# Ericonaldo/ILSwiss

Hardware: AMD Instinct MI355X
Metric: env-steps/s + SAC grad-steps/s, Hopper-v2 4096 envs (higher is better)
Workload: dtype f32

## Files before the change

ilswiss_amd/_lib.py:

```python
import ctypes as C
import os

_HERE = os.path.dirname(os.path.abspath(__file__))
LIB_PATH = os.path.join(_HERE, "libilsx.so")

c_f32p = C.POINTER(C.c_float)
c_u8p = C.POINTER(C.c_uint8)
c_i64p = C.POINTER(C.c_int64)
vp = C.c_void_p


class MlpCfg(C.Structure):
    _fields_ = [("in_dim", C.c_int32), ("n_hidden", C.c_int32), ("hidden", C.c_int32),
                ("out_dim", C.c_int32), ("n_heads", C.c_int32), ("act", C.c_int32), ("hidden_sizes", C.c_int32 * 3)]


class SacCfg(C.Structure):
    _fields_ = [("reward_scale", C.c_float), ("discount", C.c_float), ("policy_lr", C.c_float),
                ("qf_lr", C.c_float), ("alpha_lr", C.c_float), ("soft_target_tau", C.c_float),
                ("alpha", C.c_float), ("train_alpha", C.c_int32),
                ("policy_mean_reg_weight", C.c_float), ("policy_std_reg_weight", C.c_float),
                ("beta_1", C.c_float), ("has_target_entropy", C.c_int32), ("target_entropy", C.c_float),
                ("max_batch", C.c_int32), ("grad_world", C.c_int32)]

# ... 152 lines not shown


PROTOTYPES = {
    "ilsx_sac_group_create": (C.c_int, [vp, C.POINTER(vp), C.c_int, C.POINTER(vp)]),
    "ilsx_sac_group_destroy": (C.c_int, [vp]),
    "ilsx_sac_group_train_from_replay": (C.c_int, [vp, C.POINTER(vp), C.c_int, C.c_int, C.c_int]),
    "ilsx_advirl_train": (C.c_int, [vp, vp, vp, vp, C.c_int, C.c_int, C.c_int, C.c_int, C.c_int, C.c_int, C.c_int, C.c_float,
                                    C.c_int, C.c_float, C.POINTER(DiscStats), C.POINTER(SacStats), vp]),
    "ilsx_net_set_noise_policy": (C.c_int, [vp, C.c_float, C.c_float, C.c_float]),
    "ilsx_net_set_output_linear": (C.c_int, [vp, C.c_int]),
    "ilsx_td3_create": (C.c_int, [vp, C.POINTER(Td3Cfg), vp, vp, vp, C.POINTER(vp)]),
    "ilsx_td3_destroy": (C.c_int, [vp]),
    "ilsx_td3_train_step": (C.c_int, [vp, vp, vp, vp, vp, vp, C.c_int, vp, C.POINTER(Td3Stats)]),
    "ilsx_td3_train_from_replay": (C.c_int, [vp, vp, C.c_int, C.c_int, C.POINTER(Td3Stats)]),
    "ilsx_td3_get_params": (C.c_int, [vp, C.c_int, vp, C.c_size_t]),
    "ilsx_td3_set_params": (C.c_int, [vp, C.c_int, vp, C.c_size_t]),
    "ilsx_sacv_create": (C.c_int, [vp, C.POINTER(SacvCfg), vp, vp, vp, vp, C.POINTER(vp)]),
    "ilsx_sacv_destroy": (C.c_int, [vp]),
    "ilsx_sacv_train_step": (C.c_int, [vp, vp, vp, vp, vp, vp, C.c_int, vp, C.POINTER(SacvStats)]),
    "ilsx_sacv_train_from_replay": (C.c_int, [vp, vp, C.c_int, C.c_int, C.POINTER(SacvStats)]),
    "ilsx_sacv_get_params": (C.c_int, [vp, C.c_int, vp, C.c_size_t]),
    "ilsx_sacv_set_params": (C.c_int, [vp, C.c_int, vp, C.c_size_t]),
    "ilsx_bc_create": (C.c_int, [vp, C.POINTER(BcCfg), vp, C.POINTER(vp)]),
    "ilsx_bc_destroy": (C.c_int, [vp]),
    "ilsx_bc_train_step": (C.c_int, [vp, vp, vp, C.c_int, vp, C.POINTER(C.c_float)]),
    "ilsx_bc_train_from_replay": (C.c_int, [vp, vp, C.c_int, C.c_int, C.POINTER(C.c_float)]),
    "ilsx_ppo_create": (C.c_int, [vp, C.POINTER(PpoCfg), C.POINTER(vp)]),
    "ilsx_ppo_destroy": (C.c_int, [vp]),
    "ilsx_ppo_num_params": (C.c_int, [vp, C.c_int, C.POINTER(C.c_size_t)]),
    "ilsx_ppo_set_params": (C.c_int, [vp, C.c_int, vp, C.c_size_t]),
    "ilsx_ppo_get_params": (C.c_int, [vp, C.c_int, vp, C.c_size_t]),
    "ilsx_ppo_gae": (C.c_int, [vp, vp, vp, vp, vp, C.c_int, vp, vp, vp, vp, vp]),
    "ilsx_ppo_values": (C.c_int, [vp, vp, C.c_int, vp]),
    "ilsx_ppo_train": (C.c_int, [vp, vp, vp, vp, vp, C.c_int, vp, vp]),
    "ilsx_rollout_step_relabel": (C.c_int, [vp, vp, vp, C.c_int, vp, C.c_int, C.c_int]),
    "ilsx_eval_rollout": (C.c_int, [vp, vp, vp, C.c_int, C.c_int, C.c_int, vp]),
    "ilsx_ppo_rollout": (C.c_int, [vp, vp, C.c_int, C.c_int, vp, vp, vp, vp, vp]),
    "ilsx_vecenv_set_obs_affine": (C.c_int, [vp, vp, vp]),
    "ilsx_is_terminal": (C.c_int, [vp, C.c_int, vp, C.c_int, C.c_int, vp]),
    "ilsx_vecenv_obs_norm": (C.c_int, [vp, C.c_int, C.c_int]),
    "ilsx_vecenv_get_obs_rms": (C.c_int, [vp, vp, vp, C.POINTER(C.c_double)]),
    "ilsx_vecenv_set_obs_rms": (C.c_int, [vp, vp, vp, C.c_double]),
    "ilsx_ppo_debug_perm": (C.c_int, [vp, C.c_int, C.c_uint32, vp]),
    "ilsx_ppo_debug_grad_norm": (C.c_int, [vp, C.POINTER(C.c_float)]),
    "ilsx_ppo_policy_act": (C.c_int, [vp, vp, C.c_int, C.c_int, vp, vp, vp]),
    "ilsx_disc_create": (C.c_int, [vp, C.POINTER(DiscCfg), C.POINTER(vp)]),
    "ilsx_advirl_set_policy_batch_from_expert": (C.c_int, [vp, C.c_int]),
    "ilsx_her_gather": (C.c_int, [vp, vp, vp, C.c_int, C.c_int, C.c_int, C.c_int, C.c_int, C.c_int, C.c_float, vp, vp, vp, vp, vp]),
    "ilsx_debug_rng_stream": (C.c_int, [vp, C.c_int, C.POINTER(C.c_uint32), C.POINTER(C.c_uint64)]),
    "ilsx_debug_philox": (C.c_int, [vp, C.c_uint64, C.c_uint64, C.c_uint32, C.c_int, C.c_int, vp, vp]),
    "ilsx_disc_destroy": (C.c_int, [vp]),
    "ilsx_disc_num_params": (C.c_int, [vp, C.POINTER(C.c_size_t)]),
    "ilsx_disc_set_params": (C.c_int, [vp, vp, C.c_size_t]),
    "ilsx_disc_get_params": (C.c_int, [vp, vp, C.c_size_t]),
    "ilsx_disc_get_grads": (C.c_int, [vp, vp, C.c_size_t]),
    "ilsx_disc_get_bn_stats": (C.c_int, [vp, vp, vp, C.c_size_t]),
    "ilsx_disc_set_bn_stats": (C.c_int, [vp, vp, vp, C.c_size_t]),
    "ilsx_disc_train_step": (C.c_int, [vp, vp, vp, vp, vp, C.c_int, vp, C.POINTER(DiscStats)]),
    "ilsx_disc_reward": (C.c_int, [vp, vp, vp, C.c_int, C.c_int, C.c_int, C.c_float, C.c_int, C.c_float, vp, vp]),
    "ilsx_vecenv_create": (C.c_int, [vp, C.POINTER(PlanarModel), C.c_int, C.c_uint64, C.POINTER(vp)]),
    "ilsx_vecenv_create_spatial": (C.c_int, [vp, C.POINTER(SpatialModel), C.c_int, C.c_uint64, C.POINTER(vp)]),
    "ilsx_vecenv_state_dims": (C.c_int, [vp, C.POINTER(C.c_int), C.POINTER(C.c_int)]),
    "ilsx_vecenv_set_path_mode": (C.c_int, [vp, C.c_int]),
    "ilsx_vecenv_destroy": (C.c_int, [vp]),
    "ilsx_vecenv_dims": (C.c_int, [vp, C.POINTER(C.c_int), C.POINTER(C.c_int), C.POINTER(C.c_int), C.POINTER(C.c_int)]),
    "ilsx_vecenv_reset": (C.c_int, [vp, vp, C.c_int, vp]),
    "ilsx_vecenv_step": (C.c_int, [vp, vp, vp, C.c_int, vp, vp, vp]),
    "ilsx_vecenv_get_state": (C.c_int, [vp, vp, vp]),
    "ilsx_vecenv_set_state": (C.c_int, [vp, vp, vp]),
    "ilsx_vecenv_cur_obs": (C.c_int, [vp, C.POINTER(vp)]),
    "ilsx_rollout_step": (C.c_int, [vp, vp, vp, C.c_int, C.c_int, C.c_int, C.c_int]),
    "ilsx_rollout_step_begin": (C.c_int, [vp, vp, vp, C.c_int, C.c_int, C.c_int, C.c_int]),
    "ilsx_rollout_step_end": (C.c_int, [vp]),
    "ilsx_eval_rollouts_lockstep": (C.c_int, [C.POINTER(vp), C.POINTER(vp), C.c_int, C.c_int, C.c_int, C.c_int64, C.POINTER(C.c_double)]),
    "ilsx_rollout_steps_lockstep": (C.c_int, [C.POINTER(vp), C.POINTER(vp), C.POINTER(vp), C.c_int, C.c_int, C.c_int, C.POINTER(C.c_int64), C.c_int, C.c_int]),
    "ilsx_rollout_stats": (C.c_int, [vp, C.POINTER(C.c_double), C.POINTER(C.c_double), C.c_int]),
    "ilsx_abi_version": (C.c_int, []),
    "ilsx_last_error": (C.c_char_p, []),
    "ilsx_ctx_create": (C.c_int, [C.c_int, vp, C.c_uint64, C.POINTER(vp)]),
    "ilsx_ctx_sync": (C.c_int, [vp]),
    "ilsx_ctx_destroy": (C.c_int, [vp]),
    "ilsx_ctx_stream": (vp, [vp]),
    "ilsx_ctx_rng_stream_cursor": (C.c_int, [vp, C.c_uint32, C.POINTER(C.c_uint32)]),
    "ilsx_ctx_alloc": (C.c_int, [vp, C.c_size_t, C.POINTER(vp)]),
    "ilsx_ctx_free": (C.c_int, [vp, vp]),
    "ilsx_memcpy_h2d": (C.c_int, [vp, vp, vp, C.c_size_t]),
    "ilsx_memcpy_d2h": (C.c_int, [vp, vp, vp, C.c_size_t]),
    "ilsx_comm_unique_id": (C.c_int, [vp]),
    "ilsx_comm_init": (C.c_int, [vp, vp, C.c_int, C.c_int]),
    "ilsx_comm_destroy": (C.c_int, [vp]),
    "ilsx_comm_info": (C.c_int, [vp, C.POINTER(C.c_int), C.POINTER(C.c_int)]),
    "ilsx_comm_allreduce_sum": (C.c_int, [vp, vp, C.c_size_t]),
    "ilsx_td3_get_opt": (C.c_int, [vp, C.c_int, vp, vp, C.c_size_t, C.POINTER(OptMeta)]),
    "ilsx_td3_set_opt": (C.c_int, [vp, C.c_int, vp, vp, C.c_size_t, C.POINTER(OptMeta)]),
    "ilsx_sacv_get_opt": (C.c_int, [vp, C.c_int, vp, vp, C.c_size_t, C.POINTER(OptMeta)]),
    "ilsx_sacv_set_opt": (C.c_int, [vp, C.c_int, vp, vp, C.c_size_t, C.POINTER(OptMeta)]),
    "ilsx_bc_get_opt": (C.c_int, [vp, vp, vp, C.c_size_t, C.POINTER(OptMeta)]),
    "ilsx_bc_set_opt": (C.c_int, [vp, vp, vp, C.c_size_t, C.POINTER(OptMeta)]),
    "ilsx_ppo_get_opt": (C.c_int, [vp, C.c_int, vp, vp, C.c_size_t, C.POINTER(OptMeta)]),
    "ilsx_ppo_set_opt": (C.c_int, [vp, C.c_int, vp, vp, C.c_size_t, C.POINTER(OptMeta)]),
    "ilsx_disc_get_opt": (C.c_int, [vp, vp, vp, C.c_size_t, C.POINTER(OptMeta)]),
    "ilsx_disc_set_opt": (C.c_int, [vp, vp, vp, C.c_size_t, C.POINTER(OptMeta)]),
    "ilsx_prof_enable": (C.c_int, [vp, C.c_int]),
    "ilsx_prof_reset": (C.c_int, [vp]),
    "ilsx_prof_read": (C.c_int, [vp, C.c_int, C.POINTER(C.c_uint64), C.POINTER(C.c_double)]),
    "ilsx_prof_kernel": (C.c_char_p, [vp, C.c_int]),
    "ilsx_kernel_name": (C.c_char_p, [C.c_int]),
    "ilsx_debug_set_stamp_buffer": (C.c_int, [vp, vp, C.c_int, C.POINTER(C.c_int)]),
    "ilsx_debug_dw_split": (C.c_int, [C.c_int, C.c_int, C.POINTER(C.c_int), C.POINTER(C.c_int)]),
    "ilsx_net_create": (C.c_int, [vp, C.POINTER(MlpCfg), C.POINTER(vp)]),
    "ilsx_net_destroy": (C.c_int, [vp]),
    "ilsx_net_num_params": (C.c_int, [vp, C.POINTER(C.c_size_t)]),
    "ilsx_net_init": (C.c_int, [vp, C.c_uint64, C.c_float, C.c_float]),
    "ilsx_net_set_params": (C.c_int, [vp, vp, C.c_size_t, C.c_int]),
    "ilsx_net_get_params": (C.c_int, [vp, vp, C.c_size_t, C.c_int]),
    "ilsx_mlp_forward": (C.c_int, [vp, vp, C.c_int, vp]),
    "ilsx_policy_act": (C.c_int, [vp, vp, C.c_int, C.c_int, vp, vp, vp]),
    "ilsx_policy_log_prob": (C.c_int, [vp, vp, vp, C.c_int, vp]),
    "ilsx_replay_create": (C.c_int, [vp, C.c_int64, C.c_int, C.c_int, C.c_uint64, C.POINTER(vp)]),
    "ilsx_replay_destroy": (C.c_int, [vp]),
    "ilsx_replay_add": (C.c_int, [vp, vp, vp, vp, vp, vp, C.c_int, vp, C.c_int]),
    "ilsx_replay_terminate_episode": (C.c_int, [vp]),
    "ilsx_replay_set_absorbing": (C.c_int, [vp, C.c_int64, C.c_int, vp]),
    "ilsx_replay_get_absorbing": (C.c_int, [vp, vp, C.c_int, vp]),
    "ilsx_replay_sample": (C.c_int, [vp, C.c_int, vp, vp, vp, vp, vp, vp, vp]),
    "ilsx_replay_sample_many": (C.c_int, [vp, C.c_int, C.c_int, vp]),
    "ilsx_replay_record_floats": (C.c_int, [vp, C.POINTER(C.c_int)]),
    "ilsx_replay_size": (C.c_int, [vp, c_i64p, c_i64p]),
    "ilsx_replay_clear": (C.c_int, [vp]),
    "ilsx_replay_traj_endpoints": (C.c_int, [vp, c_i64p, c_i64p, C.c_int, C.POINTER(C.c_int)]),
    "ilsx_sac_create": (C.c_int, [vp, C.POINTER(SacCfg), vp, vp, vp, C.POINTER(vp)]),
    "ilsx_sac_destroy": (C.c_int, [vp]),
    "ilsx_sac_train_step": (C.c_int, [vp, vp, vp, vp, vp, vp, C.c_int, vp, vp, C.POINTER(SacStats)]),
    "ilsx_sac_train_from_replay": (C.c_int, [vp, vp, C.c_int, C.c_int, C.POINTER(SacStats)]),
    "ilsx_sac_set_batch": (C.c_int, [vp, vp, vp, vp, vp, vp, C.c_int, vp, vp]),
    "ilsx_sac_critic_backward": (C.c_int, [vp]),
    "ilsx_sac_critic_update": (C.c_int, [vp]),
    "ilsx_sac_actor_backward": (C.c_int, [vp]),
    "ilsx_sac_actor_update": (C.c_int, [vp]),
    "ilsx_sac_last_stats": (C.c_int, [vp, C.POINTER(SacStats)]),
    "ilsx_sac_get_params": (C.c_int, [vp, C.c_int, vp, C.c_size_t, C.c_int]),
    "ilsx_sac_set_params": (C.c_int, [vp, C.c_int, vp, C.c_size_t, C.c_int]),
    "ilsx_sac_get_grads": (C.c_int, [vp, C.c_int, vp, C.c_size_t, C.c_int]),
    "ilsx_sac_grads_ptr": (C.c_int, [vp, C.c_int, C.POINTER(vp), C.POINTER(C.c_size_t)]),
    "ilsx_sac_get_log_alpha": (C.c_int, [vp, C.POINTER(C.c_double)]),
    "ilsx_sac_set_log_alpha": (C.c_int, [vp, C.c_double]),
    "ilsx_sac_get_adam": (C.c_int, [vp, C.c_int, vp, vp, C.c_size_t, c_i64p]),
    "ilsx_sac_set_adam": (C.c_int, [vp, C.c_int, vp, vp, C.c_size_t, C.c_int64]),
    "ilsx_sac_get_alpha_opt": (C.c_int, [vp, C.POINTER(C.c_double), C.POINTER(C.c_double), c_i64p, C.POINTER(C.c_uint64)]),
    "ilsx_sac_debug_batch": (C.c_int, [vp, vp, C.c_uint64, C.c_int, vp, vp, vp, vp, vp, vp, vp, vp]),
    "ilsx_sac_debug_last_batch": (C.c_int, [vp, C.c_int, vp, vp, vp, vp, vp, vp]),
    "ilsx_sac_phase_state": (C.c_int, [vp, C.POINTER(C.c_int), C.POINTER(C.c_int), C.POINTER(C.c_int), C.POINTER(C.c_int), C.POINTER(C.c_int)]),
    "ilsx_sac_debug_break_phase": (C.c_int, [vp]),
    "ilsx_sac_set_alpha_opt": (C.c_int, [vp, C.c_double, C.c_double, C.c_int64, C.c_uint64]),
    "ilsx_bnn_create": (C.c_int, [vp, C.POINTER(BnnCfg), C.POINTER(vp)]),
    "ilsx_bnn_destroy": (C.c_int, [vp]),
    "ilsx_bnn_num_params": (C.c_int, [vp, C.POINTER(C.c_size_t)]),
    "ilsx_bnn_init": (C.c_int, [vp, C.c_uint64]),
    "ilsx_bnn_get_params": (C.c_int, [vp, vp, C.c_size_t]),
    "ilsx_bnn_set_params": (C.c_int, [vp, vp, C.c_size_t]),
    "ilsx_bnn_get_opt": (C.c_int, [vp, vp, vp, C.c_size_t, C.POINTER(OptMeta)]),
    "ilsx_bnn_set_opt": (C.c_int, [vp, vp, vp, C.c_size_t, C.POINTER(OptMeta)]),
    "ilsx_bnn_set_normalizer": (C.c_int, [vp, vp, vp]),
    "ilsx_bnn_get_normalizer": (C.c_int, [vp, vp, vp]),
    "ilsx_bnn_fit_stats": (C.c_int, [vp, vp, vp, C.c_int]),
    "ilsx_bnn_train_batch": (C.c_int, [vp, vp, vp, C.c_int64, C.c_int, vp]),
    "ilsx_bnn_mse": (C.c_int, [vp, vp, vp, C.c_int64, C.c_int, C.c_int, vp]),
    "ilsx_bnn_predict": (C.c_int, [vp, vp, C.c_int, vp, vp, C.c_int]),
    "ilsx_bnn_debug_padding": (C.c_int, [vp, C.POINTER(C.c_double)]),
    "ilsx_net_set_categorical": (C.c_int, [vp, C.c_int]),
    "ilsx_policy_log_pis": (C.c_int, [vp, vp, C.c_int, vp]),
    "ilsx_vecenv_create_classic": (C.c_int, [vp, C.c_int, C.c_int, C.c_uint64, C.POINTER(vp)]),
    "ilsx_vecenv_create_cartchain": (C.c_int, [vp, C.POINTER(CartChainModel), C.c_int, C.c_uint64, C.POINTER(vp)]),
    "ilsx_vecenv_create_swimmer": (C.c_int, [vp, C.POINTER(SwimmerModel), C.c_int, C.c_uint64, C.POINTER(vp)]),
    "ilsx_vecenv_action_space": (C.c_int, [vp, C.POINTER(C.c_int)]),
    "ilsx_dsac_create": (C.c_int, [vp, C.POINTER(DsacCfg), vp, vp, vp, C.POINTER(vp)]),
    "ilsx_dsac_destroy": (C.c_int, [vp]),
    "ilsx_dsac_train_step": (C.c_int, [vp, vp, vp, vp, vp, vp, C.c_int, C.POINTER(DsacStats)]),
    "ilsx_dsac_train_from_replay": (C.c_int, [vp, vp, C.c_int, C.c_int, C.POINTER(DsacStats)]),
    "ilsx_dsac_get_params": (C.c_int, [vp, C.c_int, vp, C.c_size_t]),
    "ilsx_dsac_set_params": (C.c_int, [vp, C.c_int, vp, C.c_size_t]),
    "ilsx_dsac_get_opt": (C.c_int, [vp, C.c_int, vp, vp, C.c_size_t, C.POINTER(OptMeta)]),
    "ilsx_dsac_set_opt": (C.c_int, [vp, C.c_int, vp, vp, C.c_size_t, C.POINTER(OptMeta)]),
    "ilsx_mbpo_model_step": (C.c_int, [vp, vp, vp, C.c_int, vp, vp, C.c_int, vp, C.c_int, C.c_int, vp, vp, vp, vp, vp,
                                       C.POINTER(C.c_int)]),
    "ilsx_her_horizon_gather": (C.c_int, [vp, vp, vp, C.c_int, C.c_int, C.c_int, C.c_int, C.c_int, vp, vp, vp]),
    "ilsx_bncat_create": (C.c_int, [vp, C.c_int, C.c_int, C.c_int, C.c_int, C.c_int, C.POINTER(vp)]),
    "ilsx_bncat_destroy": (C.c_int, [vp]),
    "ilsx_bncat_num_params": (C.c_int, [vp, C.POINTER(C.c_int)]),
    "ilsx_bncat_get": (C.c_int, [vp, C.c_int, vp, C.c_size_t]),
    "ilsx_bncat_set": (C.c_int, [vp, C.c_int, vp, C.c_size_t]),
    "ilsx_bncat_get_meta": (C.c_int, [vp, C.POINTER(C.c_int64), C.POINTER(C.c_uint64)]),
    "ilsx_bncat_set_meta": (C.c_int, [vp, C.c_int64, C.c_uint64]),
    "ilsx_bncat_input": (C.c_int, [vp, C.POINTER(vp), C.POINTER(vp)]),
    "ilsx_bncat_train_step": (C.c_int, [vp, C.c_int, C.c_float, vp]),
    "ilsx_bncat_act": (C.c_int, [vp, vp, C.c_int, C.c_int, vp, vp]),
    "ilsx_gcsl_create": (C.c_int, [vp, C.POINTER(GcslCfg), vp, vp, C.c_int, C.POINTER(vp)]),
    "ilsx_gcsl_destroy": (C.c_int, [vp]),
    "ilsx_gcsl_train_from_replay": (C.c_int, [vp, vp, vp, vp, C.c_int, vp]),
    "ilsx_gcsl_train_step": (C.c_int, [vp, vp, vp, C.c_int, vp]),
}

_lib = None


def load():
    global _lib
    if _lib is not None:
        return _lib
    path = os.environ.get("ILSX_LIB", LIB_PATH)
    if not os.path.exists(path):
        raise RuntimeError(
            f"{path} is missing: build it with `python -c 'import __graft_entry__ as g; g.build()'` "
            "or `make -C ilswiss_amd/csrc`.  ilswiss_amd has no CPU fallback.")
    lib = C.CDLL(path)
    for name, (res, args) in PROTOTYPES.items():
        fn = getattr(lib, name)
        fn.restype = res
        fn.argtypes = args
    if lib.ilsx_abi_version() != 1:
        raise RuntimeError(f"libilsx ABI {lib.ilsx_abi_version()} != 1")
    _lib = lib
    return lib


ILSX_ERR_UNSUPPORTED = -5


def check(rc):
    if rc != 0:
        msg = load().ilsx_last_error()
        raise RuntimeError(f"libilsx error {rc}: {msg.decode() if msg else '?'}")
```

ilswiss_amd/csrc/bwd_split_tile.inc:

```
  constexpr int NTH = 4 * H / CS, NWV = NTH / 64, NC = H / 16, SLW = H / CS, RPW = 16 / NWV, KPL = SLW / 64;
  constexpr int RPT = 16 * H / NTH, RSTEP = NTH / H;
  constexpr int LDH = H + ILSX_LDS_PAD, LDSL = SLW + ILSX_LDS_PAD;
  constexpr int MR = 16 * MT;
  static_assert(NTH % H == 0 && RPW >= 1 && KPL >= 1, "unsupported split geometry");
  static_assert(MT == 1 || MT == 2 || MT == 4, "macro tile = 1, 2 or 4 row tiles");
  const NetView& N = T.net;
  const int NO = N.NO;
  float* d1 = smem;
  float* d0s = d1 + MR * LDH;
  float* dout = d0s + MR * LDSL;
  if (bx & ((1u << A.xs) - 1u)) return;
  if ((int)(bx >> A.xs) * MR >= A.rows) return;
  const int tid = threadIdx.x, lane = tid & 63, wave = tid >> 6, li = lane & 15, g = lane >> 4;
  const int r0 = (bx >> A.xs) * MR, rows = A.rows;
  const bool lead = cs == 0;
  const bool full_tile = r0 + MR <= rows;
  ILSX_STAMP(A.dbg, 0);

  const int k1 = tid % H, rb1 = tid / H;
  const int lc = wave * 16 + li, col0 = cs * SLW + lc;
  float h1v[MT > 1 ? 2 : 1][RPT];
  float h0v[MT][4];
  float4 wreg[NC];
  constexpr int WHP = 12;
  float whp[WHP];
#pragma unroll
  for (int j = 0; j < WHP; ++j) whp[j] = (N.base + N.off_Wh)[(size_t)(j < NO ? j : 0) * H + k1];
  constexpr int DXT = 2;
  static_assert(SLW / 16 == NWV, "one k16 chunk of the slice per wave in the dL/dx phase");
  float w0b[DXT][4];
  if (T.dx) {
    const float* W0 = N.base + N.off_W[0];
    const int ld0 = N.ld[0];
#pragma unroll
    for (int t = 0; t < DXT; ++t)
#pragma unroll
      for (int s4 = 0; s4 < 4; ++s4) {
        const int c = 16 * t + li;
        w0b[t][s4] = c < T.dx_cols ? W0[pack_f(cs * SLW + 16 * wave + 4 * g + s4, T.dx_col0 + c, ld0)] : 0.0f;
      }
  }
  if constexpr (XCH) {
    {
      const float* wp = N.base + N.off_Wb[1] + (size_t)(cs * NWV + wave) * NC * 256 + 4 * lane;
#pragma unroll
      for (int c = 0; c < NC; ++c) wreg[c] = *reinterpret_cast<const float4*>(wp + 256 * c);
    }
  }
  XCH_HOOK_ACT
  {
    const float* const h1p = T.hsave[1] + (size_t)(r0 + rb1) * H + k1;
    const float* const h0p = T.hsave[0] + (size_t)(r0 + 4 * g) * H + col0;
    if (full_tile) {
#pragma unroll
      for (int i = 0; i < RPT; ++i) h1v[0][i] = ldx<XCH>(h1p + (size_t)(RSTEP * i) * H);
#pragma unroll
      for (int m = 0; m < MT; ++m)
#pragma unroll
        for (int v = 0; v < 4; ++v) h0v[m][v] = ldx<XCH>(h0p + (size_t)(16 * m + v) * H);
    } else {
#pragma unroll
      for (int i = 0; i < RPT; ++i) {
        const int gr = r0 + rb1 + RSTEP * i;
        h1v[0][i] = gr < rows ? ldx<XCH>(h1p + (size_t)(RSTEP * i) * H) : 0.0f;
      }
#pragma unroll
      for (int m = 0; m < MT; ++m)
#pragma unroll
        for (int v = 0; v < 4; ++v) {
          const int gr = r0 + 16 * m + 4 * g + v;
          h0v[m][v] = gr < rows ? ldx<XCH>(h0p + (size_t)(16 * m + v) * H) : 0.0f;
        }
    }
  }
  XCH_HOOK_HEAD
  for (int e = tid; e < MR * NO; e += NTH) {
    const int row = e / NO, j = e - row * NO, gr = r0 + row;
    float d = 0.0f;
    if (gr < rows) {
      d = bwd_head_grad<XCH>(T, A, gr, j, NO);
      if (T.dhead && lead) T.dhead[(size_t)gr * NO + j] = d;
    }
    dout[row * ILSX_MAX_NO + j] = d;
  }
  constexpr bool LATEW = GRP == 3 && MT == 1 && !XCH;
  if constexpr (!XCH && !LATEW) {
    {
      const float* wp = N.base + N.off_Wb[1] + (size_t)(cs * NWV + wave) * NC * 256 + 4 * lane;
#pragma unroll
      for (int c = 0; c < NC; ++c) wreg[c] = *reinterpret_cast<const float4*>(wp + 256 * c);
    }
  }
  lds_barrier();
  ILSX_STAMP(A.dbg, 1);
#pragma unroll
  for (int m = 0; m < MT; ++m) {
    if (m + 1 < MT) {
#pragma unroll
      for (int i = 0; i < RPT; ++i) {
        const int gr = r0 + 16 * (m + 1) + rb1 + RSTEP * i;
        h1v[(m + 1) & 1][i] = gr < rows ? T.hsave[1][(size_t)gr * H + k1] : 0.0f;
      }
    }
    const float* Wh = N.base + N.off_Wh;
    const float* dom = dout + 16 * m * ILSX_MAX_NO;
    float accd[RPT];
#pragma unroll
    for (int i = 0; i < RPT; ++i) accd[i] = 0.0f;
#pragma unroll
    for (int j = 0; j < WHP; ++j) {
      if (j < NO) {
#pragma unroll
        for (int i = 0; i < RPT; ++i) accd[i] = fmaf(dom[(rb1 + RSTEP * i) * ILSX_MAX_NO + j], whp[j], accd[i]);
      }
    }
#pragma unroll 4
    for (int j = WHP; j < NO; ++j) {
      const float w = Wh[(size_t)j * H + k1];
#pragma unroll
      for (int i = 0; i < RPT; ++i) accd[i] = fmaf(dom[(rb1 + RSTEP * i) * ILSX_MAX_NO + j], w, accd[i]);
    }
    float* ds = lead ? T.dsave[1] : nullptr;
    float* const dsp = ds ? ds + (size_t)(r0 + 16 * m + rb1) * H + k1 : nullptr;
    if (full_tile) {
#pragma unroll
      for (int i = 0; i < RPT; ++i) {
        const float dv = accd[i] * act_grad_from_out<ACT>(h1v[m & 1][i]);
        if (ds) dsp[(size_t)(RSTEP * i) * H] = dv;
        d1[(16 * m + rb1 + RSTEP * i) * LDH + k1] = dv;
      }
    } else {
#pragma unroll
      for (int i = 0; i < RPT; ++i) {
        const int row = 16 * m + rb1 + RSTEP * i, gr = r0 + row;
        float dv = 0.0f;
        if (gr < rows) {
          dv = accd[i] * act_grad_from_out<ACT>(h1v[m & 1][i]);
          if (ds) dsp[(size_t)(RSTEP * i) * H] = dv;
        }
        d1[row * LDH + k1] = dv;
      }
    }
  }
  if constexpr (LATEW) {
    const float* wp = N.base + N.off_Wb[1] + (size_t)(cs * NWV + wave) * NC * 256 + 4 * lane;
#pragma unroll
    for (int c = 0; c < NC; ++c) wreg[c] = *reinterpret_cast<const float4*>(wp + 256 * c);
  }
  lds_barrier();
  ILSX_STAMP(A.dbg, 2);
  {
    f32x4 acc0[MT], acc1[MT];
#pragma unroll
    for (int m = 0; m < MT; ++m) { acc0[m] = (f32x4){0.f, 0.f, 0.f, 0.f}; acc1[m] = acc0[m]; }
    const float* ap = d1 + li * LDH + 4 * g;
#pragma unroll
    for (int c = 0; c < NC; ++c) {
#pragma unroll
      for (int m = 0; m < MT; ++m) {
        const float4 a = *reinterpret_cast<const float4*>(ap + m * 16 * LDH + 16 * c);
        acc0[m] = MFMA16(a.x, wreg[c].x, acc0[m]); acc1[m] = MFMA16(a.y, wreg[c].y, acc1[m]);
        acc0[m] = MFMA16(a.z, wreg[c].z, acc0[m]); acc1[m] = MFMA16(a.w, wreg[c].w, acc1[m]);
      }
    }
    float* ds = T.dsave[0];
#pragma unroll
    for (int m = 0; m < MT; ++m) {
      float* const drow = ds ? ds + (size_t)(r0 + 16 * m + 4 * g) * H + col0 : nullptr;
      if (full_tile) {
#pragma unroll
        for (int v = 0; v < 4; ++v) {
          const float dv = (acc0[m][v] + acc1[m][v]) * act_grad_from_out<ACT>(h0v[m][v]);
          if (ds) drow[v * H] = dv;
          d0s[(16 * m + 4 * g + v) * LDSL + lc] = dv;
        }
      } else {
#pragma unroll
        for (int v = 0; v < 4; ++v) {
          const int row = 16 * m + 4 * g + v, gr = r0 + row;
          float dv = 0.0f;
          if (gr < rows) {
            dv = (acc0[m][v] + acc1[m][v]) * act_grad_from_out<ACT>(h0v[m][v]);
            if (ds) drow[v * H] = dv;
          }
          d0s[row * LDSL + lc] = dv;
        }
      }
    }
  }
  ILSX_STAMP(A.dbg, 3);
  if (T.dx) {
    lds_barrier();
    float* red = d1;
    const int ntile = (T.dx_cols + 15) >> 4;
#pragma unroll
    for (int m = 0; m < MT; ++m) {
      const float4 a4 = *reinterpret_cast<const float4*>(d0s + (16 * m + li) * LDSL + 16 * wave + 4 * g);
#pragma unroll
      for (int t = 0; t < DXT; ++t) {
        if (t < ntile) {
          f32x4 acc = (f32x4){0.f, 0.f, 0.f, 0.f};
          acc = MFMA16(a4.x, w0b[t][0], acc); acc = MFMA16(a4.y, w0b[t][1], acc);
          acc = MFMA16(a4.z, w0b[t][2], acc); acc = MFMA16(a4.w, w0b[t][3], acc);
#pragma unroll
          for (int v = 0; v < 4; ++v) red[(((m * DXT + t) * NWV + wave) * 4 + v) * 64 + lane] = acc[v];
        }
      }
    }
    lds_barrier();
#pragma unroll
    for (int m = 0; m < MT; ++m)
    for (int e = tid; e < ntile * 256; e += NTH) {
      const int t = e >> 8, v = (e >> 6) & 3, ol = e & 63;
      float sum = 0.0f;
#pragma unroll
      for (int w2 = 0; w2 < NWV; ++w2) sum += red[(((m * DXT + t) * NWV + w2) * 4 + v) * 64 + ol];
      const int row = 16 * m + 4 * (ol >> 4) + v, c = 16 * t + (ol & 15), gr = r0 + row;
      if (c < T.dx_cols && gr < rows) stx<XCH>(T.dx + ((size_t)cs * A.part_stride + gr) * T.dx_cols + c, sum);
    }
  }
  ILSX_STAMP(A.dbg, 7);
```

ilswiss_amd/csrc/fwd_split_tile.inc:

```
  constexpr int NTH = 4 * H / CS, NWV = NTH / 64, NC = H / 16, SLW = H / CS, NCS = SLW / 16;
  constexpr int NT0 = PH == 1 ? 1 : CS;
  constexpr int LDH = H + ILSX_LDS_PAD, LDSL = SLW + ILSX_LDS_PAD;
  constexpr int MR = 16 * MT;
  static_assert(NCS == NWV, "one k16 chunk of the slice per wave in the head phase");
  static_assert(MT == 1 || MT == 2 || MT == 4, "macro tile = 1, 2 or 4 row tiles");
  const DevScalars* scal = GRP ? GP->scal : A.scal;
  const NetView& N = T.net;
  const int KP = N.KP, LDX = KP + ILSX_LDS_PAD, NO = N.NO, NCH0 = KP >> 4, NOT = (NO + 15) >> 4;
  float* xs = smem;
  float* h0 = xs + (PH == 2 && MT > 1 ? 0 : MR * LDX);
  float* hs = h0 + (PH == 1 && MT > 1 ? 0 : MR * LDH);
  float* red = hs + MR * LDSL;
  const int RNT = MT == 1 ? 4 : NOT;
  if (bx & ((1u << A.xs) - 1u)) return;
  if ((int)(bx >> A.xs) * (A.rt > 0 ? A.rt : 1) * MR >= A.rows) return;
  const int tid = threadIdx.x, lane = tid & 63, wave = tid >> 6, li = lane & 15, g = lane >> 4;
  const int rows = A.rows;
  const int RT = A.rt > 0 ? A.rt : 1;
  const bool lead = cs == 0;
  ILSX_STAMP(A.dbg, 0);

  const int ct0 = PH == 1 ? cs * NWV + wave : wave * CS;
  const float* w0p = N.base + N.off_W[0] + (size_t)ct0 * NCH0 * 256 + 4 * lane;
  constexpr int L0D = 8;
  float4 b0[NT0], b0first[NT0];
  float4 l0first[PH == 1 ? L0D : 1];
  float bias0[NT0];
  if constexpr (PH == 1) {
#pragma unroll
    for (int d = 0; d < L0D; ++d) l0first[d] = *reinterpret_cast<const float4*>(w0p + (size_t)(d < NCH0 ? d : 0) * 256);
  }
  if constexpr (PH != 2) {
#pragma unroll
    for (int i = 0; i < NT0; ++i) b0[i] = *reinterpret_cast<const float4*>(w0p + (size_t)i * NCH0 * 256);
#pragma unroll
    for (int i = 0; i < NT0; ++i) b0first[i] = b0[i];
#pragma unroll
    for (int i = 0; i < NT0; ++i) bias0[i] = (N.base + N.off_b[0])[(ct0 + i) * 16 + li];
  }
  const int lc = wave * 16 + li, col1 = cs * SLW + lc;
  float bias1 = 0.0f;
  float4 whf[4];
  float4 wreg[NC];
  constexpr bool LATEW = GRP == 3 && MT == 1 && PH == 0;
  if constexpr (PH != 1) {
    bias1 = (N.base + N.off_b[1])[col1];
#pragma unroll
    for (int t = 0; t < 4; ++t) {
      const int j = 16 * t + li;
      whf[t] = (t < NOT && j < NO) ? *reinterpret_cast<const float4*>(N.base + N.off_Wh + (size_t)j * H + cs * SLW + 16 * wave + 4 * g)
                                   : make_float4(0.f, 0.f, 0.f, 0.f);
    }
    if constexpr (!LATEW) {
      const float* wp = N.base + N.off_W[1] + (size_t)(cs * NWV + wave) * NC * 256 + 4 * lane;
#pragma unroll
      for (int c = 0; c < NC; ++c) wreg[c] = *reinterpret_cast<const float4*>(wp + 256 * c);
    }
  }
#ifdef XCH_FINE_DBG
  ILSX_STAMP_SYNC(XCH_FINE_DBG, 6);
#endif
  const bool fin = (GRP ? GP->fin_on : A.fin_on) != 0 && !T.no_fin && T.d1 > 0;
  const GatherSpec& G = GRP ? GP->gather : A.gather;
  for (int rt = 0; rt < RT; ++rt) {
  const int r0 = ((bx >> A.xs) * RT + rt) * MR;
  if (r0 >= rows) break;
  const bool full_tile = r0 + MR <= rows;
  bool fin_logp = false;
  if constexpr (PH != 2) {
#pragma unroll
  for (int i = 0; i < NT0; ++i) b0[i] = b0first[i];
  XCH_HOOK_STAGE
  if constexpr (PH == 0) {
    long long* ridx0 = reinterpret_cast<long long*>(hs);
    if constexpr (MT > 1 || GRP != 0) {
      if (G.on) {
        if (tid < MR) ridx0[tid] = r0 + tid < rows ? replay_draw(G.seed, scal->gather_step, G.stream, (uint32_t)(r0 + tid), G.st->size) : 0;
        lds_barrier();
      }
    }
    for (int e = tid; e < MR * KP; e += NTH) {
      const int r = e / KP, k = e - r * KP, gr = r0 + r;
      const bool act_col = k >= T.d0 && k < T.d0 + T.d1;
      if (fin && act_col) continue;
      float v = 0.0f;
      if (gr < rows) {
        if (G.on) {
          long long idx;
          if constexpr (MT > 1 || GRP != 0) idx = ridx0[r];
          else idx = replay_draw(G.seed, scal->gather_step, G.stream, (uint32_t)gr, G.st->size);
          const float* rec = G.records + (size_t)idx * G.rec;
          if (k < T.d0) v = rec[T.g0_off + k];
          else if (act_col) v = rec[T.g1_off + (k - T.d0)];
          if (lead && T.publish == 1) {
            if (k < T.d0) G.s[(size_t)gr * G.o + k] = v;
            else if (act_col) G.a[(size_t)gr * G.adim + (k - T.d0)] = v;
            if (k == 0) { stx<XCH>(G.r + gr, rec[G.o + G.adim]); stx<XCH>(G.d + gr, rec[G.o + G.adim + 1]); }
          } else if (lead && T.publish == 2 && k < T.d0) {
            G.s2[(size_t)gr * G.o + k] = v;
          }
        } else {
          if (k < T.d0) v = T.x0[(size_t)gr * T.s0 + k];
          else if (act_col) v = T.x1[(size_t)gr * T.s1 + (k - T.d0)];
        }
        if (T.xsave && lead) T.xsave[(size_t)gr * KP + k] = v;
      }
      xs[r * LDX + k] = v;
    }
  } else {
    auto stage = [&](int r, int k, int gr, const float* rec) {
      const bool act_col = k >= T.d0 && k < T.d0 + T.d1;
      if (fin && act_col) return;
      float v = 0.0f;
      if (gr < rows) {
        if (G.on) {
          if (k < T.d0) v = rec[T.g0_off + k];
          else if (act_col) v = rec[T.g1_off + (k - T.d0)];
          if (lead && T.publish == 1) {
            if (k < T.d0) G.s[(size_t)gr * G.o + k] = v;
            else if (act_col) G.a[(size_t)gr * G.adim + (k - T.d0)] = v;
            if (k == 0) { G.r[gr] = rec[G.o + G.adim]; G.d[gr] = rec[G.o + G.adim + 1]; }
          } else if (lead && T.publish == 2 && k < T.d0) {
            G.s2[(size_t)gr * G.o + k] = v;
          }
        } else {
          if (k < T.d0) v = T.x0[(size_t)gr * T.s0 + k];
          else if (act_col) v = T.x1[(size_t)gr * T.s1 + (k - T.d0)];
        }
        if (T.xsave && lead) T.xsave[(size_t)gr * KP + k] = v;
      }
      xs[r * LDX + k] = v;
    };
    long long* ridx = reinterpret_cast<long long*>(hs);
    if (G.on) {
      if (tid < MR) ridx[tid] = r0 + tid < rows ? replay_draw(G.seed, scal->gather_step, G.stream, (uint32_t)(r0 + tid), G.st->size) : 0;
      lds_barrier();
    }
    if (KP <= 512 && T.d1 <= 64) {
      constexpr int RW = 16 / NWV, U = 8;
      const bool acts = T.d1 > 0 && !fin;
#pragma unroll
      for (int mt = 0; mt < MT; ++mt) {
      float vo[RW][U], va[RW];
#pragma unroll
      for (int rr = 0; rr < RW; ++rr) {
        const int r = 16 * mt + wave + NWV * rr, grc = r0 + r < rows ? r0 + r : rows - 1;
        const float* rec = G.on ? G.records + (size_t)ridx[r] * G.rec : nullptr;
        const float* s0p = G.on ? rec + T.g0_off : T.x0 + (size_t)grc * T.s0;
#pragma unroll
        for (int u = 0; u < U; ++u) { const int k = lane + 64 * u; vo[rr][u] = s0p[k < T.d0 ? k : T.d0 - 1]; }
        va[rr] = 0.0f;
        if (acts) { const float* s1p = G.on ? rec + T.g1_off : T.x1 + (size_t)grc * T.s1; va[rr] = s1p[lane < T.d1 ? lane : T.d1 - 1]; }
      }
#pragma unroll
      for (int rr = 0; rr < RW; ++rr) {
        const int r = 16 * mt + wave + NWV * rr, gr = r0 + r;
        const bool rowok = gr < rows;
        const bool pub1 = G.on && lead && T.publish == 1 && rowok, pub2 = G.on && lead && T.publish == 2 && rowok, xsv = T.xsave && lead && rowok;
#pragma unroll
        for (int u = 0; u < U; ++u) {
          const int k = lane + 64 * u;
          if (k < T.d0) {
            const float x = rowok ? vo[rr][u] : 0.0f;
            if (pub1) G.s[(size_t)gr * G.o + k] = x;
            if (pub2) G.s2[(size_t)gr * G.o + k] = x;
            if (xsv) T.xsave[(size_t)gr * KP + k] = x;
            xs[r * LDX + k] = x;
          }
        }
        if (acts && lane < T.d1) {
          const float x = rowok ? va[rr] : 0.0f;
          if (pub1) G.a[(size_t)gr * G.adim + lane] = x;
          if (xsv) T.xsave[(size_t)gr * KP + T.d0 + lane] = x;
          xs[r * LDX + T.d0 + lane] = x;
        }
        if (pub1 && lane == 0) { const float* rec = G.records + (size_t)ridx[r] * G.rec; G.r[gr] = rec[G.o + G.adim]; G.d[gr] = rec[G.o + G.adim + 1]; }
        for (int k = T.d0 + T.d1 + lane; k < KP; k += 64) {
          if (xsv) T.xsave[(size_t)gr * KP + k] = 0.0f;
          xs[r * LDX + k] = 0.0f;
        }
        if (T.d1 > 0 && !acts) {  }
      }
      }
    } else {
      for (int r = wave; r < MR; r += NWV) {
        const int gr = r0 + r;
        const float* rec = G.on ? G.records + (size_t)ridx[r] * G.rec : nullptr;
        for (int k = lane; k < KP; k += 64) stage(r, k, gr, rec);
      }
    }
  }
  XCH_HOOK_FIN
  if (fin) {
    const PolicyFinishArgs& P = GRP ? GP->fin : A.fin;
    const bool det = P.head == HEAD_DET_TANH_NOISE || P.head == HEAD_DET_LIN_NOISE;
    const int a = P.a, NOp = det ? a : 2 * a;
    const bool pub = lead && (GRP ? T.first != 0 : first_task);
    float* lp3 = red;
    const unsigned long long fstep = P.scal ? (P.use_gather_step ? P.scal->gather_step : P.scal->step) : P.step_host;
    const int LPS = MT == 1 ? 32 : a;
    for (int e = tid; e < MR * a; e += NTH) {
      const int row = e / a, j = e - row * a, gr = r0 + row;
      float act = 0.0f, c0 = 0.0f, c1 = 0.0f, c2 = 0.0f;
      if (gr < rows) {
        float pm[4], pl[4];
#pragma unroll
// ... 15 lines not shown
            const int q = j & 3;
            ep = q == 0 ? z4[0] : q == 1 ? z4[1] : q == 2 ? z4[2] : z4[3];
          }
        }
        if (det) {
          act = P.max_act * (P.head == HEAD_DET_LIN_NOISE ? mu : tanhf(mu));
          if (P.noise != 0.0f) act += fminf(fmaxf(P.noise * ep, -P.noise_clip), P.noise_clip);
          if (pub && P.raw) stx<XCH>(P.raw + (size_t)gr * a + j, mu);
        } else {
          const float ls = fminf(fmaxf(lsr, LOG_SIG_MIN), LOG_SIG_MAX);
          const float sd = expf(ls);
          const float z = ep * sd + mu;
          act = tanhf(z);
          const float dm = mu - z;
          c0 = dm * dm / expf(2.0f * ls); c1 = ls; c2 = logf(1.0f - act * act + TANH_EPS);
          if (pub && P.raw) { stx<XCH>(P.raw + (size_t)gr * NOp + j, mu); stx<XCH>(P.raw + (size_t)gr * NOp + a + j, lsr); }
        }
        if (T.xsave && lead) T.xsave[(size_t)gr * KP + T.d0 + j] = act;
        if (pub) {
          if (P.action) stx<XCH>(P.action + (size_t)gr * a + j, act);
          if (P.eps_save) stx<XCH>(P.eps_save + (size_t)gr * a + j, ep);
        }
      }
      xs[row * LDX + T.d0 + j] = act;
      lp3[(row * LPS + j) * 3 + 0] = c0; lp3[(row * LPS + j) * 3 + 1] = c1; lp3[(row * LPS + j) * 3 + 2] = c2;
    }
    fin_logp = pub && P.logp && !det;
  }
  }
  else {
    const float* hsrc = T.hsave[0];
    for (int e = tid; e < MR * (H / 4); e += NTH) {
      const int row = e / (H / 4), c4 = e - row * (H / 4), gr = r0 + row;
      const float4 v = gr < rows ? *reinterpret_cast<const float4*>(hsrc + (size_t)gr * H + 4 * c4) : make_float4(0.f, 0.f, 0.f, 0.f);
      *reinterpret_cast<float4*>(h0 + row * LDH + 4 * c4) = v;
    }
  }
  lds_barrier();
  ILSX_STAMP(A.dbg, 1);
  if (fin_logp && tid < MR && r0 + tid < rows) {
    const PolicyFinishArgs& P = GRP ? GP->fin : A.fin;
    float q = 0.f, l = 0.f, jc = 0.f;
    const int LPS = MT == 1 ? 32 : P.a;
    for (int j = 0; j < P.a; ++j) { q += red[(tid * LPS + j) * 3]; l += red[(tid * LPS + j) * 3 + 1]; jc += red[(tid * LPS + j) * 3 + 2]; }
    stx<XCH>(P.logp + r0 + tid, -0.5f * q - (l + HALF_LOG_2PI) - jc);
  }
  if constexpr (PH == 1) {
    f32x4 acc[MT];
#pragma unroll
    for (int m = 0; m < MT; ++m) acc[m] = (f32x4){0.f, 0.f, 0.f, 0.f};
    const float* ap = xs + li * LDX + 4 * g;
    float4 cur[L0D], nxt[L0D];
#pragma unroll
    for (int d = 0; d < L0D; ++d) cur[d] = l0first[d];
    for (int cb = 0; cb < NCH0; cb += L0D) {
#pragma unroll
      for (int d = 0; d < L0D; ++d) {
        const int c = cb + L0D + d;
        nxt[d] = *reinterpret_cast<const float4*>(w0p + (size_t)(c < NCH0 ? c : 0) * 256);
      }
#pragma unroll
      for (int d = 0; d < L0D; ++d) {
        if (cb + d < NCH0) {
#pragma unroll
          for (int m = 0; m < MT; ++m) {
            const float4 a = *reinterpret_cast<const float4*>(ap + m * 16 * LDX + 16 * (cb + d));
            acc[m] = MFMA16(a.x, cur[d].x, acc[m]); acc[m] = MFMA16(a.y, cur[d].y, acc[m]);
            acc[m] = MFMA16(a.z, cur[d].z, acc[m]); acc[m] = MFMA16(a.w, cur[d].w, acc[m]);
          }
        }
      }
#pragma unroll
      for (int d = 0; d < L0D; ++d) cur[d] = nxt[d];
    }
    float* hsv = T.hsave[0];
    const int col = ct0 * 16 + li;
#pragma unroll
    for (int m = 0; m < MT; ++m)
#pragma unroll
      for (int v = 0; v < 4; ++v) {
        const int row = 16 * m + 4 * g + v;
        if (r0 + row < rows) hsv[(size_t)(r0 + row) * H + col] = act_fn<ACT>(acc[m][v] + bias0[0]);
      }
  } else if constexpr (PH != 2) {
#pragma unroll
    for (int m = 0; m < MT; ++m) {
    f32x4 acc[NT0];
#pragma unroll
    for (int i = 0; i < NT0; ++i) acc[i] = (f32x4){0.f, 0.f, 0.f, 0.f};
    if (m > 0) {
#pragma unroll
      for (int i = 0; i < NT0; ++i) b0[i] = b0first[i];
    }
    const float* ap = xs + (16 * m + li) * LDX + 4 * g;
    for (int kc = 0; kc < KP; kc += 16) {
      float4 bn[NT0];
#pragma unroll
      for (int i = 0; i < NT0; ++i) {
        bn[i] = b0[i];
        if (kc + 16 < KP) bn[i] = *reinterpret_cast<const float4*>(w0p + (size_t)i * NCH0 * 256 + (kc + 16) * 16);
      }
      const float4 a = *reinterpret_cast<const float4*>(ap + kc);
#pragma unroll
      for (int i = 0; i < NT0; ++i) acc[i] = MFMA16(a.x, b0[i].x, acc[i]);
#pragma unroll
      for (int i = 0; i < NT0; ++i) acc[i] = MFMA16(a.y, b0[i].y, acc[i]);
#pragma unroll
      for (int i = 0; i < NT0; ++i) acc[i] = MFMA16(a.z, b0[i].z, acc[i]);
#pragma unroll
      for (int i = 0; i < NT0; ++i) acc[i] = MFMA16(a.w, b0[i].w, acc[i]);
#pragma unroll
      for (int i = 0; i < NT0; ++i) b0[i] = bn[i];
    }
    float* hsv = (PH == 1 || lead) ? T.hsave[0] : nullptr;
    float* const hrow = hsv ? hsv + (size_t)(r0 + 16 * m + 4 * g) * H + ct0 * 16 + li : nullptr;
#pragma unroll
    for (int i = 0; i < NT0; ++i) {
      const int col = (ct0 + i) * 16 + li;
#pragma unroll
      for (int v = 0; v < 4; ++v) {
        const int row = 16 * m + 4 * g + v;
        const float h = act_fn<ACT>(acc[i][v] + bias0[i]);
        if constexpr (PH == 0) h0[row * LDH + col] = h;
        acc[i][v] = h;
      }
    }
    if (hsv) {
      if (full_tile) {
#pragma unroll
        for (int i = 0; i < NT0; ++i)
#pragma unroll
          for (int v = 0; v < 4; ++v) stx<XCH>(hrow + v * H + i * 16, acc[i][v]);
      } else {
#pragma unroll
        for (int i = 0; i < NT0; ++i)
#pragma unroll
          for (int v = 0; v < 4; ++v)
            if (r0 + 16 * m + 4 * g + v < rows) stx<XCH>(hrow + v * H + i * 16, acc[i][v]);
      }
    }
    }
  }
  if constexpr (PH == 1) {
    lds_barrier();
    continue;
  }
  if constexpr (PH == 0) lds_barrier();
  ILSX_STAMP(A.dbg, 2);
  if constexpr (LATEW) {
    const float* wp = N.base + N.off_W[1] + (size_t)(cs * NWV + wave) * NC * 256 + 4 * lane;
#pragma unroll
    for (int c = 0; c < NC; ++c) wreg[c] = *reinterpret_cast<const float4*>(wp + 256 * c);
  }
  {
    f32x4 acc0[MT], acc1[MT];
#pragma unroll
    for (int m = 0; m < MT; ++m) { acc0[m] = (f32x4){0.f, 0.f, 0.f, 0.f}; acc1[m] = acc0[m]; }
    const float* ap = h0 + li * LDH + 4 * g;
#pragma unroll
    for (int c = 0; c < NC; ++c) {
#pragma unroll
      for (int m = 0; m < MT; ++m) {
        const float4 a = *reinterpret_cast<const float4*>(ap + m * 16 * LDH + 16 * c);
        acc0[m] = MFMA16(a.x, wreg[c].x, acc0[m]); acc1[m] = MFMA16(a.y, wreg[c].y, acc1[m]);
        acc0[m] = MFMA16(a.z, wreg[c].z, acc0[m]); acc1[m] = MFMA16(a.w, wreg[c].w, acc1[m]);
      }
    }
    float* hsv = T.hsave[1];
#pragma unroll
    for (int m = 0; m < MT; ++m) {
      float* const hrow = hsv ? hsv + (size_t)(r0 + 16 * m + 4 * g) * H + col1 : nullptr;
#pragma unroll
      for (int v = 0; v < 4; ++v) {
        const int row = 16 * m + 4 * g + v;
        const float h = act_fn<ACT>(acc0[m][v] + acc1[m][v] + bias1);
        hs[row * LDSL + lc] = h;
        acc0[m][v] = h;
      }
      if (hsv) {
        if (full_tile) {
#pragma unroll
          for (int v = 0; v < 4; ++v) stx<XCH>(hrow + v * H, acc0[m][v]);
        } else {
#pragma unroll
          for (int v = 0; v < 4; ++v)
            if (r0 + 16 * m + 4 * g + v < rows) stx<XCH>(hrow + v * H, acc0[m][v]);
        }
      }
    }
  }
  lds_barrier();
  ILSX_STAMP(A.dbg, 3);
#pragma unroll
  for (int m = 0; m < MT; ++m) {
    const float4 a = *reinterpret_cast<const float4*>(hs + (16 * m + li) * LDSL + 16 * wave + 4 * g);
#pragma unroll
    for (int t = 0; t < 4; ++t) {
      if (t < NOT) {
        f32x4 acc = (f32x4){0.f, 0.f, 0.f, 0.f};
        acc = MFMA16(a.x, whf[t].x, acc); acc = MFMA16(a.y, whf[t].y, acc);
        acc = MFMA16(a.z, whf[t].z, acc); acc = MFMA16(a.w, whf[t].w, acc);
#pragma unroll
        for (int v = 0; v < 4; ++v) red[(((m * RNT + t) * NWV + wave) * 4 + v) * 64 + lane] = acc[v];
      }
    }
  }
  lds_barrier();
  const float* bh = N.base + N.off_bh;
#pragma unroll
  for (int m = 0; m < MT; ++m)
  for (int e = tid; e < NOT * 256; e += NTH) {
    const int t = e >> 8, v = (e >> 6) & 3, ol = e & 63;
    float sum = 0.0f;
#pragma unroll
    for (int w2 = 0; w2 < NWV; ++w2) sum += red[(((m * RNT + t) * NWV + w2) * 4 + v) * 64 + ol];
    const int row = 16 * m + 4 * (ol >> 4) + v, j = 16 * t + (ol & 15), gr = r0 + row;
    if (j < NO && gr < rows) stx<XCH>(T.part + ((size_t)cs * A.part_stride + gr) * NO + j, sum + (lead ? bh[j] : 0.0f));
  }
  lds_barrier();
  }
  ILSX_STAMP(A.dbg, 7);
```

ilswiss_amd/csrc/ilsx_core.hip:

```cpp
#include <algorithm>
#include <cmath>
#include <cstdlib>
#include <random>

#define ILSX_KERNEL_IMPL 1
#include <mutex>
#include "host_common.h"

static thread_local std::string g_err = "";

void ilsx_set_err(const char* fmt, ...) {
  char buf[1024];
  va_list ap;
  va_start(ap, fmt);
  vsnprintf(buf, sizeof buf, fmt, ap);
  va_end(ap);
  g_err = buf;
}

static int kernels_init_once();
extern "C" int ilsx_abi_version(void) { return ILSX_ABI_VERSION; }
extern "C" const char* ilsx_last_error(void) { return g_err.c_str(); }

int ctx_alloc(ilsx_ctx* c, size_t bytes, void** out, bool zero) {
// ... 173 lines not shown
  static const char* names[ILSX_K_COUNT] = {"k_mlp_fwd", "k_mlp_bwd_dx", "k_mlp_bwd_dw", "k_adam_polyak",
      "k_replay_sample", "k_replay_add", "k_replay_sample_many", "k_sac_stats", "k_sac_finish", "k_env_step",
      "k_policy_finish", "k_disc_bwd", "k_ppo_gae", "k_sac_phase_a", "k_sac_phase_c", ""};
  return (kid >= 0 && kid < ILSX_K_COUNT) ? names[kid] : "";
}

static inline int round_up(int x, int m) { return (x + m - 1) / m * m; }

int net_layout_build(const ilsx_mlp_cfg& cfg, NetLayout* L) {
  if (cfg.n_hidden < 1 || cfg.n_hidden > ILSX_MAX_HID)
    ILSX_FAIL(ILSX_ERR_UNSUPPORTED, "n_hidden=%d not in 1..%d", cfg.n_hidden, ILSX_MAX_HID);
  if (cfg.hidden != 64 && cfg.hidden != 128 && cfg.hidden != 256)
    ILSX_FAIL(ILSX_ERR_UNSUPPORTED, "hidden=%d: supported widths are 64, 128, 256", cfg.hidden);
  if (cfg.in_dim < 1 || cfg.in_dim > 1024) ILSX_FAIL(ILSX_ERR_ARG, "in_dim=%d out of range", cfg.in_dim);
  if (cfg.n_heads < 1 || cfg.n_heads > 2 || cfg.out_dim < 1 || cfg.n_heads * cfg.out_dim > ILSX_MAX_NO)
    ILSX_FAIL(ILSX_ERR_UNSUPPORTED, "heads: n_heads=%d out_dim=%d (n_heads*out_dim must be <= %d)", cfg.n_heads,
              cfg.out_dim, ILSX_MAX_NO);
  if (cfg.act != ILSX_ACT_RELU && cfg.act != ILSX_ACT_TANH) ILSX_FAIL(ILSX_ERR_ARG, "act=%d unknown", cfg.act);
  L->cfg = cfg;
  for (int l = 0; l < ILSX_MAX_HID; ++l) {
    const int hs = l < cfg.n_hidden ? cfg.hidden_sizes[l] : 0;
    if (hs < 0 || hs > cfg.hidden) ILSX_FAIL(ILSX_ERR_UNSUPPORTED, "hidden_sizes[%d]=%d: 1..hidden=%d (0 = hidden)", l, hs, cfg.hidden);
    L->hl[l] = hs > 0 ? hs : (l < cfg.n_hidden ? cfg.hidden : 0);
    L->cfg.hidden_sizes[l] = l < cfg.n_hidden ? L->hl[l] : 0;
  }
  L->KP = round_up(cfg.in_dim, 16);
  L->NO = cfg.n_heads * cfg.out_dim;
  const int H = cfg.hidden;
  size_t off = 0, nflat = 0;
  for (int l = 0; l < cfg.n_hidden; ++l) {
    L->ld[l] = l == 0 ? L->KP : H;
    L->off_W[l] = (int)off;
    off += (size_t)H * L->ld[l];
    L->off_Wb[l] = 0;
    if (l > 0) {
      L->off_Wb[l] = (int)off;
      off += (size_t)H * H;
    }
    L->off_b[l] = (int)off;
    off += H;
    nflat += (size_t)L->out_of(l) * L->in_of(l) + L->out_of(l);
  }
  L->off_Wh = (int)off;
  off += (size_t)L->NO * H;
  L->off_bh = (int)off;
  off += round_up(L->NO, 4);
  nflat += (size_t)L->NO * L->out_of(cfg.n_hidden - 1) + L->NO;
  L->n_int = off;
  L->n_flat = nflat;
  return ILSX_OK;
}

void net_flat_to_internal(const NetLayout& L, const float* flat, float* in) {
  std::fill(in, in + L.n_int, 0.0f);
  const int H = L.cfg.hidden;
  size_t f = 0;
  for (int l = 0; l < L.cfg.n_hidden; ++l) {
    const int ind = L.in_of(l), outd = L.out_of(l);
    for (int n = 0; n < outd; ++n)
      for (int k = 0; k < ind; ++k) {
        const float v = flat[f + (size_t)n * ind + k];
        in[L.off_W[l] + pack_f(n, k, L.ld[l])] = v;
        if (l > 0) in[L.off_Wb[l] + pack_b(n, k, H)] = v;
      }
    f += (size_t)outd * ind;
    for (int n = 0; n < outd; ++n) in[L.off_b[l] + n] = flat[f + n];
    f += outd;
  }
  const int od = L.cfg.out_dim, hlast = L.out_of(L.cfg.n_hidden - 1);
  for (int h = 0; h < L.cfg.n_heads; ++h) {
    for (int j = 0; j < od; ++j)
      for (int k = 0; k < hlast; ++k) in[L.off_Wh + (size_t)(h * od + j) * H + k] = flat[f + (size_t)j * hlast + k];
    f += (size_t)od * hlast;
    for (int j = 0; j < od; ++j) in[L.off_bh + h * od + j] = flat[f + j];
    f += od;
  }
}

void net_internal_to_flat(const NetLayout& L, const float* in, float* flat) {
  const int H = L.cfg.hidden;
  size_t f = 0;
  for (int l = 0; l < L.cfg.n_hidden; ++l) {
    const int ind = L.in_of(l), outd = L.out_of(l);
    for (int n = 0; n < outd; ++n)
      for (int k = 0; k < ind; ++k) flat[f + (size_t)n * ind + k] = in[L.off_W[l] + pack_f(n, k, L.ld[l])];
    f += (size_t)outd * ind;
    for (int n = 0; n < outd; ++n) flat[f + n] = in[L.off_b[l] + n];
    f += outd;
  }
  const int od = L.cfg.out_dim, hlast = L.out_of(L.cfg.n_hidden - 1);
  for (int h = 0; h < L.cfg.n_heads; ++h) {
    for (int j = 0; j < od; ++j)
      for (int k = 0; k < hlast; ++k) flat[f + (size_t)j * hlast + k] = in[L.off_Wh + (size_t)(h * od + j) * H + k];
    f += (size_t)od * hlast;
    for (int j = 0; j < od; ++j) flat[f + j] = in[L.off_bh + h * od + j];
    f += od;
  }
}

NetView net_view(const NetLayout& L, float* base) {
  NetView v;
  v.base = base;
  for (int l = 0; l < ILSX_MAX_HID; ++l) {
    v.off_W[l] = l < L.cfg.n_hidden ? L.off_W[l] : 0;
    v.off_Wb[l] = l < L.cfg.n_hidden ? L.off_Wb[l] : 0;
    v.off_b[l] = l < L.cfg.n_hidden ? L.off_b[l] : 0;
    v.ld[l] = l < L.cfg.n_hidden ? L.ld[l] : 0;
  }
  v.off_Wh = L.off_Wh;
  v.off_bh = L.off_bh;
  v.nhid = L.cfg.n_hidden;
  v.H = L.cfg.hidden;
  v.in_dim = L.cfg.in_dim;
  v.KP = L.KP;
  v.NO = L.NO;
  return v;
}

static size_t fwd_lds_bytes(int H, int KP) {
  return sizeof(float) * (16 * (KP + ILSX_LDS_PAD) + 2 * 16 * (H + ILSX_LDS_PAD) + 16 * ILSX_MAX_NO);
}
static size_t bwd_lds_bytes(int H) { return sizeof(float) * (2 * 16 * (H + ILSX_LDS_PAD) + 16 * ILSX_MAX_NO); }

static int kernels_init_once() {
  static bool done = false;
  if (done) return ILSX_OK;
  const int cap = 160 * 1024;
#define SET_FWD(HH, AA) HIPCHK(hipFuncSetAttribute((const void*)k_mlp_fwd<HH, AA>, hipFuncAttributeMaxDynamicSharedMemorySize, cap))
  SET_FWD(64, ACT_RELU); SET_FWD(128, ACT_RELU); SET_FWD(256, ACT_RELU);
  SET_FWD(64, ACT_TANH); SET_FWD(128, ACT_TANH); SET_FWD(256, ACT_TANH);
#undef SET_FWD
  HIPCHK(hipFuncSetAttribute((const void*)k_mlp_bwd_dw<false, 2, 4>, hipFuncAttributeMaxDynamicSharedMemorySize, cap));
  HIPCHK(hipFuncSetAttribute((const void*)k_mlp_bwd_dw<true, 2, 4>, hipFuncAttributeMaxDynamicSharedMemorySize, cap));
  HIPCHK(hipFuncSetAttribute((const void*)k_mlp_bwd_dw_low<true, 2, 4>, hipFuncAttributeMaxDynamicSharedMemorySize, cap));
  HIPCHK(hipFuncSetAttribute((const void*)k_mlp_bwd_dw<true, 1, 2>, hipFuncAttributeMaxDynamicSharedMemorySize, cap));
  HIPCHK(hipFuncSetAttribute((const void*)k_mlp_bwd_dw<true, 1, 1>, hipFuncAttributeMaxDynamicSharedMemorySize, cap));
  HIPCHK(hipFuncSetAttribute((const void*)k_mlp_bwd_dw<true, 1, 4>, hipFuncAttributeMaxDynamicSharedMemorySize, cap));
  HIPCHK(hipFuncSetAttribute((const void*)k_mlp_bwd_dw<false, 1, 2>, hipFuncAttributeMaxDynamicSharedMemorySize, cap));
  HIPCHK(hipFuncSetAttribute((const void*)k_mlp_bwd_dw<false, 1, 1>, hipFuncAttributeMaxDynamicSharedMemorySize, cap));
#define SET_G(HH, AA, CC, GG) HIPCHK(hipFuncSetAttribute((const void*)k_mlp2_fwd_split<HH, AA, CC, GG>, hipFuncAttributeMaxDynamicSharedMemorySize, cap))
  SET_G(256, ACT_RELU, 4, 0); SET_G(256, ACT_RELU, 4, 1); SET_G(256, ACT_RELU, 4, 2); SET_G(256, ACT_RELU, 4, 3); SET_G(256, ACT_TANH, 4, 0); SET_G(256, ACT_TANH, 4, 1); SET_G(256, ACT_TANH, 4, 2); SET_G(256, ACT_TANH, 4, 3);
#define SET_PH(AA, GG) HIPCHK(hipFuncSetAttribute((const void*)k_mlp2_fwd_split<256, AA, 4, GG, 1>, hipFuncAttributeMaxDynamicSharedMemorySize, cap)); \
  HIPCHK(hipFuncSetAttribute((const void*)k_mlp2_fwd_split<256, AA, 4, GG, 2>, hipFuncAttributeMaxDynamicSharedMemorySize, cap))
  SET_PH(ACT_RELU, 0); SET_PH(ACT_RELU, 1); SET_PH(ACT_RELU, 2); SET_PH(ACT_TANH, 0); SET_PH(ACT_TANH, 1); SET_PH(ACT_TANH, 2);
#undef SET_PH
  SET_G(128, ACT_RELU, 2, 0); SET_G(128, ACT_RELU, 2, 1); SET_G(128, ACT_RELU, 2, 2); SET_G(128, ACT_RELU, 2, 3); SET_G(128, ACT_TANH, 2, 0); SET_G(128, ACT_TANH, 2, 1); SET_G(128, ACT_TANH, 2, 2); SET_G(128, ACT_TANH, 2, 3);
#undef SET_G
#define SET_MT(AA, MM) HIPCHK(hipFuncSetAttribute((const void*)k_mlp2_fwd_split<256, AA, 4, true, 0, MM>, hipFuncAttributeMaxDynamicSharedMemorySize, cap)); \
  HIPCHK(hipFuncSetAttribute((const void*)k_mlp2_fwd_split<256, AA, 4, true, 1, MM>, hipFuncAttributeMaxDynamicSharedMemorySize, cap)); \
  HIPCHK(hipFuncSetAttribute((const void*)k_mlp2_fwd_split<256, AA, 4, true, 2, MM>, hipFuncAttributeMaxDynamicSharedMemorySize, cap)); \
  HIPCHK(hipFuncSetAttribute((const void*)k_mlp2_bwd_split<256, AA, 4, true, MM>, hipFuncAttributeMaxDynamicSharedMemorySize, cap))
  SET_MT(ACT_RELU, 2); SET_MT(ACT_RELU, 4); SET_MT(ACT_TANH, 2); SET_MT(ACT_TANH, 4);
#undef SET_MT
#define SET_PHASE(HH, AA, CC) HIPCHK(hipFuncSetAttribute((const void*)k_sac_phase_a<HH, AA, CC>, hipFuncAttributeMaxDynamicSharedMemorySize, cap)); \
  HIPCHK(hipFuncSetAttribute((const void*)k_sac_phase_a<HH, AA, CC, true>, hipFuncAttributeMaxDynamicSharedMemorySize, cap)); \
  HIPCHK(hipFuncSetAttribute((const void*)k_sac_phase_c<HH, AA, CC, true>, hipFuncAttributeMaxDynamicSharedMemorySize, cap)); \
  HIPCHK(hipFuncSetAttribute((const void*)k_sac_phase_c<HH, AA, CC>, hipFuncAttributeMaxDynamicSharedMemorySize, cap))
  SET_PHASE(256, ACT_RELU, 4); SET_PHASE(256, ACT_TANH, 4); SET_PHASE(128, ACT_RELU, 2); SET_PHASE(128, ACT_TANH, 2);
#undef SET_PHASE
  done = true;
  return ILSX_OK;
}

#define DISPATCH_H_ACT(H, act, CALL)                                   \
  do {                                                                 \
    if (act == ILSX_ACT_RELU) {                                        \
      if (H == 64) { CALL(64, ACT_RELU); }                             \
      else if (H == 128) { CALL(128, ACT_RELU); }                      \
      else { CALL(256, ACT_RELU); }                                    \
    } else {                                                           \
      if (H == 64) { CALL(64, ACT_TANH); }                             \
      else if (H == 128) { CALL(128, ACT_TANH); }                      \
      else { CALL(256, ACT_TANH); }                                    \
    }                                                                  \
  } while (0)

extern "C" int ilsx_debug_set_stamp_buffer(ilsx_ctx* c, void* dev_trace, int max_launches, int* launches_so_far) {
  if (!c) ILSX_FAIL(ILSX_ERR_ARG, "ctx is NULL");
#ifndef ILSX_STAMPS
  if (dev_trace) ILSX_FAIL(ILSX_ERR_UNSUPPORTED, "this libilsx was built without stamps: make -C ilswiss_amd/csrc STAMPS=1 and load libilsx_stamps.so (ILSX_LIB)");
#endif
  if (launches_so_far) *launches_so_far = c->dbg_launches;
  c->dbg_stamps = (unsigned long long*)dev_trace;
  c->dbg_max_launches = dev_trace ? max_launches : 0;
  c->dbg_launches = 0;
  return ILSX_OK;
}

struct ConstSlots { std::vector<std::pair<int, int>> used; };
static ConstSlots g_slots[2][16];
int grp_const_alloc(int device, bool fwd, int n, int* base) {
  if (device < 0 || device >= 16 || n < 1 || n > GRP_CONST_SLOTS) return -1;
  auto& u = g_slots[fwd ? 0 : 1][device].used;
  int at = 0;
  size_t i = 0;
  for (; i < u.size(); ++i) { if (u[i].first - at >= n) break; at = u[i].first + u[i].second; }
  if (at + n > GRP_CONST_SLOTS) return -1;
  u.insert(u.begin() + i, {at, n});
  *base = at;
  return 0;
}
void grp_const_free(int device, bool fwd, int base) {
  if (device < 0 || device >= 16) return;
  auto& u = g_slots[fwd ? 0 : 1][device].used;
  for (size_t i = 0; i < u.size(); ++i) if (u[i].first == base) { u.erase(u.begin() + i); return; }
}
int grp_const_upload(ilsx_ctx* ctx, bool fwd, int base, const void* host, size_t count) {
  const size_t rec = fwd ? sizeof(FwdTaskG) : sizeof(BwdTask);
  if (fwd) HIPCHK(hipMemcpyToSymbolAsync(HIP_SYMBOL(g_fwd_tab), host, count * rec, (size_t)base * rec, hipMemcpyHostToDevice, ctx->stream));
  else HIPCHK(hipMemcpyToSymbolAsync(HIP_SYMBOL(g_bwd_tab), host, count * rec, (size_t)base * rec, hipMemcpyHostToDevice, ctx->stream));
  HIPCHK(hipStreamSynchronize(ctx->stream));
  return ILSX_OK;
}

int mlp2_split_factor(int n_hidden, int H) {
  if (n_hidden != 2) return 1;
  return H == 256 ? 4 : H == 128 ? 2 : 1;
}

static size_t fwd_split_lds_bytes(int H, int KP, int cs) {
  return sizeof(float) * (16 * (KP + ILSX_LDS_PAD) + 16 * (H + ILSX_LDS_PAD) + 16 * (H / cs + ILSX_LDS_PAD) +
                          4 * (4 * H / cs / 64) * 4 * 64);
}
static size_t bwd_split_lds_bytes(int H, int cs, int mt = 1) {
  return sizeof(float) * mt * (16 * (H + ILSX_LDS_PAD) + 16 * (H / cs + ILSX_LDS_PAD) + 16 * ILSX_MAX_NO);
}
static size_t fwd_split_lds_bytes_mt(int H, int KP, int cs, int mt, int ph, int not_max, int a_max) {
  const size_t mr = 16 * (size_t)mt, nwv = 4 * H / cs / 64;
  size_t fl = mr * (H / cs + ILSX_LDS_PAD);
  if (ph != 2) fl += mr * (KP + ILSX_LDS_PAD);
  if (ph != 1) fl += mr * (H + ILSX_LDS_PAD);
  const size_t part = ph == 1 ? 0 : (size_t)mt * std::max(not_max, 1) * nwv * 256, lp3 = ph == 2 ? 0 : mr * std::max(a_max, 1) * 3;
  fl += std::max(part, lp3);
  return sizeof(float) * fl;
}
static int grp_swizzle_fill(GrpSwizzle* S, int ntasks, int agents, int rows, int mt) {
  if (agents < 1 || ntasks % agents) ILSX_FAIL(ILSX_ERR_ARG, "grouped launch: %d tasks do not divide over %d agents", ntasks, agents);
  S->agents = agents; S->tpa = ntasks / agents; S->tiles = (rows + 16 * mt - 1) / (16 * mt);
  S->np8 = (agents * S->tiles + 7) / 8;
  return ILSX_OK;
}

int launch_fwd(ilsx_ctx* ctx, const FwdArgs& A0, int H, int act, int KPmax, int cs) {
  if (A0.rows <= 0) return ILSX_OK;
  FwdArgs A = A0;
  A.dbg = ctx->dbg_next();
  ProfScope ps(ctx, ILSX_K_MLP_FWD);
  if (cs > 1 && A.tasks && A.mt > 1) {
    if (!(H == 256 && cs == 4) || (A.mt != 2 && A.mt != 4)) ILSX_FAIL(ILSX_ERR_UNSUPPORTED, "macro-tile forward: H=%d cs=%d mt=%d", H, cs, A.mt);
    A.xs = 0; A.rt = 1; A.ctab = 0;
    ILSX_TRY(grp_swizzle_fill(&A.swz, A.ntasks, A.swz.agents, A.rows, A.mt));
    const unsigned nwork = 8u * A.swz.np8 * A.swz.tpa * cs;
    if (A.tail_mode && (!A.tail || A.tail_n < 1)) ILSX_FAIL(ILSX_ERR_ARG, "deferred tail: bad record table");
    const dim3 grid(nwork + (A.tail_mode ? A.tail_n : 0)), gridw(nwork), block(4 * H / cs);
#define MT_CALL(AA, PP, MM, GR, AR) do { const size_t lds = fwd_split_lds_bytes_mt(H, KPmax, cs, MM, PP, A.mt_not, A.mt_a); \
      if (lds > 160 * 1024) ILSX_FAIL(ILSX_ERR_UNSUPPORTED, "forward macro tile needs %zu B of LDS (> 160 KiB)", lds); \
      ILSX_LAUNCH(ps, (k_mlp2_fwd_split<256, AA, 4, true, PP, MM>), GR, block, lds, ctx->stream, AR); } while (0)
#define MT_CALL_PH(AA, MM) do { if (A.l0_split) { FwdArgs A2 = A; A2.tail_mode = 0; A2.tail = nullptr; A2.tail_n = 0; A2.dbg = ctx->dbg_next(); \
      MT_CALL(AA, 1, MM, grid, A); MT_CALL(AA, 2, MM, gridw, A2); } else { MT_CALL(AA, 0, MM, grid, A); } } while (0)
    if (act == ILSX_ACT_RELU) { if (A.mt == 2) MT_CALL_PH(ACT_RELU, 2); else MT_CALL_PH(ACT_RELU, 4); }
    else { if (A.mt == 2) MT_CALL_PH(ACT_TANH, 2); else MT_CALL_PH(ACT_TANH, 4); }
#undef MT_CALL_PH
#undef MT_CALL
    HIPCHK(hipGetLastError());
    return ILSX_OK;
  }
  if (cs > 1) {
    const size_t lds = fwd_split_lds_bytes(H, KPmax, cs);
    if (lds > 160 * 1024) ILSX_FAIL(ILSX_ERR_UNSUPPORTED, "forward tile needs %zu B of LDS (> 160 KiB)", lds);
    A.xs = ctx->xcd_shift;
    if (A.rt <= 0) A.rt = (A.tasks && ctx->rt_grouped > 0) ? ctx->rt_grouped : ctx->rt_single;
    const int tiles = (A.rows + 15) / 16;
    dim3 grid(((((tiles + A.rt - 1) / A.rt) + 7) & ~7) << A.xs, A.ntasks, cs), block(4 * H / cs);
    if (A.tail_mode) { if (!A.tail || A.tail_n < 1 || A.tail_n > (int)(grid.x * grid.z)) ILSX_FAIL(ILSX_ERR_ARG, "deferred tail: bad record table"); grid.y += 1; }
    if (A.late < 0) A.late = (long)tiles * A.ntasks * cs > 2L * device_cus(ctx);
    if (H == 256 && cs == 4 && A.l0_split) {
      FwdArgs A2 = A;
      A2.tail_mode = 0; A2.tail = nullptr; A2.tail_n = 0; A2.dbg = ctx->dbg_next();
      dim3 grid2(grid.x, A.ntasks, cs);
#define L0_CALL(AA, GG) do { ILSX_LAUNCH(ps, (k_mlp2_fwd_split<256, AA, 4, GG, 1>), grid, block, lds, ctx->stream, A); \
                             ILSX_LAUNCH(ps, (k_mlp2_fwd_split<256, AA, 4, GG, 2>), grid2, block, lds, ctx->stream, A2); } while (0)
      const int gg = A.tasks ? (A.ctab ? 2 : 1) : 0;
      if (act == ILSX_ACT_RELU) { if (gg == 2) L0_CALL(ACT_RELU, 2); else if (gg == 1) L0_CALL(ACT_RELU, 1); else L0_CALL(ACT_RELU, 0); }
      else { if (gg == 2) L0_CALL(ACT_TANH, 2); else if (gg == 1) L0_CALL(ACT_TANH, 1); else L0_CALL(ACT_TANH, 0); }
#undef L0_CALL
    } else if (H == 256 && cs == 4) {
#define FWD_GRP_CALL(HH, AA, CC) do { if (A.tasks && A.ctab && A.late) ILSX_LAUNCH(ps, (k_mlp2_fwd_split<HH, AA, CC, 3>), grid, block, lds, ctx->stream, A); \
        else if (A.tasks && A.ctab) ILSX_LAUNCH(ps, (k_mlp2_fwd_split<HH, AA, CC, 2>), grid, block, lds, ctx->stream, A); \
        else if (A.tasks) ILSX_LAUNCH(ps, (k_mlp2_fwd_split<HH, AA, CC, 1>), grid, block, lds, ctx->stream, A); \
        else ILSX_LAUNCH(ps, (k_mlp2_fwd_split<HH, AA, CC, 0>), grid, block, lds, ctx->stream, A); } while (0)
      if (act == ILSX_ACT_RELU) FWD_GRP_CALL(256, ACT_RELU, 4); else FWD_GRP_CALL(256, ACT_TANH, 4);
    } else if (H == 128 && cs == 2) {
      if (act == ILSX_ACT_RELU) FWD_GRP_CALL(128, ACT_RELU, 2); else FWD_GRP_CALL(128, ACT_TANH, 2);
#undef FWD_GRP_CALL
    } else {
      ILSX_FAIL(ILSX_ERR_UNSUPPORTED, "no column-split forward kernel for H=%d cs=%d", H, cs);
    }
    HIPCHK(hipGetLastError());
    return ILSX_OK;
  }
  const size_t lds = fwd_lds_bytes(H, KPmax);
  if (lds > 160 * 1024) ILSX_FAIL(ILSX_ERR_UNSUPPORTED, "forward tile needs %zu B of LDS (> 160 KiB)", lds);
  dim3 grid((A.rows + 15) / 16, A.ntasks), block(4 * H);
#define CALL_FWD(HH, AA) ILSX_LAUNCH(ps, (k_mlp_fwd<HH, AA>), grid, block, lds, ctx->stream, A)
  DISPATCH_H_ACT(H, act, CALL_FWD);
#undef CALL_FWD
  HIPCHK(hipGetLastError());
  return ILSX_OK;
}

int device_cus(ilsx_ctx* ctx) {
  static int n_cu = 0;
  if (!n_cu) {
    hipDeviceProp_t pr;
    n_cu = hipGetDeviceProperties(&pr, ctx->device) == hipSuccess ? pr.multiProcessorCount : 1;
  }
  return n_cu;
}
static size_t phase_lds_bytes(int H, int KP, int cs) { return std::max(fwd_split_lds_bytes(H, KP, cs), bwd_split_lds_bytes(H, cs)); }
void phase_wgs_per_cu(int H, int cs, int* occ_a, int* occ_c) {
  static int oa[2] = {-1, -1}, oc[2] = {-1, -1};
  const int i = H == 256 ? 0 : 1;
  if (oa[i] < 0) {
    int a = 0, c = 0;
    const size_t lds = phase_lds_bytes(H, 32, cs);
    hipError_t e1, e2;
    if (H == 256) { e1 = hipOccupancyMaxActiveBlocksPerMultiprocessor(&a, (const void*)k_sac_phase_a<256, ACT_RELU, 4>, 4 * H / cs, lds);
                    e2 = hipOccupancyMaxActiveBlocksPerMultiprocessor(&c, (const void*)k_sac_phase_c<256, ACT_RELU, 4>, 4 * H / cs, lds); }
    else { e1 = hipOccupancyMaxActiveBlocksPerMultiprocessor(&a, (const void*)k_sac_phase_a<128, ACT_RELU, 2>, 4 * H / cs, lds);
           e2 = hipOccupancyMaxActiveBlocksPerMultiprocessor(&c, (const void*)k_sac_phase_c<128, ACT_RELU, 2>, 4 * H / cs, lds); }
    oa[i] = e1 == hipSuccess ? std::max(a, 1) : 1;
    oc[i] = e2 == hipSuccess ? std::max(c, 1) : 1;
  }
  *occ_a = oa[i]; *occ_c = oc[i];
}
bool phase_fits(ilsx_ctx* ctx, int rows, int H, int cs, int ntasks) {
  const int n_cu = device_cus(ctx);
  if (!((H == 256 && cs == 4) || (H == 128 && cs == 2))) return false;
  const int tiles = (rows + 15) / 16, work = tiles * ntasks * cs;
  int occ_a = 1, occ_c = 1;
  phase_wgs_per_cu(H, cs, &occ_a, &occ_c);
  return tiles <= PHASE_MAX_TILES && work <= n_cu && work + 1 <= occ_a * n_cu && tiles * 3 * cs <= occ_c * n_cu;
}

static std::vector<bool> g_phase_slots[16];
static std::mutex g_phase_slots_mu;
int phase_const_alloc(int device) {
  static const bool off = []() { const char* e = getenv("ILSX_PHASE_CT"); return e && atoi(e) == 0; }();
  if (off || device < 0 || device >= 16) return -1;
  std::lock_guard<std::mutex> lock(g_phase_slots_mu);
  auto& u = g_phase_slots[device];
  if (u.empty()) u.assign(PHASE_CONST_SLOTS, false);
  for (int i = 0; i < PHASE_CONST_SLOTS; ++i) if (!u[i]) { u[i] = true; return i; }
  return -1;
}
void phase_const_free(int device, int slot) {
  if (device < 0 || device >= 16 || slot < 0 || slot >= PHASE_CONST_SLOTS) return;
  std::lock_guard<std::mutex> lock(g_phase_slots_mu);
  if (!g_phase_slots[device].empty()) g_phase_slots[device][slot] = false;
}
void phase_const_prepare(ilsx_ctx* ctx, PhaseConst* ct) {
  if (!ct || ct->tried) return;
  ct->tried = true;
  ct->device = ctx->device;
  ct->slot = phase_const_alloc(ctx->device);
  if (ct->slot >= 0) ctx->phase_slots.push_back(ct->slot);
}
template <class Blk>
static bool phase_const_ready(ilsx_ctx* ctx, PhaseConst* ct, const Blk& blk, unsigned long long key, Blk& held, bool& valid, unsigned long long& held_key,
                              const void* symbol) {
  phase_const_prepare(ctx, ct);
  if (!ct || ct->slot < 0 || blk.dbg || !key) return false;
  if (valid && held_key == key) return true;
  hipStreamCaptureStatus cap = hipStreamCaptureStatusNone;
  if (hipStreamIsCapturing(ctx->stream, &cap) != hipSuccess || cap != hipStreamCaptureStatusNone) return false;
  if (hipStreamSynchronize(ctx->stream) != hipSuccess) return false;
  valid = false;
  memcpy(&held, &blk, sizeof blk);
  if (hipMemcpyToSymbolAsync(symbol, &held, sizeof blk, (size_t)ct->slot * sizeof blk, hipMemcpyHostToDevice, ctx->stream) != hipSuccess ||
      hipStreamSynchronize(ctx->stream) != hipSuccess) { (void)hipGetLastError(); return false; }
  valid = true; held_key = key;
  return true;
}

int launch_phase_a(ilsx_ctx* ctx, const PhaseAArgs& P0, int H, int act, int KPmax, int cs, PhaseConst* ct, unsigned long long key, bool upload_only) {
  PhaseAArgs P = P0;
  P.f1.xs = P.f2.xs = P.b1.xs = 0; P.f1.rt = P.f2.rt = 1;
  P.f1.dbg = P.f2.dbg = nullptr; P.b1.dbg = nullptr;
  P.dbg = upload_only ? nullptr : ctx->dbg_next();
  if (P.b1.ga_parts < 1) P.b1.ga_parts = 1;
  const int tiles = (P.f1.rows + 15) / 16;
  dim3 grid((tiles + 7) & ~7, 5, cs), block(4 * H / cs);
  const size_t lds = phase_lds_bytes(H, KPmax, cs);
  const bool use_ct = ct && phase_const_ready(ctx, ct, P, key, ct->a, ct->valid_a, ct->key_a, HIP_SYMBOL(g_phase_a_tab));
  if (upload_only) return ILSX_OK;
  const int slot = use_ct ? ct->slot : 0;
  static const bool trace = getenv("ILSX_PHASE_CT_TRACE") != nullptr;
  if (trace) { hipStreamCaptureStatus cap = hipStreamCaptureStatusNone; hipStreamIsCapturing(ctx->stream, &cap);
               fprintf(stderr, "launch_phase_a: %s, slot %d, capturing %d\n", use_ct ? "constant table" : "kernel arguments", ct ? ct->slot : -9, (int)cap); }
  ProfScope ps(ctx, ILSX_K_SAC_PHASE_A);
#define PHASE_A(HH, AA, CC) do { if (use_ct) ILSX_LAUNCH(ps, (k_sac_phase_a<HH, AA, CC, true>), grid, block, lds, ctx->stream, P, slot); \
                                 else ILSX_LAUNCH(ps, (k_sac_phase_a<HH, AA, CC>), grid, block, lds, ctx->stream, P, slot); } while (0)
  if (H == 256 && act == ILSX_ACT_RELU) PHASE_A(256, ACT_RELU, 4);
  else if (H == 256) PHASE_A(256, ACT_TANH, 4);
  else if (act == ILSX_ACT_RELU) PHASE_A(128, ACT_RELU, 2);
  else PHASE_A(128, ACT_TANH, 2);
#undef PHASE_A
  HIPCHK(hipGetLastError());
  return ILSX_OK;
}

int launch_phase_c(ilsx_ctx* ctx, const PhaseCArgs& P0, int H, int act, int KPmax, int cs, PhaseConst* ct, unsigned long long key, bool upload_only) {
  PhaseCArgs P = P0;
  P.f3.xs = P.b2.xs = P.b3.xs = 0; P.f3.rt = 1;
  P.f3.dbg = nullptr; P.b2.dbg = P.b3.dbg = nullptr;
  P.dbg = upload_only ? nullptr : ctx->dbg_next();
  if (P.b2.ga_parts < 1) P.b2.ga_parts = 1;
  if (P.b3.ga_parts < 1) P.b3.ga_parts = 1;
  const int tiles = (P.f3.rows + 15) / 16;
  dim3 grid((tiles + 7) & ~7, 4, cs), block(4 * H / cs);
  const size_t lds = phase_lds_bytes(H, KPmax, cs);
  const bool use_ct = ct && phase_const_ready(ctx, ct, P, key, ct->c, ct->valid_c, ct->key_c, HIP_SYMBOL(g_phase_c_tab));
  if (upload_only) return ILSX_OK;
  const int slot = use_ct ? ct->slot : 0;
  ProfScope ps(ctx, ILSX_K_SAC_PHASE_C);
#define PHASE_C(HH, AA, CC) do { if (use_ct) ILSX_LAUNCH(ps, (k_sac_phase_c<HH, AA, CC, true>), grid, block, lds, ctx->stream, P, slot); \
                                 else ILSX_LAUNCH(ps, (k_sac_phase_c<HH, AA, CC>), grid, block, lds, ctx->stream, P, slot); } while (0)
  if (H == 256 && act == ILSX_ACT_RELU) PHASE_C(256, ACT_RELU, 4);
  else if (H == 256) PHASE_C(256, ACT_TANH, 4);
  else if (act == ILSX_ACT_RELU) PHASE_C(128, ACT_RELU, 2);
  else PHASE_C(128, ACT_TANH, 2);
#undef PHASE_C
  HIPCHK(hipGetLastError());
  return ILSX_OK;
}

int launch_bwd_dx(ilsx_ctx* ctx, const BwdArgs& A0, int H, int act, int cs) {
  if (A0.rows <= 0) return ILSX_OK;
  BwdArgs A = A0;
  A.dbg = ctx->dbg_next();
  if (A.ga_parts < 1) A.ga_parts = 1;
  ProfScope ps(ctx, ILSX_K_MLP_BWD_DX);
  if (cs > 1 && A.tasks && A.mt > 1) {
    if (!(H == 256 && cs == 4) || (A.mt != 2 && A.mt != 4)) ILSX_FAIL(ILSX_ERR_UNSUPPORTED, "macro-tile backward: H=%d cs=%d mt=%d", H, cs, A.mt);
    A.xs = 0; A.ctab = 0;
    ILSX_TRY(grp_swizzle_fill(&A.swz, A.ntasks, A.swz.agents, A.rows, A.mt));
    const dim3 grid(8u * A.swz.np8 * A.swz.tpa * cs), block(4 * H / cs);
    const size_t lds = bwd_split_lds_bytes(H, cs, A.mt);
    if (lds > 160 * 1024) ILSX_FAIL(ILSX_ERR_UNSUPPORTED, "backward macro tile needs %zu B of LDS (> 160 KiB)", lds);
    if (act == ILSX_ACT_RELU) { if (A.mt == 2) ILSX_LAUNCH(ps, (k_mlp2_bwd_split<256, ACT_RELU, 4, true, 2>), grid, block, lds, ctx->stream, A); else ILSX_LAUNCH(ps, (k_mlp2_bwd_split<256, ACT_RELU, 4, true, 4>), grid, block, lds, ctx->stream, A); }
    else { if (A.mt == 2) ILSX_LAUNCH(ps, (k_mlp2_bwd_split<256, ACT_TANH, 4, true, 2>), grid, block, lds, ctx->stream, A); else ILSX_LAUNCH(ps, (k_mlp2_bwd_split<256, ACT_TANH, 4, true, 4>), grid, block, lds, ctx->stream, A); }
    HIPCHK(hipGetLastError());
    return ILSX_OK;
  }
  if (cs > 1) {
    const size_t lds = bwd_split_lds_bytes(H, cs);
    A.xs = ctx->xcd_shift;
    dim3 grid(((((A.rows + 15) / 16) + 7) & ~7) << A.xs, A.ntasks, cs), block(4 * H / cs);
    if (A.late < 0) A.late = (long)((A.rows + 15) / 16) * A.ntasks * cs > 2L * device_cus(ctx);
    if (H == 256 && cs == 4) {
#define BWD_GRP_CALL(HH, AA, CC) do { if (A.tasks && A.ctab && A.late) ILSX_LAUNCH(ps, (k_mlp2_bwd_split<HH, AA, CC, 3>), grid, block, lds, ctx->stream, A); \
        else if (A.tasks && A.ctab) ILSX_LAUNCH(ps, (k_mlp2_bwd_split<HH, AA, CC, 2>), grid, block, lds, ctx->stream, A); \
        else if (A.tasks) ILSX_LAUNCH(ps, (k_mlp2_bwd_split<HH, AA, CC, 1>), grid, block, lds, ctx->stream, A); \
        else ILSX_LAUNCH(ps, (k_mlp2_bwd_split<HH, AA, CC, 0>), grid, block, lds, ctx->stream, A); } while (0)
      if (act == ILSX_ACT_RELU) BWD_GRP_CALL(256, ACT_RELU, 4); else BWD_GRP_CALL(256, ACT_TANH, 4);
    } else if (H == 128 && cs == 2) {
      if (act == ILSX_ACT_RELU) BWD_GRP_CALL(128, ACT_RELU, 2); else BWD_GRP_CALL(128, ACT_TANH, 2);
#undef BWD_GRP_CALL
    } else {
      ILSX_FAIL(ILSX_ERR_UNSUPPORTED, "no column-split backward kernel for H=%d cs=%d", H, cs);
    }
    HIPCHK(hipGetLastError());
    return ILSX_OK;
  }
  const size_t lds = bwd_lds_bytes(H);
  dim3 grid((A.rows + 15) / 16, A.ntasks), block(4 * H);
#define CALL_BWD(HH, AA) ILSX_LAUNCH(ps, (k_mlp_bwd_dx<HH, AA>), grid, block, lds, ctx->stream, A)
  DISPATCH_H_ACT(H, act, CALL_BWD);
#undef CALL_BWD
  HIPCHK(hipGetLastError());
  return ILSX_OK;
}

int launch_policy_finish(ilsx_ctx* ctx, const PolicyFinishArgs& P) {
  if (P.rows <= 0) return ILSX_OK;
  ProfScope ps(ctx, ILSX_K_POLICY_FINISH);
  ILSX_LAUNCH(ps, k_policy_finish, dim3((P.rows + 63) / 64), dim3(64), 0, ctx->stream, P);
  HIPCHK(hipGetLastError());
  return ILSX_OK;
}

void dw_split_plan(int rows, bool big, int* splits, int* rows_per_split) {
  const int unit = big ? DWB_RC : 128, cap = big ? 64 : 32;
  int s = rows / 512;
  if (s > cap) s = cap;
  if (s < 1) s = 1;
  const int rps = ((rows + s - 1) / s + unit - 1) / unit * unit;
  *rows_per_split = rps;
  *splits = (rows + rps - 1) / rps;
}
extern "C" int ilsx_debug_dw_split(int rows, int big, int* splits, int* rows_per_split) {
  if (rows < 1 || !splits || !rows_per_split) ILSX_FAIL(ILSX_ERR_ARG, "ilsx_debug_dw_split: bad argument");
  dw_split_plan(rows, big != 0, splits, rows_per_split);
  return ILSX_OK;
}

int launch_bwd_dw(ilsx_ctx* ctx, const DwArgs& table, int rows, const AdamFuse* fuse) {
  if (table.ntiles <= 0 || rows <= 0) return ILSX_OK;
  DwArgs D = table;
  D.rows_all = rows;
  memset(&D.F, 0, sizeof D.F);
  if (fuse) D.F = *fuse;
  D.dbg = ctx->dbg_next();
  D.xs = ctx->xcd_shift;
  D.splits = 1; D.rows_per_split = rows; D.scratch = nullptr; D.span = 0;
  bool stacked = false;
  for (int i = 0; i < D.nmat && !D.gtiles; ++i) stacked = stacked || D.m[i].rows > 0;
  if (rows >= DW_SPLIT_MIN_ROWS && D.g_lo && !stacked) {
    static const int big_env = []() { const char* e = getenv("ILSX_DW_BIG"); return e ? atoi(e) : 1; }();
    const bool big = big_env && rows >= DW_BIG_MIN_ROWS;
    int splits, rps;
    dw_split_plan(rows, big, &splits, &rps);
    const size_t span = (size_t)(D.g_hi - D.g_lo);
    const size_t need = (size_t)splits * span * sizeof(float);
    ilsx_ctx::DwScratch* reg = nullptr;
    for (auto& r : ctx->dw_scratch) if (r.key == D.g_lo && r.span == span) reg = &r;
    if (!reg) { ctx->dw_scratch.push_back({D.g_lo, span, nullptr, 0}); reg = &ctx->dw_scratch.back(); }
    if (reg->bytes < need) {
      if (reg->p) ILSX_TRY(ctx_free(ctx, reg->p));
      reg->p = nullptr; reg->bytes = 0;
      ILSX_TRY(ctx_alloc(ctx, need, &reg->p, true));
      reg->bytes = need;
    }
    D.splits = splits; D.rows_per_split = rps;
    D.scratch = (float*)reg->p; D.span = span; D.xs = 0;
    const AdamFuse keep = D.F;
    D.F.on = 0;
    if (big) {
      D.ntiles = 0;
      for (int i = 0; i < D.nmat; ++i) {
        D.m[i].ktiles = (D.m[i].NB + 127) / 128;
        D.m[i].tile0 = D.ntiles;
        D.ntiles += ((D.m[i].NA + 127) / 128) * D.m[i].ktiles;
      }
      ProfScope ps(ctx, ILSX_K_MLP_BWD_DW);
      ILSX_LAUNCH(ps, k_dw_big, dim3(D.ntiles * splits), dim3(256), 0, ctx->stream, D);
    } else {
      ProfScope ps(ctx, ILSX_K_MLP_BWD_DW);
      ILSX_LAUNCH(ps, (k_mlp_bwd_dw<false, 2, 4>), dim3(D.ntiles, splits), dim3(1024), DW_LDS_BYTES_OF(2, 4), ctx->stream, D);
    }
    DwReduceArgs R;
    R.scratch = D.scratch; R.splits = splits; R.span = span; R.g_lo = D.g_lo; R.F = keep;
    R.off0 = keep.on ? (size_t)(D.g_lo - keep.Gbase) : 0;
    int blocks = (int)((span / 4 + 63) / 64);
    if (blocks > 4096) blocks = 4096;
    ProfScope ps(ctx, ILSX_K_ADAM);
    ILSX_LAUNCH(ps, k_dw_reduce, dim3(blocks), dim3(256), 0, ctx->stream, R);
    HIPCHK(hipGetLastError());
    return ILSX_OK;
  }
  ProfScope ps(ctx, ILSX_K_MLP_BWD_DW);
  if (D.gtiles && D.strip) {
    bool whole = (rows & 255) == 0;
    if (whole) ILSX_LAUNCH(ps, (k_dw_strip<true, true>), dim3(D.ntiles), dim3(64), 0, ctx->stream, D);
    else ILSX_LAUNCH(ps, (k_dw_strip<true, false>), dim3(D.ntiles), dim3(64), 0, ctx->stream, D);
  } else if (D.gtiles) {
    const int gnh = D.tile_nh ? D.tile_nh : 2, gkt = D.tile_kt ? D.tile_kt : 4;
    const char* low_e = getenv("ILSX_DW_GRP_LOW");
    const int low_env = low_e ? atoi(low_e) : -1;
    const bool low = low_env >= 0 ? low_env != 0 : D.ntiles > device_cus(ctx);
    if (gnh == 2 && gkt == 4 && low) ILSX_LAUNCH(ps, (k_mlp_bwd_dw_low<true, 2, 4>), dim3(D.ntiles << D.xs), dim3(1024), DW_LDS_BYTES_OF(2, 4), ctx->stream, D);
    else if (gnh == 2 && gkt == 4) ILSX_LAUNCH(ps, (k_mlp_bwd_dw<true, 2, 4>), dim3(D.ntiles << D.xs), dim3(1024), DW_LDS_BYTES_OF(2, 4), ctx->stream, D);
    else if (gnh == 1 && gkt == 2) ILSX_LAUNCH(ps, (k_mlp_bwd_dw<true, 1, 2>), dim3(D.ntiles << D.xs), dim3(512), DW_LDS_BYTES_OF(1, 2), ctx->stream, D);
    else if (gnh == 1 && gkt == 1) ILSX_LAUNCH(ps, (k_mlp_bwd_dw<true, 1, 1>), dim3(D.ntiles << D.xs), dim3(512), DW_LDS_BYTES_OF(1, 1), ctx->stream, D);
    else if (gnh == 1 && gkt == 4) ILSX_LAUNCH(ps, (k_mlp_bwd_dw<true, 1, 4>), dim3(D.ntiles << D.xs), dim3(512), DW_LDS_BYTES_OF(1, 4), ctx->stream, D);
    else ILSX_FAIL(ILSX_ERR_UNSUPPORTED, "grouped dW tile %d x %d", gnh, gkt);
  } else {
    const char* shape_env = getenv("ILSX_DW_TILE");
    const int shape = shape_env ? atoi(shape_env) : 0;
    int nh = 2, kt = 4;
// ... 249 lines not shown
```

ilswiss_amd/csrc/ilsx_sac.hip:

```cpp
#include <cmath>
#include <cstdlib>

#include <algorithm>
#include "host_common.h"

enum { W_PI = 0, W_Q1 = 1, W_Q2 = 2, W_TQ1 = 3, W_TQ2 = 4 };

struct SacWs {
  float *s, *a, *r, *d, *s2, *eps1, *eps2;
  float *a2, *logp2, *q1, *q2, *tq1, *tq2;
  float *xq[2], *hq[2][ILSX_MAX_HID], *dq[2][ILSX_MAX_HID], *dhq[2];
  float *raw, *an, *logp, *epss, *q1n, *q2n, *ga[2];
  float *xp, *hp[ILSX_MAX_HID], *dp[ILSX_MAX_HID], *dhp;
  float* ppart;
  float* ppart2;
};

struct StatsArgs {
  PartVal q1, q2, tq1, tq2, q1n, q2n;
  const float *logp2, *r, *d, *logp, *raw;
  int B, a;
  float gamma, reward_scale, w_mu, w_std, target_entropy, inv_B;
  DevScalars* scal;
  float* alpha_grad_slot;
// ... 813 lines not shown
                                   const float* done, const float* nobs, int B, const float* eps_next,
                                   const float* eps_cur, ilsx_sac_stats* stats) {
  if (s) ILSX_TRY(sac_check_world(s, "ilsx_sac_train_step"));
  ILSX_TRY(ilsx_sac_set_batch(s, obs, act, rew, done, nobs, B, eps_next, eps_cur));
  if (stats) ILSX_TRY(sac_request_stats(s));
  ILSX_TRY(sac_full_step(s));
  if (stats) return sac_read_stats(s, stats);
  return ILSX_OK;
}

static bool sac_phase_ok(ilsx_sac* s, int B) {
  const bool off = getenv("ILSX_NO_PHASE") != nullptr;
  return !off && !s->phase_broken && s->cs > 1 && !s->h0scr && !s->col && s->defer_tail &&
         s->ctx->xcd_shift == 0 && phase_fits(s->ctx, B, s->Lq.cfg.hidden, s->cs, 4);
}
static bool sac_phase_possible(ilsx_sac* s, int B) {
  const bool off = getenv("ILSX_NO_PHASE") != nullptr;
  return !off && s->cs > 1 && !s->h0scr && phase_fits(s->ctx, B, s->Lq.cfg.hidden, s->cs, 4);
}
static size_t sac_snap_range(const ilsx_sac* s) { return (size_t)((const char*)(s->V + (2 * s->nq + s->np)) - (const char*)s->scal); }
int sac_snapshot_take(ilsx_sac* s) {
  const size_t n = sac_snap_range(s);
  if (!s->snap) { ILSX_TRY(ctx_alloc(s->ctx, n, &s->snap, false)); s->snap_bytes = n; }
  HIPCHK(hipMemcpyAsync(s->snap, s->scal, n, hipMemcpyDeviceToDevice, s->ctx->stream));
  s->snap_valid = true;
  return ILSX_OK;
}
int sac_snapshot_restore(ilsx_sac* s) {
  if (!s->snap || !s->snap_valid) ILSX_FAIL(ILSX_ERR_STATE, "no checkpoint of this window to roll back to");
  s->snap_valid = false;
  HIPCHK(hipMemcpyAsync(s->scal, s->snap, s->snap_bytes, hipMemcpyDeviceToDevice, s->ctx->stream));
  HIPCHK(hipMemsetAsync(s->phase_flags, 0, (size_t)PHASE_FLAG_WORDS * sizeof(unsigned), s->ctx->stream));
  return ILSX_OK;
}
bool sac_window_may_use_phase(ilsx_sac* s, int B) { return !s->phase_broken && s->cs > 1 && !s->col && sac_phase_possible(s, B) && s->ctx->xcd_shift == 0; }
static int sac_phase_check(ilsx_sac* s, int B, bool deferred, const char* who, bool teardown) {
  hipStream_t st = s->ctx->stream;
  struct SnapGuard { ilsx_sac* s; bool keep = false; ~SnapGuard() { if (!keep) s->snap_valid = false; } } snap_guard{s};
  if (deferred && s->snap_valid && !teardown) {
    int err = 0;
    unsigned masks[PHASE_MAX_TILES * 32];
    HIPCHK(hipMemcpyAsync(&err, s->phase_err, sizeof err, hipMemcpyDeviceToHost, st));
    HIPCHK(hipMemcpyAsync(masks, s->phase_flags + PHASE_MASK_WORD(0), sizeof masks, hipMemcpyDeviceToHost, st));
    HIPCHK(hipStreamSynchronize(st));
    for (int t = 0; t < PHASE_MAX_TILES; ++t)
      if (masks[t * 32] & (masks[t * 32] - 1)) err |= 2;
    if (s->debug_break) { err |= 1; s->debug_break = false; }
    if (sac_is_split(s) && s->ctx->comm && s->ctx->comm_n > 1) {
      if (!s->vote) ILSX_TRY(ctx_alloc(s->ctx, 4 * sizeof(float), (void**)&s->vote, true));
      float v = err ? 1.0f : 0.0f;
      HIPCHK(hipMemcpyAsync(s->vote, &v, sizeof v, hipMemcpyHostToDevice, st));
      ILSX_TRY(comm_allreduce_sum(s->ctx, s->vote, 1));
      HIPCHK(hipMemcpyAsync(&v, s->vote, sizeof v, hipMemcpyDeviceToHost, st));
      HIPCHK(hipStreamSynchronize(st));
      if (v > 0.0f) err |= 4;
    }
    if (err) {
      s->phase_broken = true;
      if (s->graph) { hipGraphExecDestroy(s->graph); s->graph = nullptr; }
      HIPCHK(hipMemsetAsync(s->phase_err, 0, sizeof(int), st));
      if (getenv("ILSX_PHASE_VERBOSE"))
        fprintf(stderr, "[ilsx] %s: a merged phase kernel %s; the window is rolled back and re-run, this agent stays on one launch per stage\n", who,
                (err & 1) ? "timed out waiting for the workgroups of its tile (other kernels sharing this GPU?)"
                : (err & 2) ? "found the workgroups of one row tile on different XCDs" : "broke on another rank of this split run");
      s->phase_fallbacks += 1;
      snap_guard.keep = true;
      return ILSX_RETRY_WINDOW;
    }
  }
  return ILSX_OK;
}

static int sac_phase_const_prime(ilsx_sac* s, ilsx_replay* rb) {
  phase_const_prepare(s->ctx, &s->pct);
  if (s->pct.slot < 0 || s->cs <= 1) return ILSX_OK;
  static const bool no_fuse = getenv("ILSX_NO_FUSE") != nullptr;
  s->gather_rb = rb; s->phase_now = true; s->fuse_now = !no_fuse && !sac_is_split(s);
  s->phase_args_only = true;
  int rc = sac_critic_backward(s);
  if (rc == ILSX_OK) rc = sac_actor_backward(s);
  s->phase_args_only = false;
  s->gather_rb = nullptr; s->phase_now = false; s->fuse_now = false;
  return rc;
}

static int sac_sample_and_step(ilsx_sac* s, ilsx_replay* rb, int B) {
  const SacWs& w = s->ws;
  if (s->cs > 1) {
    s->gather_rb = rb;
    s->phase_now = sac_phase_ok(s, B);
    s->phase_last = s->phase_now;
    const int rc = sac_full_step(s);
    s->gather_rb = nullptr;
    s->phase_now = false;
    return rc;
  }
  ILSX_TRY(replay_launch_sample(rb, B, nullptr, s->scal, 0, w.s, w.a, w.r, w.d, w.s2, nullptr));
  return sac_full_step(s);
}

static int sac_train_from_replay_once(ilsx_sac* s, ilsx_replay* rb, int n_steps, int B, ilsx_sac_stats* stats);
static int sac_split_segment(ilsx_sac* s, ilsx_replay* rb, int B, int seg) {
  s->fuse_now = false;
  if (seg == 0) {
    if (s->cs > 1) s->gather_rb = rb;
    else { const SacWs& w = s->ws; ILSX_TRY(replay_launch_sample(rb, B, nullptr, s->scal, 0, w.s, w.a, w.r, w.d, w.s2, nullptr)); }
    const int rc = sac_critic_backward(s);
    s->gather_rb = nullptr;
    return rc;
  }
  if (seg == 1) { ILSX_TRY(sac_critic_update(s)); return sac_actor_backward(s); }
  return sac_actor_update(s);
}
static int sac_split_segments_step(ilsx_sac* s, ilsx_replay* rb, int B) {
  hipStream_t st = s->ctx->stream;
  if (s->seg_rb != rb || s->seg_B != B || !s->seg_graph[0]) {
    for (hipGraphExec_t& g : s->seg_graph) if (g) { hipGraphExecDestroy(g); g = nullptr; }
    for (int seg = 0; seg < 3; ++seg) {
      hipGraph_t g = nullptr;
      HIPCHK(hipStreamBeginCapture(st, hipStreamCaptureModeThreadLocal));
      s->no_ct = true;
      const int rc = sac_split_segment(s, rb, B, seg);
      s->no_ct = false;
      const hipError_t e = hipStreamEndCapture(st, &g);
      if (rc != ILSX_OK) { if (g) hipGraphDestroy(g); return rc; }
      if (e != hipSuccess) ILSX_FAIL(ILSX_ERR_HIP, "hipStreamEndCapture (split segment %d) failed: %s", seg, hipGetErrorString(e));
      const hipError_t e2 = hipGraphInstantiate(&s->seg_graph[seg], g, nullptr, nullptr, 0);
      hipGraphDestroy(g);
      if (e2 != hipSuccess) { s->seg_graph[seg] = nullptr; ILSX_FAIL(ILSX_ERR_HIP, "hipGraphInstantiate (split segment %d) failed: %s", seg, hipGetErrorString(e2)); }
    }
    s->seg_rb = rb; s->seg_B = B;
  }
  HIPCHK(hipGraphLaunch(s->seg_graph[0], st));
  ILSX_TRY(sac_allreduce(s, 0));
  HIPCHK(hipGraphLaunch(s->seg_graph[1], st));
  ILSX_TRY(sac_allreduce(s, 1));
  HIPCHK(hipGraphLaunch(s->seg_graph[2], st));
  return ILSX_OK;
}

extern "C" int ilsx_sac_train_from_replay(ilsx_sac* s, ilsx_replay* rb, int n_steps, int B, ilsx_sac_stats* stats) {
  if (stats && n_steps > 1) {
    ILSX_TRY(ilsx_sac_train_from_replay(s, rb, 1, B, stats));
    return ilsx_sac_train_from_replay(s, rb, n_steps - 1, B, nullptr);
  }
  int rc = sac_train_from_replay_once(s, rb, n_steps, B, stats);
  if (rc == ILSX_RETRY_WINDOW) {
    ILSX_TRY(sac_snapshot_restore(s));
    rc = sac_train_from_replay_once(s, rb, n_steps, B, stats);
    if (rc == ILSX_RETRY_WINDOW) ILSX_FAIL(ILSX_ERR_STATE, "ilsx_sac_train_from_replay: the fallback path asked for a retry");
  }
  return rc;
}
void phase_wgs_per_cu(int H, int cs, int* occ_a, int* occ_c);
extern "C" int ilsx_sac_phase_state(ilsx_sac* s, int* fallbacks, int* disabled, int* last_window_on_phase, int* wgs_per_cu_a, int* wgs_per_cu_c) {
  if (!s) ILSX_FAIL(ILSX_ERR_ARG, "ilsx_sac_phase_state: NULL agent");
  if (fallbacks) *fallbacks = s->phase_fallbacks;
  if (disabled) *disabled = s->phase_broken ? 1 : 0;
  if (last_window_on_phase) *last_window_on_phase = s->phase_last ? 1 : 0;
  int oa = 0, oc = 0;
  if (s->cs > 1 && (s->Lq.cfg.hidden == 256 || s->Lq.cfg.hidden == 128)) phase_wgs_per_cu(s->Lq.cfg.hidden, s->cs, &oa, &oc);
  if (wgs_per_cu_a) *wgs_per_cu_a = oa;
  if (wgs_per_cu_c) *wgs_per_cu_c = oc;
  return ILSX_OK;
}
extern "C" int ilsx_sac_debug_break_phase(ilsx_sac* s) {
  if (!s) ILSX_FAIL(ILSX_ERR_ARG, "ilsx_sac_debug_break_phase: NULL agent");
  static const int one = 1;
  HIPCHK(hipSetDevice(s->ctx->device));
  HIPCHK(hipMemcpyAsync(s->phase_err, &one, sizeof one, hipMemcpyHostToDevice, s->ctx->stream));
  s->debug_break = true;
  return ILSX_OK;
}
static int sac_train_from_replay_once(ilsx_sac* s, ilsx_replay* rb, int n_steps, int B, ilsx_sac_stats* stats) {
  if (!s || !rb || n_steps < 0) ILSX_FAIL(ILSX_ERR_ARG, "ilsx_sac_train_from_replay: bad argument");
  if (B < 1 || B > s->cfg.max_batch) ILSX_FAIL(ILSX_ERR_ARG, "batch %d not in 1..max_batch=%d", B, s->cfg.max_batch);
  if (rb->o != s->o || rb->a != s->a) ILSX_FAIL(ILSX_ERR_ARG, "replay dims (%d,%d) != agent dims (%d,%d)", rb->o, rb->a, s->o, s->a);
  if (rb->size < 1) ILSX_FAIL(ILSX_ERR_STATE, "replay buffer is empty");
  ILSX_TRY(sac_check_world(s, "ilsx_sac_train_from_replay"));
  HIPCHK(hipSetDevice(s->ctx->device));
  ILSX_TRY(replay_flush_state(rb));
  hipStream_t st = s->ctx->stream;
  s->B = B;
  s->eps_explicit = false;
  static const bool split_graph = getenv("ILSX_SPLIT_GRAPH") != nullptr;
  static const bool no_graph_env = getenv("ILSX_NO_GRAPH") != nullptr;
  const bool no_graph = no_graph_env || (sac_is_split(s) && !split_graph);
  if (n_steps == 0) return stats ? sac_read_stats(s, stats) : ILSX_OK;
  ILSX_TRY(sac_defer_begin(s, B));
  struct DeferGuard { ilsx_sac* s; ~DeferGuard() { s->defer_tail = false; } } guard{s};
  const bool deferred = s->defer_tail;
  if (deferred && sac_window_may_use_phase(s, B)) ILSX_TRY(sac_snapshot_take(s));
  static const bool segments = []() { const char* e = getenv("ILSX_SPLIT_SEGMENTS"); return e && atoi(e) != 0; }();
  if (sac_is_split(s) && !split_graph && !no_graph_env && segments && !s->ctx->prof_on) {
    for (int i = 0; i < n_steps; ++i) {
      if (stats && i == n_steps - 1) ILSX_TRY(sac_request_stats(s));
      ILSX_TRY(sac_split_segments_step(s, rb, B));
    }
  } else if (no_graph || s->ctx->prof_on) {
    for (int i = 0; i < n_steps; ++i) {
      if (stats && i == n_steps - 1) ILSX_TRY(sac_request_stats(s));
      const int rc = sac_sample_and_step(s, rb, B);
      if (rc != ILSX_OK) return rc;
    }
  } else {
    const bool phase = sac_phase_ok(s, B);
    s->phase_last = phase;
    static const bool no_reprime = getenv("ILSX_PHASE_CT_NO_REPRIME") != nullptr;
    const bool rebuild = !s->graph || s->graph_rb != rb || s->graph_B != B || s->graph_defer != s->defer_tail || s->graph_phase != phase;
    if (phase && (rebuild || !no_reprime)) ILSX_TRY(sac_phase_const_prime(s, rb));
    if (!s->graph || s->graph_rb != rb || s->graph_B != B || s->graph_defer != s->defer_tail || s->graph_phase != phase) {
      if (s->graph) { hipGraphExecDestroy(s->graph); s->graph = nullptr; }
      hipGraph_t g = nullptr;
      HIPCHK(hipStreamBeginCapture(st, hipStreamCaptureModeThreadLocal));
      int rc = sac_sample_and_step(s, rb, B);
      hipError_t e = hipStreamEndCapture(st, &g);
      if (rc != ILSX_OK) { if (g) hipGraphDestroy(g); return rc; }
      if (e != hipSuccess) ILSX_FAIL(ILSX_ERR_HIP, "hipStreamEndCapture failed: %s", hipGetErrorString(e));
      e = hipGraphInstantiate(&s->graph, g, nullptr, nullptr, 0);
      hipGraphDestroy(g);
      if (e != hipSuccess) { s->graph = nullptr; ILSX_FAIL(ILSX_ERR_HIP, "hipGraphInstantiate failed: %s", hipGetErrorString(e)); }
      s->graph_rb = rb; s->graph_B = B; s->graph_defer = s->defer_tail; s->graph_phase = phase;
    }
    for (int i = 0; i < n_steps; ++i) {
      if (stats && i == n_steps - 1) ILSX_TRY(sac_request_stats(s));
      HIPCHK(hipGraphLaunch(s->graph, st));
    }
  }
  s->defer_tail = false;
  ILSX_TRY(sac_flush_tail(s, deferred));
  ILSX_TRY(sac_phase_check(s, B, deferred, "ilsx_sac_train_from_replay"));
  if (stats) return sac_read_stats(s, stats);
  return ILSX_OK;
}

static const NetLayout* sac_layout(const ilsx_sac* s, int which) { return which == W_PI ? &s->Lp : &s->Lq; }

extern "C" int ilsx_sac_get_params(ilsx_sac* s, int which, float* dst, size_t n, int dst_is_device) {
  if (!s || !dst || which < 0 || which > 4) ILSX_FAIL(ILSX_ERR_ARG, "ilsx_sac_get_params: bad argument");
  HIPCHK(hipSetDevice(s->ctx->device));
  return net_download_flat(s->ctx, *sac_layout(s, which), s->base(which), dst, n, dst_is_device);
}
extern "C" int ilsx_sac_set_params(ilsx_sac* s, int which, const float* src, size_t n, int src_is_device) {
  if (!s || !src || which < 0 || which > 4) ILSX_FAIL(ILSX_ERR_ARG, "ilsx_sac_set_params: bad argument");
  HIPCHK(hipSetDevice(s->ctx->device));
  return net_upload_flat(s->ctx, *sac_layout(s, which), s->base(which), src, n, src_is_device);
}
extern "C" int ilsx_sac_get_grads(ilsx_sac* s, int which, float* dst, size_t n, int dst_is_device) {
  if (!s || !dst || which < 0 || which > 2) ILSX_FAIL(ILSX_ERR_ARG, "ilsx_sac_get_grads: bad argument");
  HIPCHK(hipSetDevice(s->ctx->device));
  return net_download_flat(s->ctx, *sac_layout(s, which), s->gbase(which), dst, n, dst_is_device);
}
extern "C" int ilsx_sac_grads_ptr(ilsx_sac* s, int segment, float** dev_ptr, size_t* n) {
  if (!s || !dev_ptr || !n || segment < 0 || segment > 1) ILSX_FAIL(ILSX_ERR_ARG, "ilsx_sac_grads_ptr: bad argument");
  if (segment == 0) { *dev_ptr = s->G; *n = 2 * s->nq; }
  else { *dev_ptr = s->G + 2 * s->nq; *n = s->np + 4; }
  return ILSX_OK;
}
extern "C" int ilsx_sac_get_log_alpha(ilsx_sac* s, double* out) {
  if (!s || !out) ILSX_FAIL(ILSX_ERR_ARG, "NULL argument");
  HIPCHK(hipSetDevice(s->ctx->device));
  DevScalars h;
  HIPCHK(hipMemcpyAsync(&h, s->scal, sizeof h, hipMemcpyDeviceToHost, s->ctx->stream));
  HIPCHK(hipStreamSynchronize(s->ctx->stream));
  *out = h.log_alpha;
  return ILSX_OK;
}
extern "C" int ilsx_sac_set_log_alpha(ilsx_sac* s, double v) {
  if (!s) ILSX_FAIL(ILSX_ERR_ARG, "NULL argument");
  HIPCHK(hipSetDevice(s->ctx->device));
  DevScalars h;
  HIPCHK(hipMemcpyAsync(&h, s->scal, sizeof h, hipMemcpyDeviceToHost, s->ctx->stream));
  HIPCHK(hipStreamSynchronize(s->ctx->stream));
  h.log_alpha = v;
  h.alpha = (float)std::exp(v);
  HIPCHK(hipMemcpyAsync(s->scal, &h, sizeof h, hipMemcpyHostToDevice, s->ctx->stream));
  HIPCHK(hipStreamSynchronize(s->ctx->stream));
  return ILSX_OK;
}
extern "C" int ilsx_sac_get_adam(ilsx_sac* s, int which, float* m_host, float* v_host, size_t n, int64_t* t) {
  if (!s || !m_host || !v_host || which < 0 || which > 2) ILSX_FAIL(ILSX_ERR_ARG, "ilsx_sac_get_adam: bad argument");
  HIPCHK(hipSetDevice(s->ctx->device));
  const size_t off = s->trainable_off(which);
  ILSX_TRY(net_download_flat(s->ctx, *sac_layout(s, which), s->M + off, m_host, n, 0));
  ILSX_TRY(net_download_flat(s->ctx, *sac_layout(s, which), s->V + off, v_host, n, 0));
  if (t) {
    DevScalars h;
    HIPCHK(hipMemcpyAsync(&h, s->scal, sizeof h, hipMemcpyDeviceToHost, s->ctx->stream));
    HIPCHK(hipStreamSynchronize(s->ctx->stream));
    *t = which == W_PI ? h.t_pi : h.t_q;
  }
  return ILSX_OK;
}
extern "C" int ilsx_sac_set_adam(ilsx_sac* s, int which, const float* m_host, const float* v_host, size_t n, int64_t t) {
  if (!s || !m_host || !v_host || which < 0 || which > 2) ILSX_FAIL(ILSX_ERR_ARG, "ilsx_sac_set_adam: bad argument");
  HIPCHK(hipSetDevice(s->ctx->device));
  const size_t off = s->trainable_off(which);
  ILSX_TRY(net_upload_flat(s->ctx, *sac_layout(s, which), s->M + off, m_host, n, 0));
  ILSX_TRY(net_upload_flat(s->ctx, *sac_layout(s, which), s->V + off, v_host, n, 0));
  DevScalars h;
  HIPCHK(hipMemcpyAsync(&h, s->scal, sizeof h, hipMemcpyDeviceToHost, s->ctx->stream));
  HIPCHK(hipStreamSynchronize(s->ctx->stream));
  if (which == W_PI) h.t_pi = (int)t; else h.t_q = (int)t;
  HIPCHK(hipMemcpyAsync(s->scal, &h, sizeof h, hipMemcpyHostToDevice, s->ctx->stream));
  HIPCHK(hipStreamSynchronize(s->ctx->stream));
  return sac_refresh_adam(s);
}
extern "C" int ilsx_sac_get_alpha_opt(ilsx_sac* s, double* m, double* v, int64_t* t, uint64_t* rng_step) {
  if (!s) ILSX_FAIL(ILSX_ERR_ARG, "NULL argument");
  HIPCHK(hipSetDevice(s->ctx->device));
  DevScalars h;
  HIPCHK(hipMemcpyAsync(&h, s->scal, sizeof h, hipMemcpyDeviceToHost, s->ctx->stream));
  HIPCHK(hipStreamSynchronize(s->ctx->stream));
  if (m) *m = h.m_alpha;
// ... 395 lines not shown
```

ilswiss_amd/csrc/kernels.h:

```cpp
#pragma once
#include <hip/hip_runtime.h>
#include <stdint.h>

typedef float f32x4 __attribute__((ext_vector_type(4)));

#define ILSX_LDS_PAD 4
#ifndef ILSX_LATE_WAVES
#define ILSX_LATE_WAVES 4
#endif
#ifndef ILSX_MT_WAVES
#define ILSX_MT_WAVES 2
#endif
#define ILSX_MAX_HID 3
#define ILSX_MAX_NO 64

enum { HEAD_RAW = 0, HEAD_TANH_SAMPLE = 1, HEAD_TANH_DET = 2, HEAD_TANH_LOGP_OF_ACT = 3,
       HEAD_GAUSS_SAMPLE = 4, HEAD_GAUSS_LOGP_OF_ACT = 5,
       HEAD_DET_TANH_NOISE = 6,
       HEAD_DET_LIN_NOISE = 7 };
enum { LOSS_GIVEN = 0, LOSS_SAC_CRITIC = 1, LOSS_SAC_ACTORQ = 2, LOSS_SAC_POLICY = 3, LOSS_MSE = 4, LOSS_PPO_POLICY = 5,
       LOSS_TD_CRITIC = 6, LOSS_SACV_VALUE = 7, LOSS_CONST = 8, LOSS_TD3_POLICY = 9, LOSS_BC_MLE = 10, LOSS_BC_MSE = 11 };
enum { ACT_RELU = 0, ACT_TANH = 1 };

#define LOG_SIG_MIN (-20.0f)
// ... 797 lines not shown
  int sw_bx = 0, sw_task = 0, sw_cs = 0;
  if constexpr (GRP && MT > 1) {
    const unsigned nwork = 8u * A.swz.np8 * A.swz.tpa * CS;
    if (blockIdx.x >= nwork) {
      const int ag = blockIdx.x - nwork;
      if (A.tail_mode && ag < A.tail_n) {
        const TailLite& TL = A.tail[ag];
        if (A.tail_mode == 1) tail_lite_run(TL, smem);
        else if (threadIdx.x == 0) TL.scal->gather_step += 1;
      }
      return;
    }
    if (!grp_swizzle(A.swz, CS, blockIdx.x, &sw_bx, &sw_task, &sw_cs)) return;
  } else {
  if (A.tail_mode && (int)blockIdx.y == A.ntasks) {
    const int ag = blockIdx.x + gridDim.x * blockIdx.z;
    if (ag < A.tail_n) {
      const TailLite& TL = A.tail[ag];
      if (A.tail_mode == 1) tail_lite_run(TL, smem);
      else if (threadIdx.x == 0) TL.scal->gather_step += 1;
    }
    return;
  }
  }
  FwdTaskG Rg;
  const int ty = (GRP && MT > 1) ? sw_task : (int)blockIdx.y;
  if (GRP == 1) Rg = A.tasks[ty];
  const FwdTaskG& Rc = g_fwd_tab[GRP >= 2 ? A.ctab - 1 + ty : 0];
  const FwdTask& T = GRP >= 2 ? Rc.t : GRP == 1 ? Rg.t : A.t[ty];
  const FwdGroup* GP = GRP >= 2 ? &Rc.g : GRP == 1 ? &Rg.g : nullptr;
  constexpr bool XCH = false;
  const int bx = (GRP && MT > 1) ? sw_bx : (int)blockIdx.x, cs = (GRP && MT > 1) ? sw_cs : (int)blockIdx.z;
  const bool first_task = ty == 0;
#define XCH_HOOK_STAGE
#define XCH_HOOK_FIN
#include "fwd_split_tile.inc"
#undef XCH_HOOK_STAGE
#undef XCH_HOOK_FIN
}
#endif
#ifdef ILSX_KERNEL_IMPL
__global__ __launch_bounds__(64) void k_policy_finish(const PolicyFinishArgs P) {
  const int gr = blockIdx.x * 64 + threadIdx.x;
  if (gr >= P.rows) return;
  const int a = P.a, NO = 2 * a;
  float lp_quad = 0.f, lp_ls = 0.f, lp_jac = 0.f;
  const uint64_t step = P.scal ? P.scal->step : P.step_host;
  for (int j0 = 0; j0 < a; j0 += 4) {
    float z4[4] = {0.f, 0.f, 0.f, 0.f};
    if (P.head == HEAD_TANH_SAMPLE && !P.eps) philox_normal4(P.seed, step, P.rng_stream, gr, j0 >> 2, z4);
    for (int jj = 0; jj < 4 && j0 + jj < a; ++jj) {
      const int j = j0 + jj;
      float mu = 0.f, lsr = 0.f;
      for (int c = 0; c < P.cs; ++c) {
        mu += P.part[((size_t)c * P.part_stride + gr) * NO + j];
        lsr += P.part[((size_t)c * P.part_stride + gr) * NO + a + j];
      }
      if (P.raw) { P.raw[(size_t)gr * NO + j] = mu; P.raw[(size_t)gr * NO + a + j] = lsr; }
      const float ls = fminf(fmaxf(lsr, LOG_SIG_MIN), LOG_SIG_MAX);
      const float sd = expf(ls);
      float e = 0.f, z, act;
      if (P.head == HEAD_TANH_DET) {
        z = mu; act = tanhf(mu);
      } else if (P.head == HEAD_TANH_LOGP_OF_ACT) {
        act = P.act_in[(size_t)gr * a + j];
        z = 0.5f * (logf(1.0f + act + TANH_EPS) - logf(1.0f - act + TANH_EPS));
      } else {
        e = P.eps ? P.eps[(size_t)gr * a + j] : z4[jj];
        z = e * sd + mu;
        act = tanhf(z);
      }
      const float dm = mu - z;
      lp_quad += dm * dm / expf(2.0f * ls);
      lp_ls += ls;
      lp_jac += logf(1.0f - act * act + TANH_EPS);
      if (P.action) P.action[(size_t)gr * a + j] = act;
      if (P.eps_save) P.eps_save[(size_t)gr * a + j] = e;
    }
  }
  if (P.logp) P.logp[gr] = -0.5f * lp_quad - (lp_ls + HALF_LOG_2PI) - lp_jac;
}

template <int H, int ACT, int CS, int GRP, int MT = 1>
__global__ __launch_bounds__(4 * H / CS, (MT > 1 ? ILSX_MT_WAVES : GRP == 3 ? ILSX_LATE_WAVES : 1)) void k_mlp2_bwd_split(const BwdArgs A) {
  extern __shared__ __attribute__((aligned(16))) float smem[];
  static_assert(MT == 1 || GRP, "macro tiles are a grouped-launch shape");
  int sw_bx = 0, sw_task = 0, sw_cs = 0;
  if constexpr (GRP && MT > 1) {
    if (!grp_swizzle(A.swz, CS, blockIdx.x, &sw_bx, &sw_task, &sw_cs)) return;
  }
  const int ty = (GRP && MT > 1) ? sw_task : (int)blockIdx.y;
  BwdTask Tg;
  if (GRP == 1) Tg = A.tasks[ty];
  const BwdTask& T = GRP >= 2 ? g_bwd_tab[A.ctab - 1 + ty] : GRP == 1 ? Tg : A.t[ty];
  constexpr bool XCH = false;
  const int bx = (GRP && MT > 1) ? sw_bx : (int)blockIdx.x, cs = (GRP && MT > 1) ? sw_cs : (int)blockIdx.z;
#define XCH_HOOK_ACT
#define XCH_HOOK_HEAD
#include "bwd_split_tile.inc"
#undef XCH_HOOK_ACT
#undef XCH_HOOK_HEAD
}
#endif

#define PHASE_MAX_TILES 64
#define PHASE_TAIL_FLAG (3 * PHASE_MAX_TILES)
#define PHASE_NFLAGS (3 * PHASE_MAX_TILES + 1)
#define PHASE_MASK_WORD(t) ((PHASE_NFLAGS + (t)) * 32)
#define PHASE_FLAG_WORDS ((PHASE_NFLAGS + PHASE_MAX_TILES) * 32)
struct PhaseAArgs {
  FwdArgs f1, f2; BwdArgs b1; unsigned* flags; int* err; unsigned long long* dbg;
  PolicyFinishArgs fin_pi; int fin_pi_on, pad;
};
struct PhaseCArgs {
  FwdArgs f3; BwdArgs b2, b3; unsigned* flags; int* err; unsigned long long* dbg;
  float* polyak_T; const float* polyak_P; int polyak_n; float polyak_tau;
  float* aslot; const float* aslot_logp; int aslot_B; float aslot_te, aslot_invB;
};

static_assert(sizeof(PhaseAArgs) <= 4096 && sizeof(PhaseCArgs) <= 4096, "phase-kernel descriptors travel in the kernel-argument segment (4 KB)");
#define PHASE_CONST_SLOTS 64
#ifdef ILSX_KERNEL_IMPL
__constant__ PhaseAArgs g_phase_a_tab[PHASE_CONST_SLOTS];
__constant__ PhaseCArgs g_phase_c_tab[PHASE_CONST_SLOTS];
#endif

#ifdef ILSX_KERNEL_IMPL
__device__ __forceinline__ void xch_arrive(unsigned* flag) {
  asm volatile("s_waitcnt vmcnt(0)" ::: "memory");
  __syncthreads();
  if (threadIdx.x == 0) __hip_atomic_fetch_add(flag, 1u, __ATOMIC_RELAXED, __HIP_MEMORY_SCOPE_AGENT);
}
#define PHASE_FLAG_DEAD 0x40000000u
__device__ __forceinline__ void xch_wait(const unsigned* flag, unsigned target, int* err) {
  if (threadIdx.x == 0) {
    int spins = 0;
    while (__hip_atomic_load(flag, __ATOMIC_RELAXED, __HIP_MEMORY_SCOPE_AGENT) < target) {
      __builtin_amdgcn_s_sleep(2);
      if (++spins > (1 << 16)) { __hip_atomic_store(err, 1, __ATOMIC_RELAXED, __HIP_MEMORY_SCOPE_AGENT); break; }
    }
  }
  __syncthreads();
  asm volatile("buffer_inv sc0" ::: "memory");
}
__device__ __forceinline__ unsigned xcc_id() {
  unsigned v;
  asm volatile("s_getreg_b32 %0, hwreg(HW_REG_XCC_ID)" : "=s"(v));
  return v & 15u;
}
__device__ __forceinline__ void xch_mark_xcd(unsigned* mask) {
  if (threadIdx.x == 0) __hip_atomic_fetch_or(mask, 1u << xcc_id(), __ATOMIC_RELAXED, __HIP_MEMORY_SCOPE_AGENT);
}

__device__ __forceinline__ void policy_fin_tile(const PolicyFinishArgs& P, int r0, int rows, float* lp3, int nth) {
  const int a = P.a, NOp = 2 * a, tid = threadIdx.x;
  const unsigned long long fstep = P.scal ? (P.use_gather_step ? P.scal->gather_step : P.scal->step) : P.step_host;
  for (int e = tid; e < 16 * a; e += nth) {
    const int row = e / a, j = e - row * a, gr = r0 + row;
    float c0 = 0.0f, c1 = 0.0f, c2 = 0.0f;
    if (gr < rows) {
      float pm[4], pl[4];
#pragma unroll
      for (int c = 0; c < 4; ++c) {
        const size_t at = ((size_t)(c < P.cs ? c : 0) * P.part_stride + gr) * NOp + j;
        pm[c] = P.part[at];
        pl[c] = P.part[at + a];
      }
      float mu = 0.f, lsr = 0.f;
#pragma unroll
      for (int c = 0; c < 4; ++c) { mu += c < P.cs ? pm[c] : 0.0f; lsr += c < P.cs ? pl[c] : 0.0f; }
      float ep;
      if (P.eps) {
        ep = P.eps[(size_t)gr * a + j];
      } else {
        float z4[4];
        philox_normal4(P.seed, fstep, P.rng_stream, gr, j >> 2, z4);
        const int q = j & 3;
        ep = q == 0 ? z4[0] : q == 1 ? z4[1] : q == 2 ? z4[2] : z4[3];
      }
      const float ls = fminf(fmaxf(lsr, LOG_SIG_MIN), LOG_SIG_MAX);
      const float sd = expf(ls);
      const float z = ep * sd + mu;
      const float act = tanhf(z);
      const float dm = mu - z;
      c0 = dm * dm / expf(2.0f * ls); c1 = ls; c2 = logf(1.0f - act * act + TANH_EPS);
      if (P.raw) { P.raw[(size_t)gr * NOp + j] = mu; P.raw[(size_t)gr * NOp + a + j] = lsr; }
      if (P.action) P.action[(size_t)gr * a + j] = act;
      if (P.eps_save) P.eps_save[(size_t)gr * a + j] = ep;
    }
    lp3[(row * 32 + j) * 3 + 0] = c0; lp3[(row * 32 + j) * 3 + 1] = c1; lp3[(row * 32 + j) * 3 + 2] = c2;
  }
  lds_barrier();
  if (P.logp && tid < 16 && r0 + tid < rows) {
    float q = 0.f, l = 0.f, jc = 0.f;
    for (int j = 0; j < a; ++j) { q += lp3[(tid * 32 + j) * 3]; l += lp3[(tid * 32 + j) * 3 + 1]; jc += lp3[(tid * 32 + j) * 3 + 2]; }
    P.logp[r0 + tid] = -0.5f * q - (l + HALF_LOG_2PI) - jc;
  }
  lds_barrier();
}

template <int H, int ACT, int CS, bool CT = false>
__global__ __launch_bounds__(4 * H / CS) void k_sac_phase_a(const PhaseAArgs Pk, int slot) {
  const PhaseAArgs& P = CT ? g_phase_a_tab[slot] : Pk;
  constexpr int GRP = 0; constexpr bool XCH = true;
  constexpr int PH = 0, MT = 1;
  extern __shared__ __attribute__((aligned(16))) float smem[];
  const FwdGroup* GP = nullptr;
  const int bx = blockIdx.x, cs = blockIdx.z, y = blockIdx.y;
  unsigned* tflag = P.flags + PHASE_TAIL_FLAG * 32;
  if (y == 4) {
    if (bx == 0 && cs == 0) {
      const TailLite& TL = P.f1.tail[0];
      tail_lite_run(TL, smem);
      if (threadIdx.x == 0) {
        __hip_atomic_store(&TL.scal->alpha, TL.scal->alpha, __ATOMIC_RELAXED, __HIP_MEMORY_SCOPE_AGENT);
        asm volatile("s_waitcnt vmcnt(0)" ::: "memory");
        __hip_atomic_store(tflag, 1u, __ATOMIC_RELAXED, __HIP_MEMORY_SCOPE_AGENT);
      }
    }
    return;
  }
  if (bx * 16 >= P.f1.rows) return;
  unsigned* f1 = P.flags + (3 * bx) * 32;
  unsigned* f2 = P.flags + (3 * bx + 1) * 32;
  ILSX_STAMP(P.dbg, 0);
#if defined(ILSX_STAMPS) && defined(ILSX_STAMPS_FINE)
  if (P.dbg && threadIdx.x == 0 && (y == 1 || y == 2)) P.dbg[(size_t)ILSX_WG_LINEAR * ILSX_TRACE_SLOTS + 5] = clock64();
#endif
  xch_mark_xcd(P.flags + PHASE_MASK_WORD(bx));
  {
    const FwdArgs& A = P.f1;
    const FwdTask& T = A.t[y];
    const bool first_task = y == 0;
#define XCH_HOOK_STAGE
#define XCH_HOOK_FIN
#include "fwd_split_tile.inc"
#undef XCH_HOOK_STAGE
#undef XCH_HOOK_FIN
  }
  ILSX_STAMP(P.dbg, 1);
  unsigned* f0 = P.flags + (3 * bx + 2) * 32;
  if (y == 0) {
    asm volatile("s_waitcnt vmcnt(0)" ::: "memory");
    __syncthreads();
    if (threadIdx.x == 0) {
      __hip_atomic_fetch_add(f0, 1u, __ATOMIC_RELAXED, __HIP_MEMORY_SCOPE_AGENT);
      __hip_atomic_fetch_add(f1, 1u, __ATOMIC_RELAXED, __HIP_MEMORY_SCOPE_AGENT);
    }
  } else {
    xch_arrive(f1);
  }
  ILSX_STAMP(P.dbg, 2);
  if (y == 0 || y == 3) {
    {
      const FwdArgs& A = P.f2;
      const FwdTask& T = A.t[y == 0 ? 0 : 1];
      const bool first_task = y == 0;
#define XCH_HOOK_STAGE ILSX_STAMP_SYNC(P.dbg, 7); xch_wait(f0, CS, P.err); ILSX_STAMP(P.dbg, 3);
#define XCH_HOOK_FIN
#define XCH_FINE_DBG P.dbg
#include "fwd_split_tile.inc"
#undef XCH_FINE_DBG
#undef XCH_HOOK_STAGE
#undef XCH_HOOK_FIN
    }
    ILSX_STAMP(P.dbg, 4);
    xch_arrive(f2);
    ILSX_STAMP(P.dbg, 5);
  } else {
    xch_wait(f1, 4 * CS, P.err);
    if (P.fin_pi_on && y == 1 && cs == 0) {
      xch_wait(tflag, 1u, P.err);
      policy_fin_tile(P.fin_pi, bx * 16, P.f1.rows, smem, 4 * H / CS);
    }
    {
      const BwdArgs& A = P.b1;
      const BwdTask& T = A.t[y - 1];
#define XCH_HOOK_ACT
#define XCH_HOOK_HEAD xch_wait(f2, 2 * CS, P.err); xch_wait(tflag, 1u, P.err); ILSX_STAMP(P.dbg, 3);
#include "bwd_split_tile.inc"
#undef XCH_HOOK_ACT
#undef XCH_HOOK_HEAD
    }
    ILSX_STAMP(P.dbg, 4);
#if defined(ILSX_STAMPS) && defined(ILSX_STAMPS_FINE)
    if (P.dbg && threadIdx.x == 0) P.dbg[(size_t)ILSX_WG_LINEAR * ILSX_TRACE_SLOTS + 6] = clock64();
#endif
  }
}

template <int H, int ACT, int CS, bool CT = false>
__global__ __launch_bounds__(4 * H / CS) void k_sac_phase_c(const PhaseCArgs Pk, int slot) {
  const PhaseCArgs& P = CT ? g_phase_c_tab[slot] : Pk;
  constexpr int GRP = 0; constexpr bool XCH = true;
  constexpr int PH = 0, MT = 1;
  extern __shared__ __attribute__((aligned(16))) float smem[];
  const FwdGroup* GP = nullptr;
  const int bx = blockIdx.x, cs = blockIdx.z, y = blockIdx.y;
  if (y == 3) {
    if (bx == 0 && cs == 0 && threadIdx.x == 0) P.f3.tail[0].scal->gather_step += 1;
    if (P.aslot && bx == 1 && cs == 0) alpha_slot_run(P.aslot_logp, P.aslot_B, P.aslot_te, P.aslot_invB, P.aslot, smem);
    const float tau = P.polyak_tau;
    for (int i = ((int)(cs * gridDim.x + bx) * (int)blockDim.x + (int)threadIdx.x) * 4; i < P.polyak_n; i += (int)(gridDim.x * gridDim.z * blockDim.x) * 4) {
      const float4 p = *reinterpret_cast<const float4*>(P.polyak_P + i);
      float4 t = *reinterpret_cast<const float4*>(P.polyak_T + i);
      t.x = t.x * (1.0f - tau) + p.x * tau; t.y = t.y * (1.0f - tau) + p.y * tau;
      t.z = t.z * (1.0f - tau) + p.z * tau; t.w = t.w * (1.0f - tau) + p.w * tau;
      *reinterpret_cast<float4*>(P.polyak_T + i) = t;
    }
    return;
  }
  if (bx * 16 >= P.f3.rows) return;
  unsigned* f1 = P.flags + (3 * bx) * 32;
  unsigned* f2 = P.flags + (3 * bx + 1) * 32;
  ILSX_STAMP(P.dbg, 0);
  xch_mark_xcd(P.flags + PHASE_MASK_WORD(bx));
  if (y == 2) {
    {
      const BwdArgs& A = P.b3;
      const BwdTask& T = A.t[0];
#define XCH_HOOK_ACT
#define XCH_HOOK_HEAD xch_wait(f2, 2 * CS, P.err); ILSX_STAMP(P.dbg, 4);
#include "bwd_split_tile.inc"
#undef XCH_HOOK_ACT
#undef XCH_HOOK_HEAD
    }
    ILSX_STAMP(P.dbg, 5);
    return;
  }
  {
    const FwdArgs& A = P.f3;
    const FwdTask& T = A.t[y];
    const bool first_task = y == 0;
#define XCH_HOOK_STAGE
#define XCH_HOOK_FIN
#include "fwd_split_tile.inc"
#undef XCH_HOOK_STAGE
#undef XCH_HOOK_FIN
  }
  ILSX_STAMP(P.dbg, 1);
  xch_arrive(f1);
  {
    const BwdArgs& A = P.b2;
    const BwdTask& T = A.t[y];
#define XCH_HOOK_ACT xch_wait(f1, 2 * CS, P.err); ILSX_STAMP(P.dbg, 2);
#define XCH_HOOK_HEAD
#include "bwd_split_tile.inc"
#undef XCH_HOOK_ACT
#undef XCH_HOOK_HEAD
  }
  ILSX_STAMP(P.dbg, 3);
  xch_arrive(f2);
}
#endif

enum { DW_OUT_NATURAL = 0, DW_OUT_PACK_F = 1, DW_OUT_PACK_FB = 2 };
struct DwMat {
  const float* A; const float* Bm; float* dW; float* dWb; float* db;
  int lda, NA, ldb, NB, ldw, mode;
  int rows, bias_rows;
  int tile0, ktiles;
  int agent;
};
#define DW_MAX_MATS 10
struct AdamFuse {
  const float* Gbase; float* P; float* M; float* V; float* T;
  float b1, b2, eps, tau;
  const float* step_size; const float* bc2_sqrt;
  int on;
  float l2x2;
};
struct DwArgs {
  DwMat m[DW_MAX_MATS];
  int nmat, rows_all, ntiles, pad;
  AdamFuse F;
  unsigned long long* dbg;
  int xs;
  int splits, rows_per_split;
  float* g_lo; float* g_hi;
  float* scratch; size_t span;
  const struct DwTileG* gtiles;
  unsigned* zero_flags;
  const int* zero_err;
  int tile_nh, tile_kt;
  int strip;
};
struct DwTileG { DwMat J; AdamFuse F; };
#define DW_SPLIT_MIN_ROWS 1024
#define DW_BIG_MIN_ROWS 4096
#define DW_TILE_N 32
#define DW_TILE_K 64

#ifdef ILSX_KERNEL_IMPL
#define ILSX_ST(ptr, val) (*(ptr) = (val))
typedef float __attribute__((address_space(1))) ilsx_gfloat;
#ifdef ILSX_FLAT_TABLE_PTRS
#define ILSX_G(G) false
#else
#define ILSX_G(G) (G)
#endif
template <bool G>
__device__ __forceinline__ float ld_f(const float* p) {
  if (ILSX_G(G)) return *(const ilsx_gfloat*)p;
  return *p;
}
template <bool G>
__device__ __forceinline__ void st_f(float* p, float v) {
  if (ILSX_G(G)) *(ilsx_gfloat*)p = v;
  else ILSX_ST(p, v);
}
struct AdamOperands { float p, m, v, t; };
template <bool G = false>
__device__ __forceinline__ AdamOperands adam_prefetch(const AdamFuse& F, size_t i0) {
  AdamOperands o;
  o.p = ld_f<G>(F.P + i0); o.m = ld_f<G>(F.M + i0); o.v = ld_f<G>(F.V + i0); o.t = F.T ? ld_f<G>(F.T + i0) : 0.0f;
  return o;
}
template <bool G = false>
__device__ __forceinline__ void adam_apply(const AdamFuse& F, float step, float bc2s, const AdamOperands& o, size_t i0,
                                           size_t i1, bool two, float g) {
  g = g + F.l2x2 * o.p;
  const float m = o.m * F.b1 + (1.0f - F.b1) * g;
  const float v = o.v * F.b2 + (1.0f - F.b2) * g * g;
  const float p = o.p - step * (m / (sqrtf(v) / bc2s + F.eps));
  st_f<G>(F.M + i0, m); st_f<G>(F.V + i0, v); st_f<G>(F.P + i0, p);
  float tg = 0.0f;
  if (F.T) { tg = o.t * (1.0f - F.tau) + p * F.tau; st_f<G>(F.T + i0, tg); }
  if (two) {
    st_f<G>(F.M + i1, m); st_f<G>(F.V + i1, v); st_f<G>(F.P + i1, p);
    if (F.T) st_f<G>(F.T + i1, tg);
  }
}

#define DW_LDS_BYTES_OF(NH, KT) ((8 * (NH) * 4 * (KT) * 64 + 8 * (NH) * 16) * 4)
template <bool GRP, int NH, int KT, bool LOW>
__device__ __forceinline__ void dw_tile_body(const DwArgs& D, float* smem) {
  constexpr int NW = 8 * NH, NT = 512 * NH, TN = 16 * NH, TK = 16 * KT, EPT = (KT + 1) / 2;
  float* part = smem;
  float* bpart = smem + NW * 4 * KT * 64;
  if (blockIdx.x & ((1u << D.xs) - 1u)) return;
  const int bx = blockIdx.x >> D.xs;
  if (D.zero_flags && bx == 0 && blockIdx.y == 0 && threadIdx.x < PHASE_NFLAGS)
    D.zero_flags[threadIdx.x * 32] = (D.zero_err && *D.zero_err) ? PHASE_FLAG_DEAD : 0u;
  int mi = 0;
  if (!GRP) {
#pragma unroll
    for (int i = 1; i < DW_MAX_MATS; ++i)
      if (i < D.nmat && bx >= D.m[i].tile0) mi = i;
  }
  DwTileG Rg;
  if (GRP) {
    Rg = D.gtiles[bx];
  } else { Rg.J = D.m[mi]; Rg.F = D.F; }
  const DwMat& J = Rg.J;
  const AdamFuse& F = Rg.F;
  const int local = bx - J.tile0;
  const int n0 = (local / J.ktiles) * TN, k0 = (local % J.ktiles) * TK;
  int rows = J.rows > 0 ? J.rows : D.rows_all, brows = J.rows > 0 ? J.bias_rows : D.rows_all;
  int r_begin = 0;
  float* out_shift = nullptr;
  if (D.splits > 1) {
    r_begin = blockIdx.y * D.rows_per_split;
    rows = min(rows, r_begin + D.rows_per_split);
    brows = rows;
    out_shift = D.scratch + (size_t)blockIdx.y * D.span;
  }
  const int tid = threadIdx.x, lane = tid & 63, wave = tid >> 6, li = lane & 15, g = lane >> 4;
  const int wn = wave % NH, wr = wave / NH;
  const int nsub = n0 + 16 * wn;
  const bool n_ok = nsub + li < J.NA;
  int ntk = (J.NB - k0 + 15) / 16;
  if (ntk > KT) ntk = KT;
  ILSX_STAMP(D.dbg, 0);
  const bool packed = J.mode != DW_OUT_NATURAL;
  float* g0p[EPT]; float* g1p[EPT]; bool live[EPT];
  AdamOperands ao[EPT];
  float ad_step = 0.f, ad_bc2s = 1.f;
  bool bias_thread = false;
  float* gbp = nullptr;
  AdamOperands aob;
#define DW_OUTPUT_ELEMS()                                                                                                          \
  {                                                                                                                                \
    if (F.on) { ad_step = ld_f<GRP>(F.step_size); ad_bc2s = ld_f<GRP>(F.bc2_sqrt); }                                                                   \
    _Pragma("unroll") for (int h = 0; h < EPT; ++h) {                                                                              \
      const int e = tid + NT * h, ee = e % (256 * NH * KT);                                                                        \
      const int on = ee / (256 * KT), rest = ee % (256 * KT), t = rest >> 8, q = rest & 255;                                       \
                                                                                                   \
      const int v = packed ? (q >> 2) & 3 : (q >> 6) & 3;                                                                          \
      const int ol = packed ? ((q >> 4) & 3) * 16 + 4 * (q >> 6) + (q & 3) : q & 63;                                               \
      const int n = n0 + 16 * on + 4 * (ol >> 4) + v, k = k0 + 16 * t + (ol & 15);                                                 \
      live[h] = e < 256 * NH * KT && t < ntk && n < J.NA && k < J.NB;                                                              \
      g0p[h] = nullptr; g1p[h] = nullptr;                                                                                          \
      if (live[h]) {                                                                                                               \
        g0p[h] = J.mode == DW_OUT_NATURAL ? J.dW + (size_t)n * J.ldw + k : J.dW + pack_f(n, k, J.ldw);                             \
        g1p[h] = J.mode == DW_OUT_PACK_FB ? J.dWb + pack_b(n, k, J.NA) : nullptr;                                                  \
        if (out_shift) {                                                                                                           \
          g0p[h] = out_shift + (g0p[h] - D.g_lo);                                                                                  \
          if (g1p[h]) g1p[h] = out_shift + (g1p[h] - D.g_lo);                                                                      \
        }                                                                                                                          \
        if (F.on) ao[h] = adam_prefetch<GRP>(F, (size_t)(g0p[h] - F.Gbase));                                                            \
      }                                                                                                                            \
    }                                                                                                                              \
    bias_thread = J.db && k0 == 0 && tid < 16 * NH && n0 + 16 * (tid >> 4) + (tid & 15) < J.NA;                                    \
    gbp = bias_thread ? J.db + n0 + 16 * (tid >> 4) + (tid & 15) : nullptr;                                                        \
    if (gbp && out_shift) gbp = out_shift + (gbp - D.g_lo);                                                                        \
// ... 544 lines not shown
```

include/ilsx.h:

```cpp
#ifndef ILSX_H
#define ILSX_H
#include <stddef.h>
#include <stdint.h>

#ifdef __cplusplus
extern "C" {
#endif

#define ILSX_ABI_VERSION 1

typedef enum {
  ILSX_OK = 0,
  ILSX_ERR_ARG = -1,
  ILSX_ERR_HIP = -2,
  ILSX_ERR_NOMEM = -3,
  ILSX_ERR_STATE = -4,
  ILSX_ERR_UNSUPPORTED = -5
} ilsx_status;

typedef struct ilsx_ctx ilsx_ctx;
typedef struct ilsx_net ilsx_net;
typedef struct ilsx_replay ilsx_replay;
typedef struct ilsx_sac ilsx_sac;
typedef struct ilsx_sac_group ilsx_sac_group;
typedef struct ilsx_vecenv ilsx_vecenv;
typedef struct ilsx_disc ilsx_disc;
typedef struct ilsx_ppo ilsx_ppo;
typedef struct ilsx_td3 ilsx_td3;
typedef struct ilsx_sacv ilsx_sacv;
typedef struct ilsx_bc ilsx_bc;
typedef struct ilsx_dsac ilsx_dsac;

enum { ILSX_ACT_RELU = 0, ILSX_ACT_TANH = 1 };

int ilsx_abi_version(void);
const char* ilsx_last_error(void);
int ilsx_ctx_create(int hip_device, void* hip_stream, uint64_t seed, ilsx_ctx** out);
int ilsx_ctx_sync(ilsx_ctx* ctx);
int ilsx_ctx_destroy(ilsx_ctx* ctx);
void* ilsx_ctx_stream(ilsx_ctx* ctx);
int ilsx_ctx_rng_stream_cursor(ilsx_ctx* ctx, uint32_t set_to, uint32_t* current);
int ilsx_ctx_alloc(ilsx_ctx* ctx, size_t bytes, void** out);
int ilsx_ctx_free(ilsx_ctx* ctx, void* ptr);
int ilsx_memcpy_h2d(ilsx_ctx* ctx, void* dst_dev, const void* src_host, size_t bytes);
int ilsx_memcpy_d2h(ilsx_ctx* ctx, void* dst_host, const void* src_dev, size_t bytes);

#define ILSX_COMM_ID_BYTES 128
int ilsx_comm_unique_id(uint8_t* id_host );
int ilsx_comm_init(ilsx_ctx* ctx, const uint8_t* id_host, int n_ranks, int rank);
int ilsx_comm_destroy(ilsx_ctx* ctx);
int ilsx_comm_info(const ilsx_ctx* ctx, int* n_ranks, int* rank);
int ilsx_comm_allreduce_sum(ilsx_ctx* ctx, float* dev_buf, size_t n);

enum { ILSX_K_MLP_FWD = 0, ILSX_K_MLP_BWD_DX = 1, ILSX_K_MLP_BWD_DW = 2, ILSX_K_ADAM = 3,
       ILSX_K_REPLAY_SAMPLE = 4, ILSX_K_REPLAY_ADD = 5, ILSX_K_REPLAY_SAMPLE_MANY = 6, ILSX_K_SAC_STATS = 7,
       ILSX_K_SAC_FINISH = 8, ILSX_K_ENV_STEP = 9, ILSX_K_POLICY_FINISH = 10, ILSX_K_DISC_BWD = 11, ILSX_K_PPO_GAE = 12,
       ILSX_K_SAC_PHASE_A = 13, ILSX_K_SAC_PHASE_C = 14,
       ILSX_K_COUNT = 16 };
int ilsx_prof_enable(ilsx_ctx* ctx, int on);
int ilsx_prof_reset(ilsx_ctx* ctx);
int ilsx_prof_read(ilsx_ctx* ctx, int kernel_id, uint64_t* launches, double* total_ms);
const char* ilsx_prof_kernel(ilsx_ctx* ctx, int kernel_id);
const char* ilsx_kernel_name(int kernel_id);
int ilsx_debug_set_stamp_buffer(ilsx_ctx* ctx, void* dev_trace, int max_launches, int* launches_so_far);
int ilsx_debug_dw_split(int rows, int big, int* splits, int* rows_per_split);

typedef struct {
  int32_t in_dim;
  int32_t n_hidden;
  int32_t hidden;
  int32_t out_dim;
  int32_t n_heads;
  int32_t act;
  int32_t hidden_sizes[3];
} ilsx_mlp_cfg;

int ilsx_net_create(ilsx_ctx* ctx, const ilsx_mlp_cfg* cfg, ilsx_net** out);
int ilsx_net_destroy(ilsx_net* net);
int ilsx_net_num_params(const ilsx_net* net, size_t* out);
int ilsx_net_init(ilsx_net* net, uint64_t seed, float init_w, float b_init);
int ilsx_net_set_params(ilsx_net* net, const float* src, size_t n, int src_is_device);
int ilsx_net_get_params(const ilsx_net* net, float* dst, size_t n, int dst_is_device);
int ilsx_mlp_forward(ilsx_net* net, const float* x, int rows, float* y);
int ilsx_policy_act(ilsx_net* pi, const float* obs, int n, int deterministic, const float* eps,
                    float* act, float* logp);
int ilsx_policy_log_prob(ilsx_net* pi, const float* obs, const float* act, int n, float* logp);
int ilsx_net_set_noise_policy(ilsx_net* pi, float policy_noise, float policy_noise_clip, float max_act);
int ilsx_net_set_output_linear(ilsx_net* pi, int linear);
int ilsx_net_set_categorical(ilsx_net* pi, int on);
int ilsx_policy_log_pis(ilsx_net* pi, const float* obs, int n_rows, float* log_pis);

int ilsx_replay_create(ilsx_ctx* ctx, int64_t capacity, int obs_dim, int act_dim, uint64_t seed,
                       ilsx_replay** out);
int ilsx_replay_destroy(ilsx_replay* rb);
int ilsx_replay_add(ilsx_replay* rb, const float* obs, const float* act, const float* rew,
                    const uint8_t* done, const float* nobs, int n, const uint8_t* ep_end_host,
                    int data_is_device);
int ilsx_replay_terminate_episode(ilsx_replay* rb);
int ilsx_replay_set_absorbing(ilsx_replay* rb, int64_t slot0, int n, const float* absorbing_host);
int ilsx_replay_get_absorbing(ilsx_replay* rb, const int64_t* idx, int n, float* absorbing);
int ilsx_replay_sample(ilsx_replay* rb, int B, const int64_t* idx, float* obs, float* act, float* rew,
                       float* done, float* nobs, int64_t* idx_out);
int ilsx_replay_sample_many(ilsx_replay* rb, int n_batches, int B, float* out_records);
int ilsx_replay_record_floats(const ilsx_replay* rb, int* out);
int ilsx_her_gather(ilsx_replay* rb, const int64_t* idx, const int64_t* idx_relabel, int B, int n_relabel, int relabel_on, int d_obs,
                    int d_goal, int reward_kind, float threshold, float* obs_cat, float* act, float* rew, float* done, float* nobs_cat);
int ilsx_replay_size(ilsx_replay* rb, int64_t* size, int64_t* top);
int ilsx_replay_clear(ilsx_replay* rb);
int ilsx_replay_traj_endpoints(ilsx_replay* rb, int64_t* starts_host, int64_t* ends_host, int max, int* n);

typedef struct {
  float reward_scale, discount, policy_lr, qf_lr, alpha_lr, soft_target_tau, alpha;
  int32_t train_alpha;
  float policy_mean_reg_weight, policy_std_reg_weight, beta_1;
  int32_t has_target_entropy;
  float target_entropy;
  int32_t max_batch;
  int32_t grad_world;
} ilsx_sac_cfg;

typedef struct {
  float qf1_loss, qf2_loss, policy_loss, alpha_loss, alpha;
  float q1_mean, q2_mean, log_pi_mean, policy_mu_mean, policy_log_std_mean;
  double log_alpha;
  float ext_std[5], ext_max[5], ext_min[5];
} ilsx_sac_stats;

int ilsx_sac_create(ilsx_ctx* ctx, const ilsx_sac_cfg* cfg, ilsx_net* pi, ilsx_net* q1, ilsx_net* q2,
                    ilsx_sac** out);
int ilsx_sac_destroy(ilsx_sac* sac);
int ilsx_sac_train_step(ilsx_sac* sac, const float* obs, const float* act, const float* rew,
                        const float* done, const float* nobs, int B, const float* eps_next,
                        const float* eps_cur, ilsx_sac_stats* stats);
int ilsx_sac_train_from_replay(ilsx_sac* sac, ilsx_replay* rb, int n_steps, int B, ilsx_sac_stats* stats);
int ilsx_sac_phase_state(ilsx_sac* sac, int* fallbacks, int* disabled, int* last_window_on_phase, int* wgs_per_cu_a, int* wgs_per_cu_c);
int ilsx_sac_debug_break_phase(ilsx_sac* sac);
int ilsx_sac_set_batch(ilsx_sac* sac, const float* obs, const float* act, const float* rew,
                       const float* done, const float* nobs, int B, const float* eps_next,
                       const float* eps_cur);
int ilsx_sac_critic_backward(ilsx_sac* sac);
int ilsx_sac_critic_update(ilsx_sac* sac);
int ilsx_sac_actor_backward(ilsx_sac* sac);
int ilsx_sac_actor_update(ilsx_sac* sac);
int ilsx_sac_last_stats(ilsx_sac* sac, ilsx_sac_stats* stats);
int ilsx_sac_get_params(ilsx_sac* sac, int which, float* dst, size_t n, int dst_is_device);
int ilsx_sac_set_params(ilsx_sac* sac, int which, const float* src, size_t n, int src_is_device);
int ilsx_sac_get_grads(ilsx_sac* sac, int which, float* dst, size_t n, int dst_is_device);
int ilsx_sac_grads_ptr(ilsx_sac* sac, int segment, float** dev_ptr, size_t* n);
int ilsx_sac_get_log_alpha(ilsx_sac* sac, double* out);
int ilsx_sac_set_log_alpha(ilsx_sac* sac, double v);
int ilsx_sac_get_adam(ilsx_sac* sac, int which, float* m_host, float* v_host, size_t n, int64_t* t);
int ilsx_sac_set_adam(ilsx_sac* sac, int which, const float* m_host, const float* v_host, size_t n, int64_t t);
int ilsx_sac_get_alpha_opt(ilsx_sac* sac, double* m, double* v, int64_t* t, uint64_t* rng_step);
int ilsx_sac_set_alpha_opt(ilsx_sac* sac, double m, double v, int64_t t, uint64_t rng_step);

int ilsx_sac_debug_batch(ilsx_sac* sac, ilsx_replay* rb, uint64_t step, int B, float* obs, float* act, float* rew,
                         float* done, float* nobs, float* eps_next, float* eps_cur, int64_t* idx);
int ilsx_sac_debug_last_batch(ilsx_sac* sac, int B, float* obs, float* act, float* rew, float* done, float* nobs,
                              float* eps_cur);
int ilsx_debug_rng_stream(const void* object, int kind, uint32_t* stream, uint64_t* seed);
int ilsx_debug_philox(ilsx_ctx* ctx, uint64_t seed, uint64_t step, uint32_t stream, int n_rows, int a, uint32_t* raw, float* normals);

enum { ILSX_DISC_AIRL = 0, ILSX_DISC_GAIL = 1, ILSX_DISC_GAIL2 = 2, ILSX_DISC_FAIRL = 3 };
typedef struct {
  int32_t obs_dim, act_dim;
  int32_t hid_dim, hid_act;
  int32_t use_grad_pen;
  float clamp_magnitude, disc_lr, disc_momentum, grad_pen_weight;
  int32_t max_batch;
  int32_t state_only;
  int32_t num_layer_blocks;
  int32_t use_bn;
  int32_t grad_world;
} ilsx_disc_cfg;
typedef struct { float ce_loss, grad_pen, accuracy; } ilsx_disc_stats;
int ilsx_disc_create(ilsx_ctx* ctx, const ilsx_disc_cfg* cfg, ilsx_disc** out);
int ilsx_disc_destroy(ilsx_disc* disc);
int ilsx_disc_num_params(const ilsx_disc* disc, size_t* out);
int ilsx_disc_set_params(ilsx_disc* disc, const float* src_host, size_t n);
int ilsx_disc_get_params(ilsx_disc* disc, float* dst_host, size_t n);
int ilsx_disc_get_grads(ilsx_disc* disc, float* dst_host, size_t n);
int ilsx_disc_get_bn_stats(ilsx_disc* disc, float* running_mean_host, float* running_var_host, size_t n);
int ilsx_disc_set_bn_stats(ilsx_disc* disc, const float* running_mean_host, const float* running_var_host, size_t n);
int ilsx_disc_train_step(ilsx_disc* disc, const float* exp_obs, const float* exp_act, const float* pol_obs,
                         const float* pol_act, int B, const float* eps, ilsx_disc_stats* stats);
int ilsx_disc_reward(ilsx_disc* disc, const float* obs, const float* act, int n, int mode, int has_min, float rew_clip_min,
                     int has_max, float rew_clip_max, float* rew, float* logits);

int ilsx_sac_group_create(ilsx_ctx* ctx, ilsx_sac* const* agents, int n_agents, ilsx_sac_group** out);
int ilsx_sac_group_destroy(ilsx_sac_group* group);
int ilsx_sac_group_train_from_replay(ilsx_sac_group* group, ilsx_replay* const* rbs, int n_steps, int B, int want_stats);

int ilsx_advirl_train(ilsx_disc* disc, ilsx_sac* policy_trainer, ilsx_replay* expert_rb, ilsx_replay* policy_rb, int loops,
                      int disc_updates, int policy_updates, int disc_batch, int policy_batch, int mode, int has_min,
                      float rew_clip_min, int has_max, float rew_clip_max, ilsx_disc_stats* disc_stats,
                      ilsx_sac_stats* sac_stats, float* rew_stats4);
int ilsx_advirl_set_policy_batch_from_expert(ilsx_disc* disc, int n_from_expert);

typedef struct {
  float reward_scale, discount, policy_lr, qf_lr;
  int32_t policy_and_target_update_period;
  float soft_target_tau, policy_noise, policy_noise_clip, max_act;
  int32_t max_batch;
  int32_t her;
  float clip_return_l, clip_return_r;
} ilsx_td3_cfg;
typedef struct {
  float qf1_loss, qf2_loss, policy_loss;
  float q1_pred[4], q2_pred[4], q_target[4], bellman1[4], bellman2[4], policy_action[4];
} ilsx_td3_stats;
int ilsx_td3_create(ilsx_ctx* ctx, const ilsx_td3_cfg* cfg, ilsx_net* pi, ilsx_net* qf1, ilsx_net* qf2, ilsx_td3** out);
int ilsx_td3_destroy(ilsx_td3* td3);
int ilsx_td3_train_step(ilsx_td3* td3, const float* obs, const float* act, const float* rew, const float* done,
                        const float* nobs, int B, const float* eps_target, ilsx_td3_stats* stats);
int ilsx_td3_train_from_replay(ilsx_td3* td3, ilsx_replay* rb, int n_steps, int B, ilsx_td3_stats* stats);
int ilsx_td3_get_params(ilsx_td3* td3, int which, float* dst_host, size_t n);
int ilsx_td3_set_params(ilsx_td3* td3, int which, const float* src_host, size_t n);

typedef struct {
  float discount, reward_scale, alpha, soft_target_tau, policy_lr, qf_lr, beta_1;
  int32_t max_batch;
} ilsx_dsac_cfg;
typedef struct {
  float qf1_loss, qf2_loss, policy_loss;
  float q1_pred[4], q2_pred[4];
} ilsx_dsac_stats;
int ilsx_dsac_create(ilsx_ctx* ctx, const ilsx_dsac_cfg* cfg, ilsx_net* pi, ilsx_net* qf1, ilsx_net* qf2, ilsx_dsac** out);
int ilsx_dsac_destroy(ilsx_dsac* d);
int ilsx_dsac_train_step(ilsx_dsac* d, const float* obs, const float* act, const float* rew, const float* done, const float* nobs, int B,
                         ilsx_dsac_stats* stats);
int ilsx_dsac_train_from_replay(ilsx_dsac* d, ilsx_replay* rb, int n_steps, int B, ilsx_dsac_stats* stats);
int ilsx_dsac_get_params(ilsx_dsac* d, int which, float* dst_host, size_t n);
int ilsx_dsac_set_params(ilsx_dsac* d, int which, const float* src_host, size_t n);

typedef struct {
  float reward_scale, discount, alpha, policy_lr, qf_lr, vf_lr, soft_target_tau;
  float policy_mean_reg_weight, policy_std_reg_weight, beta_1;
  int32_t max_batch;
} ilsx_sacv_cfg;
typedef struct {
  float qf1_loss, qf2_loss, vf_loss, policy_loss;
  float q1_pred[4], q2_pred[4], v_pred[4], log_pi[4], policy_mu[4], policy_log_std[4];
} ilsx_sacv_stats;
int ilsx_sacv_create(ilsx_ctx* ctx, const ilsx_sacv_cfg* cfg, ilsx_net* pi, ilsx_net* qf1, ilsx_net* qf2, ilsx_net* vf,
                     ilsx_sacv** out);
int ilsx_sacv_destroy(ilsx_sacv* sac);
int ilsx_sacv_train_step(ilsx_sacv* sac, const float* obs, const float* act, const float* rew, const float* done,
                         const float* nobs, int B, const float* eps, ilsx_sacv_stats* stats);
int ilsx_sacv_train_from_replay(ilsx_sacv* sac, ilsx_replay* rb, int n_steps, int B, ilsx_sacv_stats* stats);
int ilsx_sacv_get_params(ilsx_sacv* sac, int which, float* dst_host, size_t n);
int ilsx_sacv_set_params(ilsx_sacv* sac, int which, const float* src_host, size_t n);

typedef struct { int64_t t; uint64_t rng_step; int64_t n_train_steps; } ilsx_opt_meta;
int ilsx_td3_get_opt(ilsx_td3* td3, int which, float* m_host, float* v_host, size_t n, ilsx_opt_meta* meta);
int ilsx_td3_set_opt(ilsx_td3* td3, int which, const float* m_host, const float* v_host, size_t n, const ilsx_opt_meta* meta);
int ilsx_dsac_get_opt(ilsx_dsac* d, int which, float* m_host, float* v_host, size_t n, ilsx_opt_meta* meta);
int ilsx_dsac_set_opt(ilsx_dsac* d, int which, const float* m_host, const float* v_host, size_t n, const ilsx_opt_meta* meta);
int ilsx_sacv_get_opt(ilsx_sacv* sac, int which, float* m_host, float* v_host, size_t n, ilsx_opt_meta* meta);
int ilsx_sacv_set_opt(ilsx_sacv* sac, int which, const float* m_host, const float* v_host, size_t n, const ilsx_opt_meta* meta);
int ilsx_bc_get_opt(ilsx_bc* bc, float* m_host, float* v_host, size_t n, ilsx_opt_meta* meta);
int ilsx_bc_set_opt(ilsx_bc* bc, const float* m_host, const float* v_host, size_t n, const ilsx_opt_meta* meta);
int ilsx_ppo_get_opt(ilsx_ppo* ppo, int which, float* m_host, float* v_host, size_t n, ilsx_opt_meta* meta);
int ilsx_ppo_set_opt(ilsx_ppo* ppo, int which, const float* m_host, const float* v_host, size_t n, const ilsx_opt_meta* meta);
int ilsx_disc_get_opt(ilsx_disc* disc, float* m_host, float* v_host, size_t n, ilsx_opt_meta* meta);
int ilsx_disc_set_opt(ilsx_disc* disc, const float* m_host, const float* v_host, size_t n, const ilsx_opt_meta* meta);

enum { ILSX_BC_MLE = 0, ILSX_BC_MSE = 1 };
typedef struct { int32_t mode; float lr, momentum; int32_t max_batch; } ilsx_bc_cfg;
int ilsx_bc_create(ilsx_ctx* ctx, const ilsx_bc_cfg* cfg, ilsx_net* pi, ilsx_bc** out);
int ilsx_bc_destroy(ilsx_bc* bc);
int ilsx_bc_train_step(ilsx_bc* bc, const float* obs, const float* act, int B, const float* eps, float* stat);
int ilsx_bc_train_from_replay(ilsx_bc* bc, ilsx_replay* expert_rb, int n_updates, int B, float* stat);

typedef struct {
  int32_t obs_dim, act_dim, n_hidden, hidden;
  float reward_scale, discount, clip_eps, policy_lr, value_lr, gae_tau, value_l2_reg;
  int32_t mini_batch_size, update_epoch;
  int32_t max_samples;
  int32_t use_value_clip;
  int32_t conditioned_std;
  int32_t hidden_sizes[3];
  int32_t grad_world;
} ilsx_ppo_cfg;
int ilsx_ppo_create(ilsx_ctx* ctx, const ilsx_ppo_cfg* cfg, ilsx_ppo** out);
int ilsx_ppo_destroy(ilsx_ppo* ppo);
int ilsx_ppo_num_params(const ilsx_ppo* ppo, int which, size_t* out);
int ilsx_ppo_set_params(ilsx_ppo* ppo, int which, const float* src_host, size_t n);
int ilsx_ppo_get_params(ilsx_ppo* ppo, int which, float* dst_host, size_t n);
// ... 177 lines not shown
```

Measured before the change: 17270.

## Add loader waves that stage next-layer weights into LDS for SAC phase kernels

Doubles the phase kernels' block size with extra loader waves that prefetch the next layer's weight slices from global memory and publish them to LDS. The publishes are matched to the compute waves' barriers, so compute waves read weights from LDS instead of loading them into registers up front. The goal is to hide weight-load latency and free registers in the compute waves. In exchange it costs more LDS and threads per block, relies on a hand-counted barrier schedule that is fragile, and is used only when occupancy allows (env ILSX_PHASE_LOADER, on by default).

```diff
diff --git a/ilswiss_amd/_lib.py b/ilswiss_amd/_lib.py
--- a/ilswiss_amd/_lib.py
+++ b/ilswiss_amd/_lib.py
@@ -328,6 +328,7 @@
     "ilsx_sac_debug_last_batch": (C.c_int, [vp, C.c_int, vp, vp, vp, vp, vp, vp]),
     "ilsx_sac_phase_state": (C.c_int, [vp, C.POINTER(C.c_int), C.POINTER(C.c_int), C.POINTER(C.c_int), C.POINTER(C.c_int), C.POINTER(C.c_int)]),
     "ilsx_sac_debug_break_phase": (C.c_int, [vp]),
+    "ilsx_phase_launch_shape": (C.c_int, [C.c_int, C.c_int, C.c_int, C.POINTER(C.c_int), C.POINTER(C.c_int)]),
     "ilsx_sac_set_alpha_opt": (C.c_int, [vp, C.c_double, C.c_double, C.c_int64, C.c_uint64]),
     "ilsx_bnn_create": (C.c_int, [vp, C.POINTER(BnnCfg), C.POINTER(vp)]),
     "ilsx_bnn_destroy": (C.c_int, [vp]),
diff --git a/ilswiss_amd/csrc/bwd_split_tile.inc b/ilswiss_amd/csrc/bwd_split_tile.inc
--- a/ilswiss_amd/csrc/bwd_split_tile.inc
+++ b/ilswiss_amd/csrc/bwd_split_tile.inc
@@ -1,3 +1,8 @@
+#ifndef XCH_LDR
+#define XCH_LDR false
+#define XCH_WSLICE (static_cast<const float4*>(nullptr))
+#define XCH_LDR_DEFAULTED
+#endif
   constexpr int NTH = 4 * H / CS, NWV = NTH / 64, NC = H / 16, SLW = H / CS, RPW = 16 / NWV, KPL = SLW / 64;
   constexpr int RPT = 16 * H / NTH, RSTEP = NTH / H;
   constexpr int LDH = H + ILSX_LDS_PAD, LDSL = SLW + ILSX_LDS_PAD;
@@ -40,7 +45,7 @@
         w0b[t][s4] = c < T.dx_cols ? W0[pack_f(cs * SLW + 16 * wave + 4 * g + s4, T.dx_col0 + c, ld0)] : 0.0f;
       }
   }
-  if constexpr (XCH) {
+  if constexpr (XCH && !(XCH_LDR)) {
     {
       const float* wp = N.base + N.off_Wb[1] + (size_t)(cs * NWV + wave) * NC * 256 + 4 * lane;
 #pragma unroll
@@ -149,6 +154,11 @@
   }
   lds_barrier();
   ILSX_STAMP(A.dbg, 2);
+  if constexpr (XCH_LDR) {
+    const float4* wl = XCH_WSLICE + wave * NC * 64 + lane;
+#pragma unroll
+    for (int c = 0; c < NC; ++c) wreg[c] = wl[64 * c];
+  }
   {
     f32x4 acc0[MT], acc1[MT];
 #pragma unroll
@@ -220,3 +230,8 @@
     }
   }
   ILSX_STAMP(A.dbg, 7);
+#ifdef XCH_LDR_DEFAULTED
+#undef XCH_LDR
+#undef XCH_WSLICE
+#undef XCH_LDR_DEFAULTED
+#endif
diff --git a/ilswiss_amd/csrc/fwd_split_tile.inc b/ilswiss_amd/csrc/fwd_split_tile.inc
--- a/ilswiss_amd/csrc/fwd_split_tile.inc
+++ b/ilswiss_amd/csrc/fwd_split_tile.inc
@@ -1,3 +1,8 @@
+#ifndef XCH_LDR
+#define XCH_LDR false
+#define XCH_WSLICE (static_cast<const float4*>(nullptr))
+#define XCH_LDR_DEFAULTED
+#endif
   constexpr int NTH = 4 * H / CS, NWV = NTH / 64, NC = H / 16, SLW = H / CS, NCS = SLW / 16;
   constexpr int NT0 = PH == 1 ? 1 : CS;
   constexpr int LDH = H + ILSX_LDS_PAD, LDSL = SLW + ILSX_LDS_PAD;
@@ -51,7 +56,7 @@
       whf[t] = (t < NOT && j < NO) ? *reinterpret_cast<const float4*>(N.base + N.off_Wh + (size_t)j * H + cs * SLW + 16 * wave + 4 * g)
                                    : make_float4(0.f, 0.f, 0.f, 0.f);
     }
-    if constexpr (!LATEW) {
+    if constexpr (!LATEW && !(XCH_LDR)) {
       const float* wp = N.base + N.off_W[1] + (size_t)(cs * NWV + wave) * NC * 256 + 4 * lane;
 #pragma unroll
       for (int c = 0; c < NC; ++c) wreg[c] = *reinterpret_cast<const float4*>(wp + 256 * c);
@@ -373,6 +378,11 @@
 #pragma unroll
     for (int c = 0; c < NC; ++c) wreg[c] = *reinterpret_cast<const float4*>(wp + 256 * c);
   }
+  if constexpr (XCH_LDR) {
+    const float4* wl = XCH_WSLICE + wave * NC * 64 + lane;
+#pragma unroll
+    for (int c = 0; c < NC; ++c) wreg[c] = wl[64 * c];
+  }
   {
     f32x4 acc0[MT], acc1[MT];
 #pragma unroll
@@ -441,3 +451,8 @@
   lds_barrier();
   }
   ILSX_STAMP(A.dbg, 7);
+#ifdef XCH_LDR_DEFAULTED
+#undef XCH_LDR
+#undef XCH_WSLICE
+#undef XCH_LDR_DEFAULTED
+#endif
diff --git a/ilswiss_amd/csrc/ilsx_core.hip b/ilswiss_amd/csrc/ilsx_core.hip
--- a/ilswiss_amd/csrc/ilsx_core.hip
+++ b/ilswiss_amd/csrc/ilsx_core.hip
@@ -349,12 +349,14 @@
   HIPCHK(hipFuncSetAttribute((const void*)k_mlp2_bwd_split<256, AA, 4, true, MM>, hipFuncAttributeMaxDynamicSharedMemorySize, cap))
   SET_MT(ACT_RELU, 2); SET_MT(ACT_RELU, 4); SET_MT(ACT_TANH, 2); SET_MT(ACT_TANH, 4);
 #undef SET_MT
-#define SET_PHASE(HH, AA, CC) HIPCHK(hipFuncSetAttribute((const void*)k_sac_phase_a<HH, AA, CC>, hipFuncAttributeMaxDynamicSharedMemorySize, cap)); \
-  HIPCHK(hipFuncSetAttribute((const void*)k_sac_phase_a<HH, AA, CC, true>, hipFuncAttributeMaxDynamicSharedMemorySize, cap)); \
-  HIPCHK(hipFuncSetAttribute((const void*)k_sac_phase_c<HH, AA, CC, true>, hipFuncAttributeMaxDynamicSharedMemorySize, cap)); \
-  HIPCHK(hipFuncSetAttribute((const void*)k_sac_phase_c<HH, AA, CC>, hipFuncAttributeMaxDynamicSharedMemorySize, cap))
+#define SET_PHASE_K(KA, KC, HH, AA, CC) HIPCHK(hipFuncSetAttribute((const void*)KA<HH, AA, CC, false>, hipFuncAttributeMaxDynamicSharedMemorySize, cap)); \
+  HIPCHK(hipFuncSetAttribute((const void*)KA<HH, AA, CC, true>, hipFuncAttributeMaxDynamicSharedMemorySize, cap)); \
+  HIPCHK(hipFuncSetAttribute((const void*)KC<HH, AA, CC, true>, hipFuncAttributeMaxDynamicSharedMemorySize, cap)); \
+  HIPCHK(hipFuncSetAttribute((const void*)KC<HH, AA, CC, false>, hipFuncAttributeMaxDynamicSharedMemorySize, cap))
+#define SET_PHASE(HH, AA, CC) SET_PHASE_K(k_sac_phase_a, k_sac_phase_c, HH, AA, CC); SET_PHASE_K(k_sac_phase_a_ld, k_sac_phase_c_ld, HH, AA, CC)
   SET_PHASE(256, ACT_RELU, 4); SET_PHASE(256, ACT_TANH, 4); SET_PHASE(128, ACT_RELU, 2); SET_PHASE(128, ACT_TANH, 2);
 #undef SET_PHASE
+#undef SET_PHASE_K
   done = true;
   return ILSX_OK;
 }
@@ -514,30 +516,59 @@
   }
   return n_cu;
 }
-static size_t phase_lds_bytes(int H, int KP, int cs) { return std::max(fwd_split_lds_bytes(H, KP, cs), bwd_split_lds_bytes(H, cs)); }
-void phase_wgs_per_cu(int H, int cs, int* occ_a, int* occ_c) {
-  static int oa[2] = {-1, -1}, oc[2] = {-1, -1};
+static bool phase_loader_on() { const char* e = getenv("ILSX_PHASE_LOADER"); return !(e && atoi(e) == 0); }
+static unsigned phase_block_threads(int H, int cs, bool ld) { return (ld ? 8 : 4) * H / cs; }
+static size_t phase_lds_bytes(int H, int KP, int cs, bool ld) {
+  return std::max(fwd_split_lds_bytes(H, KP, cs), bwd_split_lds_bytes(H, cs)) + (ld ? sizeof(float) * PHASE_WSLICE_FLOATS(H, cs) : 0);
+}
+extern "C" int ilsx_phase_launch_shape(int H, int KP, int loader, int* threads, int* lds_bytes) {
+  const int cs = H == 256 ? 4 : H == 128 ? 2 : 0;
+  if (!cs || KP < 16 || (KP & 15)) ILSX_FAIL(ILSX_ERR_ARG, "ilsx_phase_launch_shape: no phase kernel for H=%d KP=%d", H, KP);
+  if (threads) *threads = (int)phase_block_threads(H, cs, loader != 0);
+  if (lds_bytes) *lds_bytes = (int)phase_lds_bytes(H, KP, cs, loader != 0);
+  return ILSX_OK;
+}
+static void phase_occ(int H, int cs, bool ld, int* occ_a, int* occ_c) {
+  static int oa[2][2] = {{-1, -1}, {-1, -1}}, oc[2][2] = {{-1, -1}, {-1, -1}};
   const int i = H == 256 ? 0 : 1;
-  if (oa[i] < 0) {
+  if (oa[i][ld] < 0) {
     int a = 0, c = 0;
-    const size_t lds = phase_lds_bytes(H, 32, cs);
+    const size_t lds = phase_lds_bytes(H, 32, cs, ld);
+    const int nth = (int)phase_block_threads(H, cs, ld);
     hipError_t e1, e2;
-    if (H == 256) { e1 = hipOccupancyMaxActiveBlocksPerMultiprocessor(&a, (const void*)k_sac_phase_a<256, ACT_RELU, 4>, 4 * H / cs, lds);
-                    e2 = hipOccupancyMaxActiveBlocksPerMultiprocessor(&c, (const void*)k_sac_phase_c<256, ACT_RELU, 4>, 4 * H / cs, lds); }
-    else { e1 = hipOccupancyMaxActiveBlocksPerMultiprocessor(&a, (const void*)k_sac_phase_a<128, ACT_RELU, 2>, 4 * H / cs, lds);
-           e2 = hipOccupancyMaxActiveBlocksPerMultiprocessor(&c, (const void*)k_sac_phase_c<128, ACT_RELU, 2>, 4 * H / cs, lds); }
-    oa[i] = e1 == hipSuccess ? std::max(a, 1) : 1;
-    oc[i] = e2 == hipSuccess ? std::max(c, 1) : 1;
-  }
-  *occ_a = oa[i]; *occ_c = oc[i];
+#define PHASE_OCC(KA, KC, HH, CC) do { e1 = hipOccupancyMaxActiveBlocksPerMultiprocessor(&a, (const void*)KA<HH, ACT_RELU, CC, false>, nth, lds); \
+                                       e2 = hipOccupancyMaxActiveBlocksPerMultiprocessor(&c, (const void*)KC<HH, ACT_RELU, CC, false>, nth, lds); } while (0)
+    if (H == 256) { if (ld) PHASE_OCC(k_sac_phase_a_ld, k_sac_phase_c_ld, 256, 4); else PHASE_OCC(k_sac_phase_a, k_sac_phase_c, 256, 4); }
+    else { if (ld) PHASE_OCC(k_sac_phase_a_ld, k_sac_phase_c_ld, 128, 2); else PHASE_OCC(k_sac_phase_a, k_sac_phase_c, 128, 2); }
+#undef PHASE_OCC
+    oa[i][ld] = e1 == hipSuccess ? std::max(a, 1) : 1;
+    oc[i][ld] = e2 == hipSuccess ? std::max(c, 1) : 1;
+  }
+  *occ_a = oa[i][ld]; *occ_c = oc[i][ld];
+}
+static bool phase_a_resident(ilsx_ctx* ctx, int rows, int H, int cs, bool ld) {
+  int oa = 1, oc = 1;
+  phase_occ(H, cs, ld, &oa, &oc);
+  return ((rows + 15) / 16) * 4 * cs + 1 <= oa * device_cus(ctx);
+}
+static bool phase_c_resident(ilsx_ctx* ctx, int rows, int H, int cs, bool ld) {
+  int oa = 1, oc = 1;
+  phase_occ(H, cs, ld, &oa, &oc);
+  return ((rows + 15) / 16) * 3 * cs <= oc * device_cus(ctx);
+}
+static bool phase_a_loader(ilsx_ctx* ctx, int rows, int H, int cs) { return phase_loader_on() && phase_a_resident(ctx, rows, H, cs, true); }
+static bool phase_c_loader(ilsx_ctx* ctx, int rows, int H, int cs) { return phase_loader_on() && phase_c_resident(ctx, rows, H, cs, true); }
+void phase_wgs_per_cu(ilsx_ctx* ctx, int rows, int H, int cs, int* occ_a, int* occ_c) {
+  int x = 0;
+  phase_occ(H, cs, phase_a_loader(ctx, rows, H, cs), occ_a, &x);
+  phase_occ(H, cs, phase_c_loader(ctx, rows, H, cs), &x, occ_c);
 }
 bool phase_fits(ilsx_ctx* ctx, int rows, int H, int cs, int ntasks) {
   const int n_cu = device_cus(ctx);
   if (!((H == 256 && cs == 4) || (H == 128 && cs == 2))) return false;
   const int tiles = (rows + 15) / 16, work = tiles * ntasks * cs;
-  int occ_a = 1, occ_c = 1;
-  phase_wgs_per_cu(H, cs, &occ_a, &occ_c);
-  return tiles <= PHASE_MAX_TILES && work <= n_cu && work + 1 <= occ_a * n_cu && tiles * 3 * cs <= occ_c * n_cu;
+  return tiles <= PHASE_MAX_TILES && work <= n_cu && phase_a_resident(ctx, rows, H, cs, phase_a_loader(ctx, rows, H, cs)) &&
+         phase_c_resident(ctx, rows, H, cs, phase_c_loader(ctx, rows, H, cs));
 }
 
 static std::vector<bool> g_phase_slots[16];
@@ -587,17 +618,22 @@
   P.dbg = upload_only ? nullptr : ctx->dbg_next();
   if (P.b1.ga_parts < 1) P.b1.ga_parts = 1;
   const int tiles = (P.f1.rows + 15) / 16;
-  dim3 grid((tiles + 7) & ~7, 5, cs), block(4 * H / cs);
-  const size_t lds = phase_lds_bytes(H, KPmax, cs);
+  const bool ld = phase_a_loader(ctx, P.f1.rows, H, cs);
+  dim3 grid((tiles + 7) & ~7, 5, cs), block(phase_block_threads(H, cs, ld));
+  const size_t lds = phase_lds_bytes(H, KPmax, cs, ld);
+  if (lds > 160 * 1024) ILSX_FAIL(ILSX_ERR_UNSUPPORTED, "phase kernel needs %zu B of LDS (> 160 KiB)", lds);
   const bool use_ct = ct && phase_const_ready(ctx, ct, P, key, ct->a, ct->valid_a, ct->key_a, HIP_SYMBOL(g_phase_a_tab));
   if (upload_only) return ILSX_OK;
   const int slot = use_ct ? ct->slot : 0;
   static const bool trace = getenv("ILSX_PHASE_CT_TRACE") != nullptr;
   if (trace) { hipStreamCaptureStatus cap = hipStreamCaptureStatusNone; hipStreamIsCapturing(ctx->stream, &cap);
-               fprintf(stderr, "launch_phase_a: %s, slot %d, capturing %d\n", use_ct ? "constant table" : "kernel arguments", ct ? ct->slot : -9, (int)cap); }
+               fprintf(stderr, "launch_phase_a: %s, slot %d, capturing %d, weights %s\n", use_ct ? "constant table" : "kernel arguments", ct ? ct->slot : -9, (int)cap,
+                       ld ? "loader waves" : "registers"); }
   ProfScope ps(ctx, ILSX_K_SAC_PHASE_A);
-#define PHASE_A(HH, AA, CC) do { if (use_ct) ILSX_LAUNCH(ps, (k_sac_phase_a<HH, AA, CC, true>), grid, block, lds, ctx->stream, P, slot); \
-                                 else ILSX_LAUNCH(ps, (k_sac_phase_a<HH, AA, CC>), grid, block, lds, ctx->stream, P, slot); } while (0)
+#define PHASE_A(HH, AA, CC) do { if (use_ct && ld) ILSX_LAUNCH(ps, (k_sac_phase_a_ld<HH, AA, CC, true>), grid, block, lds, ctx->stream, P, slot); \
+                                 else if (use_ct) ILSX_LAUNCH(ps, (k_sac_phase_a<HH, AA, CC, true>), grid, block, lds, ctx->stream, P, slot); \
+                                 else if (ld) ILSX_LAUNCH(ps, (k_sac_phase_a_ld<HH, AA, CC, false>), grid, block, lds, ctx->stream, P, slot); \
+                                 else ILSX_LAUNCH(ps, (k_sac_phase_a<HH, AA, CC, false>), grid, block, lds, ctx->stream, P, slot); } while (0)
   if (H == 256 && act == ILSX_ACT_RELU) PHASE_A(256, ACT_RELU, 4);
   else if (H == 256) PHASE_A(256, ACT_TANH, 4);
   else if (act == ILSX_ACT_RELU) PHASE_A(128, ACT_RELU, 2);
@@ -615,14 +651,20 @@
   if (P.b2.ga_parts < 1) P.b2.ga_parts = 1;
   if (P.b3.ga_parts < 1) P.b3.ga_parts = 1;
   const int tiles = (P.f3.rows + 15) / 16;
-  dim3 grid((tiles + 7) & ~7, 4, cs), block(4 * H / cs);
-  const size_t lds = phase_lds_bytes(H, KPmax, cs);
+  const bool ld = phase_c_loader(ctx, P.f3.rows, H, cs);
+  dim3 grid((tiles + 7) & ~7, 4, cs), block(phase_block_threads(H, cs, ld));
+  const size_t lds = phase_lds_bytes(H, KPmax, cs, ld);
+  if (lds > 160 * 1024) ILSX_FAIL(ILSX_ERR_UNSUPPORTED, "phase kernel needs %zu B of LDS (> 160 KiB)", lds);
   const bool use_ct = ct && phase_const_ready(ctx, ct, P, key, ct->c, ct->valid_c, ct->key_c, HIP_SYMBOL(g_phase_c_tab));
   if (upload_only) return ILSX_OK;
   const int slot = use_ct ? ct->slot : 0;
+  static const bool trace = getenv("ILSX_PHASE_CT_TRACE") != nullptr;
+  if (trace) fprintf(stderr, "launch_phase_c: %s, slot %d, weights %s\n", use_ct ? "constant table" : "kernel arguments", ct ? ct->slot : -9, ld ? "loader waves" : "registers");
   ProfScope ps(ctx, ILSX_K_SAC_PHASE_C);
-#define PHASE_C(HH, AA, CC) do { if (use_ct) ILSX_LAUNCH(ps, (k_sac_phase_c<HH, AA, CC, true>), grid, block, lds, ctx->stream, P, slot); \
-                                 else ILSX_LAUNCH(ps, (k_sac_phase_c<HH, AA, CC>), grid, block, lds, ctx->stream, P, slot); } while (0)
+#define PHASE_C(HH, AA, CC) do { if (use_ct && ld) ILSX_LAUNCH(ps, (k_sac_phase_c_ld<HH, AA, CC, true>), grid, block, lds, ctx->stream, P, slot); \
+                                 else if (use_ct) ILSX_LAUNCH(ps, (k_sac_phase_c<HH, AA, CC, true>), grid, block, lds, ctx->stream, P, slot); \
+                                 else if (ld) ILSX_LAUNCH(ps, (k_sac_phase_c_ld<HH, AA, CC, false>), grid, block, lds, ctx->stream, P, slot); \
+                                 else ILSX_LAUNCH(ps, (k_sac_phase_c<HH, AA, CC, false>), grid, block, lds, ctx->stream, P, slot); } while (0)
   if (H == 256 && act == ILSX_ACT_RELU) PHASE_C(256, ACT_RELU, 4);
   else if (H == 256) PHASE_C(256, ACT_TANH, 4);
   else if (act == ILSX_ACT_RELU) PHASE_C(128, ACT_RELU, 2);
diff --git a/ilswiss_amd/csrc/ilsx_sac.hip b/ilswiss_amd/csrc/ilsx_sac.hip
--- a/ilswiss_amd/csrc/ilsx_sac.hip
+++ b/ilswiss_amd/csrc/ilsx_sac.hip
@@ -989,14 +989,14 @@
   }
   return rc;
 }
-void phase_wgs_per_cu(int H, int cs, int* occ_a, int* occ_c);
+void phase_wgs_per_cu(ilsx_ctx* ctx, int rows, int H, int cs, int* occ_a, int* occ_c);
 extern "C" int ilsx_sac_phase_state(ilsx_sac* s, int* fallbacks, int* disabled, int* last_window_on_phase, int* wgs_per_cu_a, int* wgs_per_cu_c) {
   if (!s) ILSX_FAIL(ILSX_ERR_ARG, "ilsx_sac_phase_state: NULL agent");
   if (fallbacks) *fallbacks = s->phase_fallbacks;
   if (disabled) *disabled = s->phase_broken ? 1 : 0;
   if (last_window_on_phase) *last_window_on_phase = s->phase_last ? 1 : 0;
   int oa = 0, oc = 0;
-  if (s->cs > 1 && (s->Lq.cfg.hidden == 256 || s->Lq.cfg.hidden == 128)) phase_wgs_per_cu(s->Lq.cfg.hidden, s->cs, &oa, &oc);
+  if (s->cs > 1 && (s->Lq.cfg.hidden == 256 || s->Lq.cfg.hidden == 128)) phase_wgs_per_cu(s->ctx, s->cfg.max_batch, s->Lq.cfg.hidden, s->cs, &oa, &oc);
   if (wgs_per_cu_a) *wgs_per_cu_a = oa;
   if (wgs_per_cu_c) *wgs_per_cu_c = oc;
   return ILSX_OK;
diff --git a/ilswiss_amd/csrc/kernels.h b/ilswiss_amd/csrc/kernels.h
--- a/ilswiss_amd/csrc/kernels.h
+++ b/ilswiss_amd/csrc/kernels.h
@@ -973,6 +973,15 @@
   if (threadIdx.x == 0) __hip_atomic_fetch_or(mask, 1u << xcc_id(), __ATOMIC_RELAXED, __HIP_MEMORY_SCOPE_AGENT);
 }
 
+__device__ __forceinline__ void ldr_bar(int n = 1) {
+#pragma unroll
+  for (int i = 0; i < n; ++i) asm volatile("s_waitcnt lgkmcnt(0)\n\ts_barrier" ::: "memory");
+}
+#define LDR_REQUEST(w, slices, slice) do { const float* wp_ = (slices) + (size_t)(slice) * NCW * 256 + 4 * ln; \
+  _Pragma("unroll") for (int c = 0; c < NCW; ++c) (w)[c] = *reinterpret_cast<const f32x4*>(wp_ + 256 * c); } while (0)
+#define LDR_PUBLISH(wl, w) do { _Pragma("unroll") for (int c = 0; c < NCW; ++c) (wl)[(lw * NCW + c) * 64 + ln] = (w)[c]; } while (0)
+#define PHASE_WSLICE_FLOATS(H, CS) (4 * (H) / (CS) * ((H) / 16) * 4)
+
 __device__ __forceinline__ void policy_fin_tile(const PolicyFinishArgs& P, int r0, int rows, float* lp3, int nth) {
   const int a = P.a, NOp = 2 * a, tid = threadIdx.x;
   const unsigned long long fstep = P.scal ? (P.use_gather_step ? P.scal->gather_step : P.scal->step) : P.step_host;
@@ -1022,156 +1031,24 @@
 
 template <int H, int ACT, int CS, bool CT = false>
 __global__ __launch_bounds__(4 * H / CS) void k_sac_phase_a(const PhaseAArgs Pk, int slot) {
-  const PhaseAArgs& P = CT ? g_phase_a_tab[slot] : Pk;
-  constexpr int GRP = 0; constexpr bool XCH = true;
-  constexpr int PH = 0, MT = 1;
-  extern __shared__ __attribute__((aligned(16))) float smem[];
-  const FwdGroup* GP = nullptr;
-  const int bx = blockIdx.x, cs = blockIdx.z, y = blockIdx.y;
-  unsigned* tflag = P.flags + PHASE_TAIL_FLAG * 32;
-  if (y == 4) {
-    if (bx == 0 && cs == 0) {
-      const TailLite& TL = P.f1.tail[0];
-      tail_lite_run(TL, smem);
-      if (threadIdx.x == 0) {
-        __hip_atomic_store(&TL.scal->alpha, TL.scal->alpha, __ATOMIC_RELAXED, __HIP_MEMORY_SCOPE_AGENT);
-        asm volatile("s_waitcnt vmcnt(0)" ::: "memory");
-        __hip_atomic_store(tflag, 1u, __ATOMIC_RELAXED, __HIP_MEMORY_SCOPE_AGENT);
-      }
-    }
-    return;
-  }
-  if (bx * 16 >= P.f1.rows) return;
-  unsigned* f1 = P.flags + (3 * bx) * 32;
-  unsigned* f2 = P.flags + (3 * bx + 1) * 32;
-  ILSX_STAMP(P.dbg, 0);
-#if defined(ILSX_STAMPS) && defined(ILSX_STAMPS_FINE)
-  if (P.dbg && threadIdx.x == 0 && (y == 1 || y == 2)) P.dbg[(size_t)ILSX_WG_LINEAR * ILSX_TRACE_SLOTS + 5] = clock64();
-#endif
-  xch_mark_xcd(P.flags + PHASE_MASK_WORD(bx));
-  {
-    const FwdArgs& A = P.f1;
-    const FwdTask& T = A.t[y];
-    const bool first_task = y == 0;
-#define XCH_HOOK_STAGE
-#define XCH_HOOK_FIN
-#include "fwd_split_tile.inc"
-#undef XCH_HOOK_STAGE
-#undef XCH_HOOK_FIN
-  }
-  ILSX_STAMP(P.dbg, 1);
-  unsigned* f0 = P.flags + (3 * bx + 2) * 32;
-  if (y == 0) {
-    asm volatile("s_waitcnt vmcnt(0)" ::: "memory");
-    __syncthreads();
-    if (threadIdx.x == 0) {
-      __hip_atomic_fetch_add(f0, 1u, __ATOMIC_RELAXED, __HIP_MEMORY_SCOPE_AGENT);
-      __hip_atomic_fetch_add(f1, 1u, __ATOMIC_RELAXED, __HIP_MEMORY_SCOPE_AGENT);
-    }
-  } else {
-    xch_arrive(f1);
-  }
-  ILSX_STAMP(P.dbg, 2);
-  if (y == 0 || y == 3) {
-    {
-      const FwdArgs& A = P.f2;
-      const FwdTask& T = A.t[y == 0 ? 0 : 1];
-      const bool first_task = y == 0;
-#define XCH_HOOK_STAGE ILSX_STAMP_SYNC(P.dbg, 7); xch_wait(f0, CS, P.err); ILSX_STAMP(P.dbg, 3);
-#define XCH_HOOK_FIN
-#define XCH_FINE_DBG P.dbg
-#include "fwd_split_tile.inc"
-#undef XCH_FINE_DBG
-#undef XCH_HOOK_STAGE
-#undef XCH_HOOK_FIN
-    }
-    ILSX_STAMP(P.dbg, 4);
-    xch_arrive(f2);
-    ILSX_STAMP(P.dbg, 5);
-  } else {
-    xch_wait(f1, 4 * CS, P.err);
-    if (P.fin_pi_on && y == 1 && cs == 0) {
-      xch_wait(tflag, 1u, P.err);
-      policy_fin_tile(P.fin_pi, bx * 16, P.f1.rows, smem, 4 * H / CS);
-    }
-    {
-      const BwdArgs& A = P.b1;
-      const BwdTask& T = A.t[y - 1];
-#define XCH_HOOK_ACT
-#define XCH_HOOK_HEAD xch_wait(f2, 2 * CS, P.err); xch_wait(tflag, 1u, P.err); ILSX_STAMP(P.dbg, 3);
-#include "bwd_split_tile.inc"
-#undef XCH_HOOK_ACT
-#undef XCH_HOOK_HEAD
-    }
-    ILSX_STAMP(P.dbg, 4);
-#if defined(ILSX_STAMPS) && defined(ILSX_STAMPS_FINE)
-    if (P.dbg && threadIdx.x == 0) P.dbg[(size_t)ILSX_WG_LINEAR * ILSX_TRACE_SLOTS + 6] = clock64();
-#endif
-  }
+  constexpr bool LD = false;
+#include "sac_phase_a.inc"
+}
+template <int H, int ACT, int CS, bool CT = false>
+__global__ __launch_bounds__(8 * H / CS) void k_sac_phase_a_ld(const PhaseAArgs Pk, int slot) {
+  constexpr bool LD = true;
+#include "sac_phase_a.inc"
 }
 
 template <int H, int ACT, int CS, bool CT = false>
 __global__ __launch_bounds__(4 * H / CS) void k_sac_phase_c(const PhaseCArgs Pk, int slot) {
-  const PhaseCArgs& P = CT ? g_phase_c_tab[slot] : Pk;
-  constexpr int GRP = 0; constexpr bool XCH = true;
-  constexpr int PH = 0, MT = 1;
-  extern __shared__ __attribute__((aligned(16))) float smem[];
-  const FwdGroup* GP = nullptr;
-  const int bx = blockIdx.x, cs = blockIdx.z, y = blockIdx.y;
-  if (y == 3) {
-    if (bx == 0 && cs == 0 && threadIdx.x == 0) P.f3.tail[0].scal->gather_step += 1;
-    if (P.aslot && bx == 1 && cs == 0) alpha_slot_run(P.aslot_logp, P.aslot_B, P.aslot_te, P.aslot_invB, P.aslot, smem);
-    const float tau = P.polyak_tau;
-    for (int i = ((int)(cs * gridDim.x + bx) * (int)blockDim.x + (int)threadIdx.x) * 4; i < P.polyak_n; i += (int)(gridDim.x * gridDim.z * blockDim.x) * 4) {
-      const float4 p = *reinterpret_cast<const float4*>(P.polyak_P + i);
-      float4 t = *reinterpret_cast<const float4*>(P.polyak_T + i);
-      t.x = t.x * (1.0f - tau) + p.x * tau; t.y = t.y * (1.0f - tau) + p.y * tau;
-      t.z = t.z * (1.0f - tau) + p.z * tau; t.w = t.w * (1.0f - tau) + p.w * tau;
-      *reinterpret_cast<float4*>(P.polyak_T + i) = t;
-    }
-    return;
-  }
-  if (bx * 16 >= P.f3.rows) return;
-  unsigned* f1 = P.flags + (3 * bx) * 32;
-  unsigned* f2 = P.flags + (3 * bx + 1) * 32;
-  ILSX_STAMP(P.dbg, 0);
-  xch_mark_xcd(P.flags + PHASE_MASK_WORD(bx));
-  if (y == 2) {
-    {
-      const BwdArgs& A = P.b3;
-      const BwdTask& T = A.t[0];
-#define XCH_HOOK_ACT
-#define XCH_HOOK_HEAD xch_wait(f2, 2 * CS, P.err); ILSX_STAMP(P.dbg, 4);
-#include "bwd_split_tile.inc"
-#undef XCH_HOOK_ACT
-#undef XCH_HOOK_HEAD
-    }
-    ILSX_STAMP(P.dbg, 5);
-    return;
-  }
-  {
-    const FwdArgs& A = P.f3;
-    const FwdTask& T = A.t[y];
-    const bool first_task = y == 0;
-#define XCH_HOOK_STAGE
-#define XCH_HOOK_FIN
-#include "fwd_split_tile.inc"
-#undef XCH_HOOK_STAGE
-#undef XCH_HOOK_FIN
-  }
-  ILSX_STAMP(P.dbg, 1);
-  xch_arrive(f1);
-  {
-    const BwdArgs& A = P.b2;
-    const BwdTask& T = A.t[y];
-#define XCH_HOOK_ACT xch_wait(f1, 2 * CS, P.err); ILSX_STAMP(P.dbg, 2);
-#define XCH_HOOK_HEAD
-#include "bwd_split_tile.inc"
-#undef XCH_HOOK_ACT
-#undef XCH_HOOK_HEAD
-  }
-  ILSX_STAMP(P.dbg, 3);
-  xch_arrive(f2);
+  constexpr bool LD = false;
+#include "sac_phase_c.inc"
+}
+template <int H, int ACT, int CS, bool CT = false>
+__global__ __launch_bounds__(8 * H / CS) void k_sac_phase_c_ld(const PhaseCArgs Pk, int slot) {
+  constexpr bool LD = true;
+#include "sac_phase_c.inc"
 }
 #endif
 
diff --git a/ilswiss_amd/csrc/sac_phase_a.inc b/ilswiss_amd/csrc/sac_phase_a.inc
--- /dev/null
+++ b/ilswiss_amd/csrc/sac_phase_a.inc
@@ -0,0 +1,123 @@
+  const PhaseAArgs& P = CT ? g_phase_a_tab[slot] : Pk;
+  constexpr int GRP = 0; constexpr bool XCH = true;
+  constexpr int PH = 0, MT = 1;
+  extern __shared__ __attribute__((aligned(16))) float smem_all[];
+  float* const smem = smem_all + (LD ? PHASE_WSLICE_FLOATS(H, CS) : 0);
+  const FwdGroup* GP = nullptr;
+  const int bx = blockIdx.x, cs = blockIdx.z, y = blockIdx.y;
+  unsigned* tflag = P.flags + PHASE_TAIL_FLAG * 32;
+  if (y == 4) {
+    if (bx == 0 && cs == 0) {
+      const TailLite& TL = P.f1.tail[0];
+      tail_lite_run(TL, smem);
+      if (threadIdx.x == 0) {
+        __hip_atomic_store(&TL.scal->alpha, TL.scal->alpha, __ATOMIC_RELAXED, __HIP_MEMORY_SCOPE_AGENT);
+        asm volatile("s_waitcnt vmcnt(0)" ::: "memory");
+        __hip_atomic_store(tflag, 1u, __ATOMIC_RELAXED, __HIP_MEMORY_SCOPE_AGENT);
+      }
+    }
+    return;
+  }
+  if (bx * 16 >= P.f1.rows) return;
+  unsigned* f1 = P.flags + (3 * bx) * 32;
+  unsigned* f2 = P.flags + (3 * bx + 1) * 32;
+  ILSX_STAMP(P.dbg, 0);
+#if defined(ILSX_STAMPS) && defined(ILSX_STAMPS_FINE)
+  if (P.dbg && threadIdx.x == 0 && (y == 1 || y == 2)) P.dbg[(size_t)ILSX_WG_LINEAR * ILSX_TRACE_SLOTS + 5] = clock64();
+#endif
+  xch_mark_xcd(P.flags + PHASE_MASK_WORD(bx));
+  if constexpr (LD) {
+    constexpr int NWC = 4 * H / CS / 64, NCW = H / 16;
+    const int wv = __builtin_amdgcn_readfirstlane((int)(threadIdx.x >> 6));
+    if (wv >= NWC) {
+      const int lw = wv - NWC, ln = threadIdx.x & 63;
+      f32x4* const wl = reinterpret_cast<f32x4*>(smem_all);
+      f32x4 w[NCW];
+      const NetView& N1 = P.f1.t[y].net;
+      LDR_REQUEST(w, N1.base + N1.off_W[1], cs * NWC + lw);
+      ldr_bar();
+      LDR_PUBLISH(wl, w);
+      ldr_bar();
+      const bool walk_fwd = y == 0 || y == 3;
+      const NetView& N2 = walk_fwd ? P.f2.t[y == 0 ? 0 : 1].net : P.b1.t[y - 1].net;
+      LDR_REQUEST(w, N2.base + (walk_fwd ? N2.off_W[1] : N2.off_Wb[1]), cs * NWC + lw);
+      ldr_bar(3);
+      ldr_bar();
+      LDR_PUBLISH(wl, w);
+      if (walk_fwd) {
+        ldr_bar();
+        ldr_bar(5);
+        ldr_bar();
+      } else {
+        ldr_bar();
+        if (P.fin_pi_on && y == 1 && cs == 0) ldr_bar(3);
+        ldr_bar(2);
+        ldr_bar(2);
+        if (P.b1.t[y - 1].dx) ldr_bar(2);
+      }
+      return;
+    }
+  }
+#define XCH_LDR LD
+#define XCH_WSLICE (reinterpret_cast<const float4*>(smem_all))
+  {
+    const FwdArgs& A = P.f1;
+    const FwdTask& T = A.t[y];
+    const bool first_task = y == 0;
+#define XCH_HOOK_STAGE
+#define XCH_HOOK_FIN
+#include "fwd_split_tile.inc"
+#undef XCH_HOOK_STAGE
+#undef XCH_HOOK_FIN
+  }
+  ILSX_STAMP(P.dbg, 1);
+  unsigned* f0 = P.flags + (3 * bx + 2) * 32;
+  if (y == 0) {
+    asm volatile("s_waitcnt vmcnt(0)" ::: "memory");
+    __syncthreads();
+    if (threadIdx.x == 0) {
+      __hip_atomic_fetch_add(f0, 1u, __ATOMIC_RELAXED, __HIP_MEMORY_SCOPE_AGENT);
+      __hip_atomic_fetch_add(f1, 1u, __ATOMIC_RELAXED, __HIP_MEMORY_SCOPE_AGENT);
+    }
+  } else {
+    xch_arrive(f1);
+  }
+  ILSX_STAMP(P.dbg, 2);
+  if (y == 0 || y == 3) {
+    {
+      const FwdArgs& A = P.f2;
+      const FwdTask& T = A.t[y == 0 ? 0 : 1];
+      const bool first_task = y == 0;
+#define XCH_HOOK_STAGE ILSX_STAMP_SYNC(P.dbg, 7); xch_wait(f0, CS, P.err); ILSX_STAMP(P.dbg, 3);
+#define XCH_HOOK_FIN
+#define XCH_FINE_DBG P.dbg
+#include "fwd_split_tile.inc"
+#undef XCH_FINE_DBG
+#undef XCH_HOOK_STAGE
+#undef XCH_HOOK_FIN
+    }
+    ILSX_STAMP(P.dbg, 4);
+    xch_arrive(f2);
+    ILSX_STAMP(P.dbg, 5);
+  } else {
+    xch_wait(f1, 4 * CS, P.err);
+    if (P.fin_pi_on && y == 1 && cs == 0) {
+      xch_wait(tflag, 1u, P.err);
+      policy_fin_tile(P.fin_pi, bx * 16, P.f1.rows, smem, 4 * H / CS);
+    }
+    {
+      const BwdArgs& A = P.b1;
+      const BwdTask& T = A.t[y - 1];
+#define XCH_HOOK_ACT
+#define XCH_HOOK_HEAD xch_wait(f2, 2 * CS, P.err); xch_wait(tflag, 1u, P.err); ILSX_STAMP(P.dbg, 3);
+#include "bwd_split_tile.inc"
+#undef XCH_HOOK_ACT
+#undef XCH_HOOK_HEAD
+    }
+    ILSX_STAMP(P.dbg, 4);
+#if defined(ILSX_STAMPS) && defined(ILSX_STAMPS_FINE)
+    if (P.dbg && threadIdx.x == 0) P.dbg[(size_t)ILSX_WG_LINEAR * ILSX_TRACE_SLOTS + 6] = clock64();
+#endif
+  }
+#undef XCH_LDR
+#undef XCH_WSLICE
diff --git a/ilswiss_amd/csrc/sac_phase_c.inc b/ilswiss_amd/csrc/sac_phase_c.inc
--- /dev/null
+++ b/ilswiss_amd/csrc/sac_phase_c.inc
@@ -0,0 +1,98 @@
+  const PhaseCArgs& P = CT ? g_phase_c_tab[slot] : Pk;
+  constexpr int GRP = 0; constexpr bool XCH = true;
+  constexpr int PH = 0, MT = 1;
+  extern __shared__ __attribute__((aligned(16))) float smem_all[];
+  float* const smem = smem_all + (LD ? PHASE_WSLICE_FLOATS(H, CS) : 0);
+  const FwdGroup* GP = nullptr;
+  const int bx = blockIdx.x, cs = blockIdx.z, y = blockIdx.y;
+  if (y == 3) {
+    if (bx == 0 && cs == 0 && threadIdx.x == 0) P.f3.tail[0].scal->gather_step += 1;
+    if (P.aslot && bx == 1 && cs == 0) alpha_slot_run(P.aslot_logp, P.aslot_B, P.aslot_te, P.aslot_invB, P.aslot, smem);
+    const float tau = P.polyak_tau;
+    for (int i = ((int)(cs * gridDim.x + bx) * (int)blockDim.x + (int)threadIdx.x) * 4; i < P.polyak_n; i += (int)(gridDim.x * gridDim.z * blockDim.x) * 4) {
+      const float4 p = *reinterpret_cast<const float4*>(P.polyak_P + i);
+      float4 t = *reinterpret_cast<const float4*>(P.polyak_T + i);
+      t.x = t.x * (1.0f - tau) + p.x * tau; t.y = t.y * (1.0f - tau) + p.y * tau;
+      t.z = t.z * (1.0f - tau) + p.z * tau; t.w = t.w * (1.0f - tau) + p.w * tau;
+      *reinterpret_cast<float4*>(P.polyak_T + i) = t;
+    }
+    return;
+  }
+  if (bx * 16 >= P.f3.rows) return;
+  unsigned* f1 = P.flags + (3 * bx) * 32;
+  unsigned* f2 = P.flags + (3 * bx + 1) * 32;
+  ILSX_STAMP(P.dbg, 0);
+  xch_mark_xcd(P.flags + PHASE_MASK_WORD(bx));
+  if constexpr (LD) {
+    constexpr int NWC = 4 * H / CS / 64, NCW = H / 16;
+    const int wv = __builtin_amdgcn_readfirstlane((int)(threadIdx.x >> 6));
+    if (wv >= NWC) {
+      const int lw = wv - NWC, ln = threadIdx.x & 63;
+      f32x4* const wl = reinterpret_cast<f32x4*>(smem_all);
+      f32x4 w[NCW];
+      if (y == 2) {
+        const NetView& N3 = P.b3.t[0].net;
+        LDR_REQUEST(w, N3.base + N3.off_Wb[1], cs * NWC + lw);
+        LDR_PUBLISH(wl, w);
+        ldr_bar();
+        ldr_bar(2);
+        if (P.b3.t[0].dx) ldr_bar(2);
+        return;
+      }
+      const NetView& N1 = P.f3.t[y].net;
+      LDR_REQUEST(w, N1.base + N1.off_W[1], cs * NWC + lw);
+      ldr_bar();
+      LDR_PUBLISH(wl, w);
+      ldr_bar();
+      const NetView& N2 = P.b2.t[y].net;
+      LDR_REQUEST(w, N2.base + N2.off_Wb[1], cs * NWC + lw);
+      ldr_bar(3);
+      ldr_bar();
+      LDR_PUBLISH(wl, w);
+      ldr_bar();
+      ldr_bar(2);
+      if (P.b2.t[y].dx) ldr_bar(2);
+      ldr_bar();
+      return;
+    }
+  }
+#define XCH_LDR LD
+#define XCH_WSLICE (reinterpret_cast<const float4*>(smem_all))
+  if (y == 2) {
+    {
+      const BwdArgs& A = P.b3;
+      const BwdTask& T = A.t[0];
+#define XCH_HOOK_ACT
+#define XCH_HOOK_HEAD xch_wait(f2, 2 * CS, P.err); ILSX_STAMP(P.dbg, 4);
+#include "bwd_split_tile.inc"
+#undef XCH_HOOK_ACT
+#undef XCH_HOOK_HEAD
+    }
+    ILSX_STAMP(P.dbg, 5);
+    return;
+  }
+  {
+    const FwdArgs& A = P.f3;
+    const FwdTask& T = A.t[y];
+    const bool first_task = y == 0;
+#define XCH_HOOK_STAGE
+#define XCH_HOOK_FIN
+#include "fwd_split_tile.inc"
+#undef XCH_HOOK_STAGE
+#undef XCH_HOOK_FIN
+  }
+  ILSX_STAMP(P.dbg, 1);
+  xch_arrive(f1);
+  {
+    const BwdArgs& A = P.b2;
+    const BwdTask& T = A.t[y];
+#define XCH_HOOK_ACT xch_wait(f1, 2 * CS, P.err); ILSX_STAMP(P.dbg, 2);
+#define XCH_HOOK_HEAD
+#include "bwd_split_tile.inc"
+#undef XCH_HOOK_ACT
+#undef XCH_HOOK_HEAD
+  }
+  ILSX_STAMP(P.dbg, 3);
+  xch_arrive(f2);
+#undef XCH_LDR
+#undef XCH_WSLICE
diff --git a/include/ilsx.h b/include/ilsx.h
--- a/include/ilsx.h
+++ b/include/ilsx.h
@@ -134,6 +134,7 @@
                         const float* eps_cur, ilsx_sac_stats* stats);
 int ilsx_sac_train_from_replay(ilsx_sac* sac, ilsx_replay* rb, int n_steps, int B, ilsx_sac_stats* stats);
 int ilsx_sac_phase_state(ilsx_sac* sac, int* fallbacks, int* disabled, int* last_window_on_phase, int* wgs_per_cu_a, int* wgs_per_cu_c);
+int ilsx_phase_launch_shape(int H, int KP, int loader, int* threads, int* lds_bytes);
 int ilsx_sac_debug_break_phase(ilsx_sac* sac);
 int ilsx_sac_set_batch(ilsx_sac* sac, const float* obs, const float* act, const float* rew,
                        const float* done, const float* nobs, int B, const float* eps_next,
```

Result: slower. 17020 (-1.4%).
